# ZZWaang/polyphonic-chord-texture-disentanglement

Measured on AMD Instinct MI355X. Metric: 2-bar piano-roll samples/sec (train step), higher is better.
Workload: dtype bf16; 1 GPU; configs[1]: 1xMI355X batch=512/GPU, bf16 MFMA GRU/Linear, z_dim=256+256, teacher-forced decoder (tfr=1), fwd+bwd+clip+Adam; per_gpu_batch=512, global_batch=512, parallelism=dp1

## Files before the change

### include/ptvae_hip.h

```cpp
#ifndef PTVAE_HIP_H
#define PTVAE_HIP_H

#ifdef __cplusplus
extern "C" {
#endif

#define PTV_PREC_F32 0
#define PTV_PREC_BF16 1

#define PTV_A_BF16 1
#define PTV_B_BF16 2
#define PTV_C_BF16 4
#define PTV_GRU_GATES_BF16 1
#define PTV_GRU_GI_BF16 2
#define PTV_GRU_GI2_BF16 4
#define PTV_GRU_DG_BF16 8
#define PTV_GRU_W_BF16 16
#define PTV_GRU_EXT_BF16 64
#define PTV_GRU_SKIP_CAST0 32

const char* ptv_arch(void);
int ptv_abi_version(void);
const char* ptv_header_hash(void);

int ptv_gemm(int prec, int transA, int transB, int M, int N, int K,
             const void* A, long lda, const void* B, long ldb,
             void* C, long ldc, const float* bias, float alpha,
             int accumulate, int act, int splitk, int dtypes, void* stream);
int ptv_gemm_mtop(int prec, int transA, int transB, int M, int N, int K, const void* A, long lda, const void* B, long ldb,
                  void* C, long ldc, const float* bias, float alpha, int accumulate, int act, int splitk, int dtypes,
                  const int* m_top, long m_unit, void* stream);
int ptv_gemm_mtop_seg(int prec, int transA, int transB, int M, int N, int K, const void* A, long lda, const void* B, long ldb,
                      void* C, long ldc, const float* bias, float alpha, int accumulate, int act, int splitk, int dtypes,
                      const int* m_top, long m_unit, const int* seg_n, long seg_unit, int seg_period, void* stream);
int ptv_gemm_priority(int p);

int ptv_gru_seq_fwd(int prec, int M, int H, int T,
                    const void* gi, long gi_step_stride, long gi_ld,
                    const void* gi2, long gi2_step_stride, long gi2_ld,
                    const void* w_hh, const float* b_hh,
                    float* hall, void* hall16, void* gates,
                    const int* lengths, int reverse, const int* gi_idx, int flags, void* stream);

int ptv_gru_step_fwd(int prec, int M, int H,
                     const float* hprev, long ld_hprev, const void* hprev16, void* hout16,
                     const void* gi, long gi_ld, const void* gi2, long gi2_ld,
                     const void* w_hh, const float* b_hh,
                     float* hout, long ld_hout,
                     void* gates, long gates_plane,
                     const int* lengths, int t, const int* gi_idx, int flags, void* stream);

int ptv_gru_seq_bwd(int prec, int M, int H, int T,
                    const float* hall, const void* gates, const void* w_hh,
                    const void* dh_ext, long ext_step_stride, long ext_ld,
                    const float* dh_last, long last_ld,
                    const float* lr_a, long lr_step_stride, long lr_lda, int lr_k, const float* lr_b,
                    void* dgi, void* dgh, float* dhz, float* dh0,
                    int reverse, int flags, void* stream);

int ptv_gru_persist_supported(int NC, int M, int H);
int ptv_gru_persist_cu_reserve(int cus);
int ptv_gru_persist_load_policy(int lp);
int ptv_gru_persist_fwd(int NC, int M, int H, int T,
                        const void* const* gi, const long* gi_step, const long* gi_ld,
                        const void* const* gi2, const long* gi2_step, const long* gi2_ld,
                        const void* const* w_hh16, const float* const* b_hh,
                        float* const* hall, void* const* hall16, void* const* gates,
                        const int* const* lengths, const int* reverse, void* const* xch, unsigned* sync, void* stream);
int ptv_gru_persist_bwd(int NC, int M, int H, int T,
                        const float* const* hall, const void* const* gates, const void* const* w_t16,
                        const void* const* dh_ext, const long* ext_step, const long* ext_ld, const int* ext_bf16,
                        const float* const* dh_last, const long* last_ld,
                        void* const* dgi, void* const* dgh, float* const* dh0,
                        const int* reverse, void* const* xch, unsigned* sync, void* stream);
int ptv_gru_persist_splitk_supported(int NC, int M, int H, int S);
long ptv_gru_persist_part_elems(int NC, int M, int H, int S);
int ptv_gru_persist_bwd_splitk(int S, int NC, int M, int H, int T,
                               const float* const* hall, const void* const* gates, const void* const* w_t16,
                               const void* const* dh_ext, const long* ext_step, const long* ext_ld, const int* ext_bf16,
                               const float* const* dh_last, const long* last_ld,
                               void* const* dgi, void* const* dgh, float* const* dh0,
                               const int* reverse, void* const* xch, float* const* part, unsigned* sync, void* stream);

int ptv_copy2d(float* dst, long ldd, const float* src, long lds, long rows, int cols, float alpha,
               int accumulate, void* stream);
int ptv_transpose01(float* dst, const float* src, int D0, int D1, int W, void* stream);
int ptv_sum_steps(float* out, const void* in, long n, int T, long stride, int accumulate, int in_bf16, void* stream);
int ptv_zero_skip(int enable);
int ptv_last_nonzero_unit(const float* x, long rows, int cols, long ld, long unit, int* top, void* stream);
int ptv_sum_steps_top(float* out, const void* in, long n, int T, long stride, int accumulate, int in_bf16, const int* t_top,
                      void* stream);
int ptv_sum_steps_seg(float* out, const void* in, long n, int T, long stride, int accumulate, int in_bf16, const int* t_top,
                      const int* seg_n, long row_elems, void* stream);
int ptv_colsum(float* out, const void* A, long lda, long rows, int N, const int* sel, int G, int a_bf16, void* stream);

int ptv_embed_fwd(const long* x, const float* W, const float* bias, float* emb, int* lengths, int B, int E, void* stream);
int ptv_multihot(const long* x, float* out, long ld, int B, void* stream);
int ptv_grid_lengths(const long* x, int* lengths, int B, void* stream);
int ptv_multihot_bf16(const long* x, void* out, long ld, int B, void* stream);
int ptv_embed_fwd_geom(const long* x, const float* W, const float* bias, float* emb, int* lengths, int B, int E,
                       int S, int N, int P, int D, int pad, void* stream);
int ptv_grid_lengths_geom(const long* x, int* lengths, int B, int S, int N, int D, int pad, void* stream);
int ptv_multihot_geom(const long* x, void* out, long ld, int B, int S, int N, int P, int D, int bf16, void* stream);

int ptv_txt_conv_relu_pool_fwd(const float* pr_mat, const float* w, const float* bias, float* pooled, int B, int C, void* stream);
int ptv_txt_conv_relu_pool_bwd(const float* pr_mat, const float* w, const float* bias, const float* dpooled,
                               float* dw, float* dbias, int B, int C, void* stream);
int ptv_txt_conv_relu_pool_fwd_rows(const float* pr_mat, const float* w, const float* bias, float* feat, long ld, int B, int C,
                                    signed char* arg, void* stream);
int ptv_txt_conv_relu_pool_bwd_rows(const float* pr_mat, const float* w, const float* bias, const float* dfeat, long ld,
                                    float* dw, float* dbias, int B, int C, const signed char* arg, void* stream);

int ptv_philox_normal(float* out, long rows, int Z, unsigned long long seed, unsigned long long stream_id, long row_offset,
                      void* stream);
int ptv_reparam_kl_fwd(const float* mu, const float* sd, const float* eps, float* z, long ldz, float* kl_sum, int B, int Z, void* stream);
int ptv_reparam_kl_bwd(const float* mu, const float* sd, const float* eps, const float* dz, long lddz,
                       const float* dmu_ext, const float* dsd_ext, float klw, int mul_sd, float* dmu, float* dlv, int B, int Z, void* stream);

int ptv_pianotree_targets(const long* x, int B, int step_major, int* pitch_t, int* dur_t, int* counts, void* stream);
int ptv_pianotree_targets_rows(const long* x, int B, int step_major, int* pitch_t, int* dur_t, int* counts, int* row_live, void* stream);
int ptv_gather_rows(void* dst, const void* src, const int* idx, long rows, int row_words, long src_plane_words, long dst_plane_words, int planes,
                    void* stream);
int ptv_scatter_rows(void* dst, const void* src, const int* idx, long rows, int row_words, long src_plane_words, long dst_plane_words, int planes,
                     void* stream);
int ptv_gather_rows_seg(void* dst, const void* src, const int* idx, long rows, int row_words, long src_plane_words, long dst_plane_words,
                        int planes, const int* seg_n, void* stream);
int ptv_scatter_rows_seg(void* dst, const void* src, const int* idx, long rows, int row_words, long src_plane_words, long dst_plane_words,
                         int planes, const int* seg_n, void* stream);
int ptv_chord_targets(const float* c, int B, int step_major, int* root_t, int* chroma_t, int* bass_t, void* stream);
int ptv_ce_fwd(const float* logits, long ld, const int* targets, long rows, int C, int ignore_index, float* nll_sum, void* stream);
int ptv_ce_bwd(const float* logits, long ld, const int* targets, long rows, int C, int ignore_index, const float* gscale,
               float* dlogits, long ldd, void* stream);
int ptv_ce_group_fwd(const float* logits, long ld, const int* targets, long rows, int C, int ignore_index, int G,
                     float* nll_sum, int* count, void* stream);
int ptv_ce_group_bwd(const float* logits, long ld, const int* targets, long rows, int C, int ignore_index, int G,
// ... 413 lines not shown
```

### polyphonic_chord_texture_disentanglement_amd/csrc/composite.hip

```cpp
#include "common.hpp"
#include "../../include/ptvae_hip.h"

namespace {

inline const void* T_(const void* const* t, int i) { return t[i]; }
template <typename X> inline X* M_(const void* const* t, int i) { return reinterpret_cast<X*>(const_cast<void*>(t[i])); }

constexpr int A16 = 1, B16 = 2, C16 = 4, CBLK16 = 16;

struct WgradGroup {
  ptv_wgrad_job jobs[8]; int n = 0; int P; void* stream;
  WgradGroup(int prec, void* st) : P(prec), stream(st) {}
  int add(int M, int N, long K, const void* A, long lda, int a_bf16, const void* B, long ldb, int b_bf16, float* C, long ldc, float* csum,
          const int* k_top = nullptr, long k_unit = 0, int k_rev = 0, int accumulate = 1, const int* seg_n = nullptr, long seg_unit = 0,
          int seg_period = 0) {
    if (P == PTV_PREC_BF16 && K >= 512) {
      if (n == 8) PTV_TRY(flush());
      jobs[n++] = ptv_wgrad_job{M, N, (int)K, A, lda, B, ldb, C, ldc, 1.f, accumulate, (a_bf16 ? 1 : 0) | (b_bf16 ? 2 : 0), 0, csum, k_top, k_unit, k_rev,
                                seg_n, seg_n ? seg_unit : 0, seg_n ? seg_period : 0};
      return PTV_OK;
    }
    if (k_top) return PTV_ERR_ARG;
    PTV_TRY(ptv_gemm(P, 1, 1, M, N, (int)K, A, lda, B, ldb, C, ldc, nullptr, 1.f, accumulate, 0, 0, (a_bf16 ? A16 : 0) | (b_bf16 ? B16 : 0), stream));
    if (csum) PTV_TRY(ptv_colsum(csum, A, lda, K, M, nullptr, 1, a_bf16, stream));
// ... 123 lines not shown
  PTV_TRY(ptv_gemm(P, 0, 0, (int)TB, nr, H, hs, H, T_(t, PTV_CDF_W_ROOT), H, M_<void>(t, PTV_CDF_ROOT), nr, (const float*)T_(t, PTV_CDF_B_ROOT), 1.f, 0,
                   0, 0, 0, stream));
  PTV_TRY(ptv_gemm(P, 0, 0, (int)TB, nc, H, hs, H, T_(t, PTV_CDF_W_CHROMA), H, M_<void>(t, PTV_CDF_CHROMA), nc, (const float*)T_(t, PTV_CDF_B_CHROMA),
                   1.f, 0, 0, 0, 0, stream));
  PTV_TRY(ptv_gemm(P, 0, 0, (int)TB, nb, H, hs, H, T_(t, PTV_CDF_W_BASS), H, M_<void>(t, PTV_CDF_BASS), nb, (const float*)T_(t, PTV_CDF_B_BASS), 1.f, 0,
                   0, 0, 0, stream));
  return PTV_OK;
}

extern "C" int ptv_chord_decoder_bwd(const void* const* t, const long* d, void* stream) {
  if (!t || !d) return PTV_ERR_ARG;
  const int B = (int)d[PTV_CDB_D_B], T = (int)d[PTV_CDB_D_T], H = (int)d[PTV_CDB_D_H], I = (int)d[PTV_CDB_D_I], Z = (int)d[PTV_CDB_D_Z],
            Zi = (int)d[PTV_CDB_D_ZI], P = (int)d[PTV_CDB_D_PREC], abf = d[PTV_CDB_D_ACT_BF16] ? 1 : 0, persist = (int)d[PTV_CDB_D_PERSIST],
            S = (int)d[PTV_CDB_D_SPLITK];
  if (B <= 0 || T <= 0 || H <= 0 || I <= 0 || Z <= 0 || Zi <= 0 || (P != PTV_PREC_F32 && P != PTV_PREC_BF16)) return PTV_ERR_ARG;
  for (int i = 0; i < PTV_CDB_COUNT; i++) {
    const bool optional = i == PTV_CDB_WT16_HH || i == PTV_CDB_DROOT || i == PTV_CDB_DCHROMA || i == PTV_CDB_DBASS || i == PTV_CDB_DHZ ||
                          i == PTV_CDB_XCH || i == PTV_CDB_PART || i == PTV_CDB_SYNC || i == PTV_CDB_WAIT_EVENT || i == PTV_CDB_RECORD_EVENT;
    if (!t[i] && !optional) return PTV_ERR_ARG;
  }
  if (persist && (!t[PTV_CDB_WT16_HH] || !t[PTV_CDB_XCH] || !t[PTV_CDB_SYNC] || !abf || (S && !t[PTV_CDB_PART]))) return PTV_ERR_ARG;
  if (!persist && !t[PTV_CDB_DHZ]) return PTV_ERR_ARG;
  hipStream_t s = (hipStream_t)stream;
  const long TB = (long)T * B, ld_ih = (long)I + Zi;
  const float* hall = (const float*)T_(t, PTV_CDB_HALL);
  const float* hs = hall + (long)B * H;
  float* dhs = M_<float>(t, PTV_CDB_DHS);
  const int heads[3][4] = {{PTV_CDB_DROOT, PTV_CDB_W_ROOT, PTV_CDB_G_W_ROOT, PTV_CDB_G_B_ROOT},
                           {PTV_CDB_DCHROMA, PTV_CDB_W_CHROMA, PTV_CDB_G_W_CHROMA, PTV_CDB_G_B_CHROMA},
                           {PTV_CDB_DBASS, PTV_CDB_W_BASS, PTV_CDB_G_W_BASS, PTV_CDB_G_B_BASS}};
  const int ncls[3] = {(int)d[PTV_CDB_D_NROOT], (int)d[PTV_CDB_D_NCHROMA], (int)d[PTV_CDB_D_NBASS]};
  bool have = false;
  WgradGroup wg(P, stream);
  for (int k = 0; k < 3; k++) {
    const void* dl = T_(t, heads[k][0]);
    if (!dl) continue;
    const int n = ncls[k];
    PTV_TRY(ptv_gemm(P, 0, 1, (int)TB, H, n, dl, n, T_(t, heads[k][1]), H, dhs, H, nullptr, 1.f, have ? 1 : 0, 0, 0, 0, stream));
    have = true;
    PTV_TRY(wg.add(n, H, TB, dl, n, 0, hs, H, 0, M_<float>(t, heads[k][2]), H, M_<float>(t, heads[k][3])));
  }
  PTV_TRY(wg.flush());
  if (!have && hipMemsetAsync(dhs, 0, sizeof(float) * TB * H, s) != hipSuccess) return PTV_ERR_LAUNCH;
  void* dgi = M_<void>(t, PTV_CDB_DGI); void* dgh = M_<void>(t, PTV_CDB_DGH);
  float* dh0 = M_<float>(t, PTV_CDB_DH0);
  if (persist) {
    const float* hall_[1] = {hall}; const void* gates_[1] = {T_(t, PTV_CDB_GATES)}; const void* wt_[1] = {T_(t, PTV_CDB_WT16_HH)};
    const void* ext_[1] = {dhs}; const long ext_step[1] = {(long)B * H}, ext_ld[1] = {(long)H}; const int ext_bf[1] = {0};
    const float* last_[1] = {nullptr}; const long last_ld[1] = {0};
    void* dgi_[1] = {dgi}; void* dgh_[1] = {dgh}; float* dh0_[1] = {dh0}; const int rev[1] = {0};
    void* xch_[1] = {M_<void>(t, PTV_CDB_XCH)}; float* part_[1] = {M_<float>(t, PTV_CDB_PART)};
    if (t[PTV_CDB_WAIT_EVENT] && hipStreamWaitEvent(s, (hipEvent_t)const_cast<void*>(t[PTV_CDB_WAIT_EVENT]), 0) != hipSuccess) return PTV_ERR_LAUNCH;
    if (S) PTV_TRY(ptv_gru_persist_bwd_splitk(S, 1, B, H, T, hall_, gates_, wt_, ext_, ext_step, ext_ld, ext_bf, last_, last_ld, dgi_, dgh_, dh0_, rev,
                                              xch_, part_, M_<unsigned>(t, PTV_CDB_SYNC), stream));
    else PTV_TRY(ptv_gru_persist_bwd(1, B, H, T, hall_, gates_, wt_, ext_, ext_step, ext_ld, ext_bf, last_, last_ld, dgi_, dgh_, dh0_, rev, xch_,
                                     M_<unsigned>(t, PTV_CDB_SYNC), stream));
    if (t[PTV_CDB_RECORD_EVENT] && hipEventRecord((hipEvent_t)const_cast<void*>(t[PTV_CDB_RECORD_EVENT]), s) != hipSuccess) return PTV_ERR_LAUNCH;
  } else {
    const void* w = t[PTV_CDB_WT16_HH] ? T_(t, PTV_CDB_WT16_HH) : T_(t, PTV_CDB_W_HH);
    const int flags = abf | (abf << 3) | ((t[PTV_CDB_WT16_HH] ? 1 : 0) << 4);
    PTV_TRY(ptv_gru_seq_bwd(P, B, H, T, hall, T_(t, PTV_CDB_GATES), w, dhs, (long)B * H, H, nullptr, 0, nullptr, 0, 0, 0, nullptr, dgi, dgh,
                            M_<float>(t, PTV_CDB_DHZ), dh0, 0, flags, stream));
  }
  const int A = abf ? A16 : 0;
  float* dzg = M_<float>(t, PTV_CDB_DZG);
  PTV_TRY(ptv_sum_steps_top(dzg, dgi, (long)B * 3 * H, T, (long)B * 3 * H, 0, abf, nullptr, stream));
  float* g_ih = M_<float>(t, PTV_CDB_G_W_IH);
  const float* w_ih = (const float*)T_(t, PTV_CDB_W_IH);
  float* dz_in = M_<float>(t, PTV_CDB_DZ_IN); float* dtok0 = M_<float>(t, PTV_CDB_DTOK0);
  PTV_TRY(ptv_gemm(P, 0, 1, B, Zi, 3 * H, dzg, 3L * H, w_ih + I, ld_ih, dz_in, Zi, nullptr, 1.f, 0, 0, 0, 0, stream));
  PTV_TRY(ptv_gemm(P, 0, 1, B, I, 3 * H, dgi, 3L * H, w_ih, ld_ih, dtok0, I, nullptr, 1.f, 0, 0, 0, A, stream));
  float* dz = M_<float>(t, PTV_CDB_DZ);
  PTV_TRY(ptv_gemm(P, 0, 1, B, Z, H, dh0, H, T_(t, PTV_CDB_W_ZHID), Z, dz, Z, nullptr, 1.f, 0, 0, 0, 0, stream));
  PTV_TRY(ptv_gemm(P, 0, 1, B, Z, Zi, dz_in, Zi, T_(t, PTV_CDB_W_ZIN), Z, dz, Z, nullptr, 1.f, 1, 0, 0, 0, stream));
  PTV_TRY(wg.add(3 * H, H, TB, dgh, 3L * H, abf, hall, H, 0, M_<float>(t, PTV_CDB_G_W_HH), H, M_<float>(t, PTV_CDB_G_B_HH)));
  PTV_TRY(wg.add(3 * H, Zi, B, dzg, 3L * H, 0, T_(t, PTV_CDB_Z_IN), Zi, 0, g_ih + I, ld_ih, M_<float>(t, PTV_CDB_G_B_IH)));
  PTV_TRY(wg.add(3 * H, I, TB, dgi, 3L * H, abf, T_(t, PTV_CDB_TOKS), I, 0, g_ih, ld_ih, nullptr));
  PTV_TRY(wg.add(H, Z, B, dh0, H, 0, T_(t, PTV_CDB_Z), Z, 0, M_<float>(t, PTV_CDB_G_W_ZHID), Z, M_<float>(t, PTV_CDB_G_B_ZHID)));
  PTV_TRY(wg.add(Zi, Z, B, dz_in, Zi, 0, T_(t, PTV_CDB_Z), Z, 0, M_<float>(t, PTV_CDB_G_W_ZIN), Z, M_<float>(t, PTV_CDB_G_B_ZIN)));
  PTV_TRY(wg.flush());
  PTV_TRY(ptv_colsum(M_<float>(t, PTV_CDB_G_INIT_INPUT), dtok0, I, B, I, nullptr, 1, 0, stream));
  return PTV_OK;
}

extern "C" int ptv_decoder_tf_bwd(const void* const* t, const long* d, void* stream) {
  if (!t || !d) return PTV_ERR_ARG;
  for (int i = 0; i < PTV_DTB_COUNT; i++)
    if (!t[i] && i != PTV_DTB_TOP_H && i != PTV_DTB_PART_T && i != PTV_DTB_WAIT_EVENT && i != PTV_DTB_RECORD_EVENT && i != PTV_DTB_PERM &&
        i != PTV_DTB_ROW_LEN && i != PTV_DTB_NS16S && i != PTV_DTB_DNS_S && i != PTV_DTB_DTOK_S && i != PTV_DTB_SEG_N)
      return PTV_ERR_ARG;
  const bool sorted = t[PTV_DTB_PERM] != nullptr;
  if (sorted != (t[PTV_DTB_ROW_LEN] != nullptr) || sorted != (t[PTV_DTB_NS16S] != nullptr) || sorted != (t[PTV_DTB_DNS_S] != nullptr) ||
      sorted != (t[PTV_DTB_DTOK_S] != nullptr) || (sorted && !t[PTV_DTB_TOP_H]))
    return PTV_ERR_ARG;
  const int* perm = (const int*)T_(t, PTV_DTB_PERM);
  const int* row_len = (const int*)T_(t, PTV_DTB_ROW_LEN);

  const int B = (int)d[PTV_DTB_D_B], E = (int)d[PTV_DTB_D_E], He = (int)d[PTV_DTB_D_HE], Ht = (int)d[PTV_DTB_D_HT], Hn = (int)d[PTV_DTB_D_HN],
            Hd = (int)d[PTV_DTB_D_HD], NP = (int)d[PTV_DTB_D_NP], Zs = (int)d[PTV_DTB_D_ZS], Zi = (int)d[PTV_DTB_D_ZI], nblk = (int)d[PTV_DTB_D_NBLK],
            S = (int)d[PTV_DTB_D_SPLITK];
  const long ldp = d[PTV_DTB_D_LDP];
  if (B <= 0 || E != 128 || Hn != 512 || Hd != 64 || NP != 130 || ldp < NP || nblk <= 0 || (S && !t[PTV_DTB_PART_T])) return PTV_ERR_UNSUPPORTED;
  const int R = 32 * B;
  const int* seg_n = t[PTV_DTB_PERM] ? (const int*)T_(t, PTV_DTB_SEG_N) : nullptr;
  if (seg_n && !ptv_wgrad_seg_supported(15L * R, R)) return PTV_ERR_ARG;
  const long M = 15L * R;
  const int P = PTV_PREC_BF16;
  hipStream_t s = (hipStream_t)stream, side = (hipStream_t)const_cast<void*>(t[PTV_DTB_SIDE_STREAM]);
  void* sside = (void*)side;
  const int psz = ptv_dur_gru_bwd_part_size();
  const int* top_h = (const int*)T_(t, PTV_DTB_TOP_H);
  const long top_unit = top_h ? R : 0;
  auto fork = [&](int k) -> int {
    hipEvent_t e = (hipEvent_t)const_cast<void*>(t[PTV_DTB_FORK_EVENT0 + k]);
    if (hipEventRecord(e, s) != hipSuccess || hipStreamWaitEvent(side, e, 0) != hipSuccess) return PTV_ERR_LAUNCH;
    return PTV_OK;
  };
  float* G_ = nullptr; (void)G_;
#define GB(i) M_<float>(t, i)

  float* ddur = GB(PTV_DTB_DDUR); float* dHD0 = GB(PTV_DTB_DHD0); float* part = GB(PTV_DTB_PART);
  const void* HD16 = T_(t, PTV_DTB_HD16);
  ptv_gemm_priority(1);
  PTV_TRY(ptv_dur_gru_bwd(Hd, M, nullptr, M * Hd, 4 * M * Hd, HD16, M * Hd, 1, ddur, 10, (const float*)T_(t, PTV_DTB_W_HH_D),
                          (const float*)T_(t, PTV_DTB_W_OUT_D), (const int*)T_(t, PTV_DTB_IDX), M, dHD0, part, nblk,
                          (const float*)T_(t, PTV_DTB_B_HH_D), (const float*)T_(t, PTV_DTB_TAB0), (const float*)T_(t, PTV_DTB_TAB), stream));
  PTV_TRY(fork(0));
  ptv_gemm_priority(0);
  PTV_TRY(ptv_dur_out_wgrad(ddur, 10, HD16, M * Hd, GB(PTV_DTB_G_W_OUT_D), M, Hd, sside));
  PTV_TRY(ptv_colsum(GB(PTV_DTB_TMP64), ddur, 64, M * 10 / 64, 64, nullptr, 1, 0, sside));
  PTV_TRY(ptv_colsum(GB(PTV_DTB_G_B_OUT_D), GB(PTV_DTB_TMP64), 2, 32, 2, nullptr, 1, 0, sside));
  PTV_TRY(ptv_colsum(GB(PTV_DTB_S), part, psz, nblk, psz, nullptr, 1, 0, sside));
  PTV_TRY(ptv_dur_bwd_finalize(GB(PTV_DTB_S), GB(PTV_DTB_G_W_HH_D), GB(PTV_DTB_G_B_HH_D), GB(PTV_DTB_G_B_IH_D), GB(PTV_DTB_G_W_IH_D), GB(PTV_DTB_G_SOS),
                               (const float*)T_(t, PTV_DTB_W_IH_D), (const float*)T_(t, PTV_DTB_SOS), 5, sside));

  float* dP = GB(PTV_DTB_DP);
  void* dNSUM = M_<void>(t, PTV_DTB_DNSUM); void* dY16 = M_<void>(t, PTV_DTB_DY16);
  ptv_gemm_priority(1);
  PTV_TRY(ptv_heads_bwd_rows(dP, ldp, dHD0, T_(t, PTV_DTB_PK_WDPT), T_(t, PTV_DTB_PK_WCAT), dNSUM, top_h ? 3 : 1, dY16, top_h, top_unit, row_len, M,
                             stream));
  PTV_TRY(fork(1));
  ptv_gemm_priority(0);
  {
    const __bf16* HN16 = (const __bf16*)T_(t, PTV_DTB_HN16);
    const __bf16* nsum = HN16 + (long)R * Hn;
    float* tmp = GB(PTV_DTB_TMP200); float* cs = GB(PTV_DTB_CS200);
    WgradGroup wg(P, sside);
    PTV_TRY(wg.add(200, Hn, M, dY16, 200, 1, nsum, Hn, 1, tmp, Hn, cs, top_h, top_unit, 0, 0, seg_n, R, 15));
    PTV_TRY(wg.add(Hd, NP, M, dHD0, Hd, 0, T_(t, PTV_DTB_PITCH), ldp, 0, GB(PTV_DTB_G_W_DH) + Hn, (long)Hn + NP, nullptr, top_h, top_unit, 0, 1, seg_n, R, 15));
    PTV_TRY(wg.flush());
    PTV_TRY(ptv_copy2d(GB(PTV_DTB_G_W_P), Hn, tmp, Hn, NP, Hn, 1.f, 1, sside));
    PTV_TRY(ptv_copy2d(GB(PTV_DTB_G_B_P), NP, cs, NP, 1, NP, 1.f, 1, sside));
    PTV_TRY(ptv_copy2d(GB(PTV_DTB_G_W_DH), (long)Hn + NP, tmp + 136L * Hn, Hn, Hd, Hn, 1.f, 1, sside));
    PTV_TRY(ptv_copy2d(GB(PTV_DTB_G_B_DH), Hd, cs + 136, Hd, 1, Hd, 1.f, 1, sside));
  }

  void* dgi_n = M_<void>(t, PTV_DTB_DGI_N); void* dgh_n = M_<void>(t, PTV_DTB_DGH_N);
  float* dHN0 = GB(PTV_DTB_DHN0); int* top_step = M_<int>(t, PTV_DTB_TOP_STEP);
  float* dGC = GB(PTV_DTB_DGC);
  float* dNS_out = GB(PTV_DTB_DNS); float* dtok_out = GB(PTV_DTB_DTOK);
  float* dNS = sorted ? GB(PTV_DTB_DNS_S) : dNS_out;
  float* dtok = sorted ? GB(PTV_DTB_DTOK_S) : dtok_out;
  const __bf16* wt_ih_n = (const __bf16*)T_(t, PTV_DTB_WT_IH_N);
  ptv_gemm_priority(1);
  PTV_TRY(ptv_notes_gru_persist_bwd_rows(T_(t, PTV_DTB_PK_NOTES_WT), T_(t, PTV_DTB_HN16), T_(t, PTV_DTB_GATES_N), dNSUM, dgi_n, dgh_n, dHN0,
                                         M_<void>(t, PTV_DTB_SCRATCH_N), R, 15 | (seg_n ? 0x10000 : 0), top_h, row_len, top_step, stream));
  PTV_TRY(ptv_sum_steps_seg(dGC, dgi_n, (long)R * 3 * Hn, 15, (long)R * 3 * Hn, 0, 1, top_step, seg_n, 3L * Hn, stream));
  if (hipMemsetAsync(dtok_out + 15L * R * E, 0, sizeof(float) * R * E, s) != hipSuccess) return PTV_ERR_LAUNCH;
  PTV_TRY(ptv_gemm_mtop_seg(P, 0, 0, (int)M, E, 3 * Hn, dgi_n, 3L * Hn, wt_ih_n + (long)Ht * 3 * Hn, 3L * Hn, dtok, E, nullptr, 1.f, 0, 0, 0, A16 | B16,
                            top_step, R, seg_n, R, 15, stream));
  PTV_TRY(ptv_gemm(P, 0, 0, R, Ht, 3 * Hn, dGC, 3L * Hn, wt_ih_n, 3L * Hn, dNS, Ht, nullptr, 1.f, 0, 0, 0, B16, stream));
  PTV_TRY(ptv_gemm(P, 0, 0, R, Ht, Hn, dHN0, Hn, T_(t, PTV_DTB_WT_T2N), Hn, dNS, Ht, nullptr, 1.f, 1, 0, 0, B16, stream));
  if (sorted) {
    PTV_TRY(ptv_scatter_rows(dNS_out, dNS, perm, R, Ht, 0, 0, 1, stream));
    PTV_TRY(ptv_scatter_rows_seg(dtok_out, dtok, perm, R, E, (long)R * E, (long)R * E, 15, seg_n, stream));
  }
  PTV_TRY(fork(2));
  ptv_gemm_priority(0);
  {
    const __bf16* HN16 = (const __bf16*)T_(t, PTV_DTB_HN16);
    const __bf16* NSf = sorted ? (const __bf16*)T_(t, PTV_DTB_NS16S) : (const __bf16*)T_(t, PTV_DTB_NS16) + (long)B * Ht;
    float* gw = GB(PTV_DTB_G_W_HH_N); float* gb = GB(PTV_DTB_G_B_HH_N); float* gih = GB(PTV_DTB_G_W_IH_N);
    WgradGroup wg(P, sside);
    PTV_TRY(wg.add(2 * Hn, Hn, M, dgi_n, 3L * Hn, 1, HN16, Hn, 1, gw, Hn, gb, top_step, R, 0, 1, seg_n, R, 15));
    PTV_TRY(wg.add(Hn, Hn, M, dgh_n, Hn, 1, HN16, Hn, 1, gw + 2L * Hn * Hn, Hn, gb + 2 * Hn, top_step, R, 0, 1, seg_n, R, 15));
    PTV_TRY(wg.add(3 * Hn, Ht, R, dGC, 3L * Hn, 0, NSf, Ht, 1, gih, (long)Ht + E, GB(PTV_DTB_G_B_IH_N)));
    PTV_TRY(wg.add(3 * Hn, E, M, dgi_n, 3L * Hn, 1, T_(t, PTV_DTB_TOK_OP), E, 0, gih + Ht, (long)Ht + E, nullptr, top_step, R, 0, 1, seg_n, R, 15));
    PTV_TRY(wg.add(Hn, Ht, R, dHN0, Hn, 0, NSf, Ht, 1, GB(PTV_DTB_G_W_T2N), Ht, GB(PTV_DTB_G_B_T2N)));
    PTV_TRY(wg.flush());
  }

  void* dgi_t = M_<void>(t, PTV_DTB_DGI_T); void* dgh_t = M_<void>(t, PTV_DTB_DGH_T);
  float* dzhid = GB(PTV_DTB_DZHID); float* dZG = GB(PTV_DTB_DZG); float* dz_in = GB(PTV_DTB_DZ_IN); float* dTOKS = GB(PTV_DTB_DTOKS);
  float* dz = GB(PTV_DTB_DZ);
  const __bf16* wt_ih_t = (const __bf16*)T_(t, PTV_DTB_WT_IH_T);
  ptv_gemm_priority(1);
  {
    const float* hall_[1] = {(const float*)T_(t, PTV_DTB_NS)}; const void* gates_[1] = {T_(t, PTV_DTB_GATES_T)};
    const void* wt_[1] = {T_(t, PTV_DTB_WT_HH_T)};
    const void* ext_[1] = {dNS_out}; const long ext_step[1] = {(long)B * Ht}, ext_ld[1] = {(long)Ht}; const int ext_bf[1] = {0};
    const float* last_[1] = {nullptr}; const long last_ld[1] = {0};
    void* dgi_[1] = {dgi_t}; void* dgh_[1] = {dgh_t}; float* dh0_[1] = {dzhid}; const int rev[1] = {0};
    void* xch_[1] = {M_<void>(t, PTV_DTB_XCH)}; float* part_[1] = {M_<float>(t, PTV_DTB_PART_T)};
    if (t[PTV_DTB_WAIT_EVENT] && hipStreamWaitEvent(s, (hipEvent_t)const_cast<void*>(t[PTV_DTB_WAIT_EVENT]), 0) != hipSuccess) return PTV_ERR_LAUNCH;
    if (S) PTV_TRY(ptv_gru_persist_bwd_splitk(S, 1, B, Ht, 32, hall_, gates_, wt_, ext_, ext_step, ext_ld, ext_bf, last_, last_ld, dgi_, dgh_, dh0_,
                                              rev, xch_, part_, M_<unsigned>(t, PTV_DTB_SYNC), stream));
    else PTV_TRY(ptv_gru_persist_bwd(1, B, Ht, 32, hall_, gates_, wt_, ext_, ext_step, ext_ld, ext_bf, last_, last_ld, dgi_, dgh_, dh0_, rev, xch_,
                                     M_<unsigned>(t, PTV_DTB_SYNC), stream));
    if (t[PTV_DTB_RECORD_EVENT] && hipEventRecord((hipEvent_t)const_cast<void*>(t[PTV_DTB_RECORD_EVENT]), s) != hipSuccess) return PTV_ERR_LAUNCH;
  }
  PTV_TRY(ptv_sum_steps_top(dZG, dgi_t, (long)B * 3 * Ht, 32, (long)B * 3 * Ht, 0, 1, nullptr, stream));
  PTV_TRY(ptv_gemm(P, 0, 0, B, Zi, 3 * Ht, dZG, 3L * Ht, wt_ih_t + 2L * He * 3 * Ht, 3L * Ht, dz_in, Zi, nullptr, 1.f, 0, 0, 0, B16, stream));
  if (hipMemsetAsync(dTOKS + 32L * B * 2 * He, 0, sizeof(float) * B * 2 * He, s) != hipSuccess) return PTV_ERR_LAUNCH;
  PTV_TRY(ptv_gemm(P, 0, 0, R, 2 * He, 3 * Ht, dgi_t, 3L * Ht, wt_ih_t, 3L * Ht, dTOKS, 2L * He, nullptr, 1.f, 0, 0, 0, A16 | B16, stream));
  PTV_TRY(ptv_gemm(P, 0, 0, B, Zs, Ht, dzhid, Ht, T_(t, PTV_DTB_WT_ZHID), Ht, dz, Zs, nullptr, 1.f, 0, 0, 0, B16, stream));
  PTV_TRY(ptv_gemm(P, 0, 0, B, Zs, Zi, dz_in, Zi, T_(t, PTV_DTB_WT_ZIN), Zi, dz, Zs, nullptr, 1.f, 1, 0, 0, B16, stream));
  PTV_TRY(fork(3));
  ptv_gemm_priority(0);
  {
    const __bf16* NS16 = (const __bf16*)T_(t, PTV_DTB_NS16);
    float* g_ih = GB(PTV_DTB_G_W_IH_T); float* gb_ih = GB(PTV_DTB_G_B_IH_T); float* gb_hh = GB(PTV_DTB_G_B_HH_T);
    const long ld_t = 2L * He + Zi;
    WgradGroup wg(P, sside);
    PTV_TRY(wg.add(3 * Ht, Ht, R, dgh_t, 3L * Ht, 1, NS16, Ht, 1, GB(PTV_DTB_G_W_HH_T), Ht, gb_hh));
    PTV_TRY(wg.add(3 * Ht, Zi, B, dZG, 3L * Ht, 0, T_(t, PTV_DTB_Z_IN), Zi, 0, g_ih + 2 * He, ld_t, gb_ih));
    PTV_TRY(wg.add(3 * Ht, 2 * He, R, dgi_t, 3L * Ht, 1, T_(t, PTV_DTB_TOKS), 2L * He, 0, g_ih, ld_t, nullptr));
    PTV_TRY(wg.add(Ht, Zs, B, dzhid, Ht, 0, T_(t, PTV_DTB_Z), Zs, 0, GB(PTV_DTB_G_W_ZHID), Zs, GB(PTV_DTB_G_B_ZHID)));
    PTV_TRY(wg.add(Zi, Zs, B, dz_in, Zi, 0, T_(t, PTV_DTB_Z), Zs, 0, GB(PTV_DTB_G_W_ZIN), Zs, GB(PTV_DTB_G_B_ZIN)));
    PTV_TRY(wg.flush());
    PTV_TRY(ptv_colsum(GB(PTV_DTB_G_INIT_INPUT), dTOKS, 2L * He, B, 2 * He, nullptr, 1, 0, sside));
  }
  ptv_gemm_priority(1);
#undef GB
  return PTV_OK;
}

extern "C" int ptv_bigru_final_bwd(const void* const* t, const long* d, void* stream) {
  if (!t || !d) return PTV_ERR_ARG;
  const int M = (int)d[PTV_BGB_D_M], T = (int)d[PTV_BGB_D_T], H = (int)d[PTV_BGB_D_H], I = (int)d[PTV_BGB_D_I], xbf = d[PTV_BGB_D_X_BF16] ? 1 : 0,
            dx_acc = d[PTV_BGB_D_DX_ACC] ? 1 : 0, S = (int)d[PTV_BGB_D_SPLITK];
  if (M <= 0 || T < 2 || H <= 0 || I <= 0) return PTV_ERR_ARG;
  const bool want_dx = t[PTV_BGB_DX] != nullptr;
  for (int i = 0; i < PTV_BGB_COUNT; i++) {
    const bool optional = i == PTV_BGB_WT_IH0 || i == PTV_BGB_WT_IH1 || i == PTV_BGB_DX || i == PTV_BGB_PART0 || i == PTV_BGB_PART1 ||
                          i == PTV_BGB_WAIT_EVENT || i == PTV_BGB_RECORD_EVENT;
    if (!t[i] && !optional) return PTV_ERR_ARG;
  }
  if ((want_dx && (!t[PTV_BGB_WT_IH0] || !t[PTV_BGB_WT_IH1])) || (S && (!t[PTV_BGB_PART0] || !t[PTV_BGB_PART1]))) return PTV_ERR_ARG;
  const int P = PTV_PREC_BF16;
  hipStream_t s = (hipStream_t)stream, side = (hipStream_t)const_cast<void*>(t[PTV_BGB_SIDE_STREAM]);
  void* sside = (void*)side;
  const long TM = (long)T * M;
  const float* dout = (const float*)T_(t, PTV_BGB_DOUT);
  void* dgi[2] = {M_<void>(t, PTV_BGB_DGI0), M_<void>(t, PTV_BGB_DGI1)};
  void* dgh[2] = {M_<void>(t, PTV_BGB_DGH0), M_<void>(t, PTV_BGB_DGH1)};
  ptv_gemm_priority(1);
  {
    const float* hall_[2] = {(const float*)T_(t, PTV_BGB_HALL0), (const float*)T_(t, PTV_BGB_HALL1)};
    const void* gates_[2] = {T_(t, PTV_BGB_GATES0), T_(t, PTV_BGB_GATES1)};
    const void* wt_[2] = {T_(t, PTV_BGB_WT_HH0), T_(t, PTV_BGB_WT_HH1)};
    const void* ext_[2] = {nullptr, nullptr}; const long ext_step[2] = {0, 0}, ext_ld[2] = {0, 0}; const int ext_bf[2] = {0, 0};
    const float* last_[2] = {dout, dout + H}; const long last_ld[2] = {2L * H, 2L * H};
    float* dh0_[2] = {nullptr, nullptr}; const int rev[2] = {0, 1};
    void* xch_[2] = {M_<void>(t, PTV_BGB_XCH0), M_<void>(t, PTV_BGB_XCH1)};
    float* part_[2] = {M_<float>(t, PTV_BGB_PART0), M_<float>(t, PTV_BGB_PART1)};
    if (t[PTV_BGB_WAIT_EVENT] && hipStreamWaitEvent(s, (hipEvent_t)const_cast<void*>(t[PTV_BGB_WAIT_EVENT]), 0) != hipSuccess) return PTV_ERR_LAUNCH;
    if (S) PTV_TRY(ptv_gru_persist_bwd_splitk(S, 2, M, H, T, hall_, gates_, wt_, ext_, ext_step, ext_ld, ext_bf, last_, last_ld, dgi, dgh, dh0_, rev,
                                              xch_, part_, M_<unsigned>(t, PTV_BGB_SYNC), stream));
    else PTV_TRY(ptv_gru_persist_bwd(2, M, H, T, hall_, gates_, wt_, ext_, ext_step, ext_ld, ext_bf, last_, last_ld, dgi, dgh, dh0_, rev, xch_,
                                     M_<unsigned>(t, PTV_BGB_SYNC), stream));
    if (t[PTV_BGB_RECORD_EVENT] && hipEventRecord((hipEvent_t)const_cast<void*>(t[PTV_BGB_RECORD_EVENT]), s) != hipSuccess) return PTV_ERR_LAUNCH;
  }
  const void* x = T_(t, PTV_BGB_X);
  auto products = [&](int dir, void* st) -> int {
    const int o = dir ? 4 : 0;
    WgradGroup wg(P, st);
    PTV_TRY(wg.add(3 * H, I, TM, dgi[dir], 3L * H, 1, x, I, xbf, M_<float>(t, PTV_BGB_G_W_IH0 + o), I, M_<float>(t, PTV_BGB_G_B_IH0 + o)));
    PTV_TRY(wg.add(3 * H, H, TM, dgh[dir], 3L * H, 1, T_(t, dir ? PTV_BGB_H16_1 : PTV_BGB_H16_0), H, 1, M_<float>(t, PTV_BGB_G_W_HH0 + o), H,
                   M_<float>(t, PTV_BGB_G_B_HH0 + o), nullptr, 0, dir ? T : 0));
    return wg.flush();
  };
  hipEvent_t ef = (hipEvent_t)const_cast<void*>(t[PTV_BGB_FORK_EVENT]), ej = (hipEvent_t)const_cast<void*>(t[PTV_BGB_JOIN_EVENT]);
  if (hipEventRecord(ef, s) != hipSuccess || hipStreamWaitEvent(side, ef, 0) != hipSuccess) return PTV_ERR_LAUNCH;
  ptv_gemm_priority(0);
  PTV_TRY(products(1, sside));
  ptv_gemm_priority(1);
  PTV_TRY(products(0, stream));
  float* dx = M_<float>(t, PTV_BGB_DX);
  if (want_dx) PTV_TRY(ptv_gemm(P, 0, 0, (int)TM, I, 3 * H, dgi[0], 3L * H, T_(t, PTV_BGB_WT_IH0), 3L * H, dx, I, nullptr, 1.f, dx_acc, 0, 0, A16 | B16, stream));
  if (hipEventRecord(ej, side) != hipSuccess || hipStreamWaitEvent(s, ej, 0) != hipSuccess) return PTV_ERR_LAUNCH;
  if (want_dx) PTV_TRY(ptv_gemm(P, 0, 0, (int)TM, I, 3 * H, dgi[1], 3L * H, T_(t, PTV_BGB_WT_IH1), 3L * H, dx, I, nullptr, 1.f, 1, 0, 0, A16 | B16, stream));
  return PTV_OK;
}

extern "C" int ptv_bigru_final_fwd(const void* const* t, const long* d, void* stream) {
  if (!t || !d) return PTV_ERR_ARG;
  const int M = (int)d[PTV_BGF_D_M], T = (int)d[PTV_BGF_D_T], H = (int)d[PTV_BGF_D_H], I = (int)d[PTV_BGF_D_I], xbf = d[PTV_BGF_D_X_BF16] ? 1 : 0;
  if (M <= 0 || T < 2 || H <= 0 || I <= 0) return PTV_ERR_ARG;
  for (int i = 0; i < PTV_BGF_COUNT; i++)
    if (!t[i] && i != PTV_BGF_LENGTHS && i != PTV_BGF_WAIT_EVENT && i != PTV_BGF_RECORD_EVENT) return PTV_ERR_ARG;
  const int P = PTV_PREC_BF16;
  hipStream_t s = (hipStream_t)stream;
  const long TM = (long)T * M;
  const int gi_slot[2] = {PTV_BGF_GI0, PTV_BGF_GI1}, hall_slot[2] = {PTV_BGF_HALL0, PTV_BGF_HALL1};
  const int wih_slot[2] = {PTV_BGF_W16_IH0, PTV_BGF_W16_IH1}, bih_slot[2] = {PTV_BGF_B_IH0, PTV_BGF_B_IH1};
  for (int dir = 0; dir < 2; dir++) {
    PTV_TRY(ptv_gemm(P, 0, 0, (int)TM, 3 * H, I, T_(t, PTV_BGF_X), I, T_(t, wih_slot[dir]), I, M_<void>(t, gi_slot[dir]), 3L * H,
                     (const float*)T_(t, bih_slot[dir]), 1.f, 0, 0, -1, (xbf ? A16 : 0) | (d[PTV_BGF_D_WIH_F32] ? 0 : B16) | C16, stream));
    if (hipMemsetAsync(M_<void>(t, hall_slot[dir]), 0, sizeof(float) * M * H, s) != hipSuccess) return PTV_ERR_LAUNCH;
  }
  {
    const void* gi[2] = {T_(t, PTV_BGF_GI0), T_(t, PTV_BGF_GI1)}; const long gi_step[2] = {(long)M * 3 * H, (long)M * 3 * H}, gi_ld[2] = {3L * H, 3L * H};
    const void* gi2[2] = {nullptr, nullptr}; const long z2[2] = {0, 0};
    const void* w16[2] = {T_(t, PTV_BGF_W16_HH0), T_(t, PTV_BGF_W16_HH1)};
    const float* bhh[2] = {(const float*)T_(t, PTV_BGF_B_HH0), (const float*)T_(t, PTV_BGF_B_HH1)};
    float* hall[2] = {M_<float>(t, PTV_BGF_HALL0), M_<float>(t, PTV_BGF_HALL1)};
    void* h16[2] = {M_<void>(t, PTV_BGF_H16_0), M_<void>(t, PTV_BGF_H16_1)};
    void* gates[2] = {M_<void>(t, PTV_BGF_GATES0), M_<void>(t, PTV_BGF_GATES1)};
    const int* len[2] = {(const int*)T_(t, PTV_BGF_LENGTHS), (const int*)T_(t, PTV_BGF_LENGTHS)}; const int rev[2] = {0, 1};
    void* xch[2] = {M_<void>(t, PTV_BGF_XCH0), M_<void>(t, PTV_BGF_XCH1)};
    if (t[PTV_BGF_WAIT_EVENT] && hipStreamWaitEvent(s, (hipEvent_t)const_cast<void*>(t[PTV_BGF_WAIT_EVENT]), 0) != hipSuccess) return PTV_ERR_LAUNCH;
    PTV_TRY(ptv_gru_persist_fwd(2, M, H, T, gi, gi_step, gi_ld, gi2, z2, z2, w16, bhh, hall, h16, gates, len, rev, xch, M_<unsigned>(t, PTV_BGF_SYNC),
                                stream));
// ... 283 lines not shown
```

### polyphonic_chord_texture_disentanglement_amd/csrc/gemm.hip

```cpp
#include <stdlib.h>
#include <mutex>
#include <type_traits>
#include "common.hpp"
#include "gemm_core.hpp"
#include "../../include/ptvae_hip.h"

namespace ptv {

struct EpiPlain {
  struct Params {
    void* C; long ldc;
    const float* bias;
    float alpha;
    int accumulate;
    int act;
    int atomic;
    int c_bf16;
    int c_blocked;
    int c_rows;
    long split_stride;
  };
  static __device__ __forceinline__ long coff(const Params& p, int m, int n) {
    return p.c_blocked ? (((long)(n >> p.c_blocked) * p.c_rows + m) << p.c_blocked) + (n & ((1 << p.c_blocked) - 1)) : (long)m * p.ldc + n;
  }
  static __device__ __forceinline__ bool dead_is_noop(const Params& p) { return (p.accumulate || p.atomic) && p.act == 0 && p.bias == nullptr; }
  template <int FM, int FN, int NG> struct Pre {};
  template <int FM, int FN, int NG>
  static __device__ __forceinline__ void prefetch(const Params&, Pre<FM, FN, NG>&, int, int, int, int) {}
  template <int FN> static constexpr bool staged() { return FN == 2 || FN == 4; }
  template <int FM, int FN, int NG> static constexpr int lds_bytes() { return staged<FN>() ? 4 * RowStage<1, (staged<FN>() ? FN * 16 : 64)>::WAVE_BYTES : 0; }
  template <int FM, int FN, int NG>
  static __device__ __forceinline__ void apply(const Params& p_in, f32x4 (&acc)[FM][NG * FN], const Pre<FM, FN, NG>&,
                                               int m0, int n0, int M, int N, int split, char* lds) {
    Params q = p_in;
    if (q.split_stride) q.C = reinterpret_cast<float*>(q.C) + (long)split * q.split_stride;
    const Params& p = q;
    const bool bf = p.c_bf16 != 0;
    const bool vec = (p.c_blocked || (p.ldc & 3) == 0) && ((reinterpret_cast<uintptr_t>(p.C) & (bf ? 7 : 15)) == 0);
    const bool use_bias = p.bias != nullptr && split == 0;
    if constexpr (staged<FN>()) {
      using RS = RowStage<1, FN * 16>;
      float* st = RS::base(lds);
      const int u = RS::unit();
      const bool bias_ok = !use_bias || (reinterpret_cast<uintptr_t>(p.bias) & 15) == 0;
      if (vec && bias_ok && p.act == 0 && m0 + 16 * FM <= M && n0 + 16 * FN <= N && !(bf && p.atomic)) {
        const int mode = p.atomic ? 3 : (p.accumulate ? (bf ? 4 : 2) : (bf ? 1 : 0));
        float4 b4 = make_float4(0.f, 0.f, 0.f, 0.f);
        if (use_bias) b4 = *reinterpret_cast<const float4*>(p.bias + n0 + u);
        if (mode == 0) fast_rows<FM, FN, 0>(p, acc, st, m0, n0 + u, b4);
        else if (mode == 1) fast_rows<FM, FN, 1>(p, acc, st, m0, n0 + u, b4);
        else if (mode == 2) fast_rows<FM, FN, 2>(p, acc, st, m0, n0 + u, b4);
        else if (mode == 4) fast_rows<FM, FN, 4>(p, acc, st, m0, n0 + u, b4);
        else fast_rows<FM, FN, 3>(p, acc, st, m0, n0 + u, b4);
        return;
      }
#pragma unroll
      for (int i = 0; i < FM; i++) {
        RS::put(st, acc[i]);
#pragma unroll
        for (int c = 0; c < RS::PASSES; c++) {
          const int row = RS::row(c), m = m0 + i * 16 + row, n = n0 + u;
          if (m < M && n < N) cell(p, m, n, N, RS::get(st, row, u), bf, vec, use_bias);
        }
        __builtin_amdgcn_wave_barrier();
      }
    } else {
      const int lane = threadIdx.x & 63;
#pragma unroll
      for (int i = 0; i < FM; i++)
#pragma unroll
        for (int j = 0; j < FN; j++) {
          const int m = m0 + i * 16 + (lane & 15), n = n0 + j * 16 + (lane >> 4) * 4;
          if (m < M && n < N) cell(p, m, n, N, acc[i][j], bf, vec, use_bias);
        }
    }
  }
  template <int FM, int FN, int MODE>
  static __device__ __forceinline__ void fast_rows(const Params& p, f32x4 (&acc)[FM][FN], float* st, int m0, int n, const float4& b4) {
    using RS = RowStage<1, FN * 16>;
    const int u = RS::unit();
#pragma unroll
    for (int i = 0; i < FM; i++) {
      RS::put(st, acc[i]);
#pragma unroll
      for (int c = 0; c < RS::PASSES; c++) {
        const int row = RS::row(c);
        const f32x4 a = RS::get(st, row, u);
        const long off = coff(p, m0 + i * 16 + row, n);
        float v0 = p.alpha * a[0] + b4.x, v1 = p.alpha * a[1] + b4.y, v2 = p.alpha * a[2] + b4.z, v3 = p.alpha * a[3] + b4.w;
        if constexpr (MODE == 1 || MODE == 4) {
          if constexpr (MODE == 4) {
            const bf16x4 q = *reinterpret_cast<const bf16x4*>(reinterpret_cast<const __bf16*>(p.C) + off);
            v0 += (float)q[0]; v1 += (float)q[1]; v2 += (float)q[2]; v3 += (float)q[3];
          }
          bf16x4 o; o[0] = (__bf16)v0; o[1] = (__bf16)v1; o[2] = (__bf16)v2; o[3] = (__bf16)v3;
          *reinterpret_cast<bf16x4*>(reinterpret_cast<__bf16*>(p.C) + off) = o;
        } else if constexpr (MODE == 3) {
          float* cp = reinterpret_cast<float*>(p.C) + off;
          atomicAdd(cp, v0); atomicAdd(cp + 1, v1); atomicAdd(cp + 2, v2); atomicAdd(cp + 3, v3);
        } else {
          float4* cp = reinterpret_cast<float4*>(reinterpret_cast<float*>(p.C) + off);
          if constexpr (MODE == 2) { const float4 q = *cp; v0 += q.x; v1 += q.y; v2 += q.z; v3 += q.w; }
          *cp = make_float4(v0, v1, v2, v3);
        }
      }
      __builtin_amdgcn_wave_barrier();
    }
  }
  static __device__ __forceinline__ void cell(const Params& p, int m, int n, int N, const f32x4& a, bool bf, bool vec, bool use_bias) {
    float v[4];
#pragma unroll
    for (int e = 0; e < 4; e++) {
      v[e] = p.alpha * a[e];
      if (use_bias && n + e < N) v[e] += p.bias[n + e];
      if (p.act == 1) v[e] = expf(v[e]);
    }
    const long off = coff(p, m, n);
    if (p.atomic) {
      float* c = reinterpret_cast<float*>(p.C) + off;
#pragma unroll
      for (int e = 0; e < 4; e++) if (n + e < N) atomicAdd(c + e, v[e]);
    } else if (vec && n + 3 < N) {
      if (p.accumulate) { const float4 q = ld4f(p.C, off, bf); v[0] += q.x; v[1] += q.y; v[2] += q.z; v[3] += q.w; }
      st4f(p.C, off, bf, v[0], v[1], v[2], v[3]);
    } else {
#pragma unroll
      for (int e = 0; e < 4; e++) if (n + e < N) st1f(p.C, off + e, bf, p.accumulate ? ld1f(p.C, off + e, bf) + v[e] : v[e]);
    }
  }
};

#ifndef PTV_PF_TN
#define PTV_PF_TN 3
#endif
#ifndef PTV_PF_NT
#define PTV_PF_NT 2
#endif
#define PLAIN_PF_BIG(KA, KB, SA, SB) ((SA) && (SB) ? ((KA) ? PTV_PF_TN : PTV_PF_NT) : 1)

template <class CT, int BM, int BN, int WGM, int WGN, bool KA, bool KB, bool SA, bool SB>
__global__ __launch_bounds__(NTHREADS, 2) void gemm_plain_kernel(GemmArgs g, EpiPlain::Params ep) {
  if (g.prio) __builtin_amdgcn_s_setprio(3);
  gemm_body<CT, BM, BN, WGM, WGN, 1, KA, KB, EpiPlain, SA, SB, (BM * BN <= 64 * 64 ? 2 : PLAIN_PF_BIG(KA, KB, SA, SB))>(g, ep);
}

__global__ void splitk_reduce_kernel(float* __restrict__ C, long ldc, const float* __restrict__ ws, int M, int N, int splits, int accumulate) {
  const long total = (long)M * N;
  for (long i = (long)blockIdx.x * blockDim.x + threadIdx.x; i < total; i += (long)gridDim.x * blockDim.x) {
    float sum = 0.f;
    for (int z = 0; z < splits; z++) sum += ws[(long)z * total + i];
    float* cp = C + (i / N) * ldc + (i % N);
    *cp = (accumulate ? *cp : 0.f) + sum;
  }
}

__global__ void fill_rows_kernel(float* C, long ldc, int M, int N, float v) {
  long i = (long)blockIdx.x * blockDim.x + threadIdx.x;
  long total = (long)M * N;
  for (; i < total; i += (long)gridDim.x * blockDim.x) C[(i / N) * ldc + (i % N)] = v;
}

template <class CT, int BM, int BN, bool KA, bool KB, bool SA, bool SB>
static void launch_plain(const GemmArgs& g, const EpiPlain::Params& ep, int splits, hipStream_t s) {
  dim3 grid(cdiv(g.N, BN), cdiv(g.M, BM), splits);
  hipLaunchKernelGGL((gemm_plain_kernel<CT, BM, BN, 2, 2, KA, KB, SA, SB>), grid, dim3(NTHREADS), 0, s, g, ep);
}

int g_splitk_ordered = [] { const char* e = getenv("PTV_WGRAD_ORDERED"); return (e && e[0] == '0') ? 0 : 1; }();

static float* splitk_workspace(hipStream_t s, size_t bytes) {
  struct Buf { float* p; size_t bytes; };
  static Buf pool[64]; static hipStream_t keys[64]; static int n = 0; static std::mutex mu;
  std::lock_guard<std::mutex> lock(mu);
  int i = 0;
  for (; i < n; i++) if (keys[i] == s) break;
  if (i == n) { if (n == 64) return nullptr; keys[n++] = s; pool[i] = Buf{nullptr, 0}; }
  Buf& b = pool[i];
  if (b.bytes < bytes) {
    hipStreamCaptureStatus st = hipStreamCaptureStatusNone;
    if (hipStreamIsCapturing(s, &st) == hipSuccess && st != hipStreamCaptureStatusNone) return nullptr;
    const size_t want = bytes + bytes / 4;
    if (hipMalloc(reinterpret_cast<void**>(&b.p), want) != hipSuccess) { b = Buf{nullptr, 0}; return nullptr; }
    b.bytes = want;
  }
  return b.p;
}

template <class CT, bool SA, bool SB>
static int gemm_dispatch(int transA, int transB, GemmArgs g, EpiPlain::Params ep, int splitk, hipStream_t s) {
  const long blocks_big = (long)cdiv(g.M, 128) * cdiv(g.N, 128);
  const bool deepk = transA && g.K >= 4096;
  const bool big = blocks_big >= 192 || (deepk && g.M >= 256 && g.N >= 256);
  const int bm = big ? 128 : 64;
  long blocks = (long)cdiv(g.M, bm) * cdiv(g.N, bm);
  int splits = 1;
  if (splitk > 0) splits = splitk;
  else if (splitk == 0 && blocks < 256 && g.K >= 8 * CT::BK && ep.act == 0 && !ep.c_bf16) {
    const long target = deepk ? (big ? 640 : 1536) : 512;
    splits = (int)((target + blocks - 1) / blocks);
    int maxs = g.K / (4 * CT::BK);
    if (splits > maxs) splits = maxs;
    if (splits > 192) splits = 192;
    if (splits < 1) splits = 1;
  }
  int kper = g.K;
  if (splits > 1) {
    if (splits >= 8) splits = (splits + 7) / 8 * 8;
    kper = cdiv(cdiv(g.K, splits), CT::BK) * CT::BK;
    const int s2 = cdiv(g.K, kper);
    if (s2 != splits && (s2 & 7) != 0 && s2 >= 8) {
      splits = s2 / 8 * 8;
      kper = cdiv(cdiv(g.K, splits), CT::BK) * CT::BK;
      splits = cdiv(g.K, kper);
    } else splits = s2;
  }
  g.k_per_split = kper;
  float* ws = nullptr;
  const EpiPlain::Params ep_user = ep;
  if (splits > 1 && g_splitk_ordered) {
    ws = splitk_workspace(s, (size_t)splits * g.M * g.N * sizeof(float));
    if (!ws) g_ord_fallbacks++;
  }
  if (ws) {
    ep.C = ws; ep.ldc = g.N; ep.accumulate = 0; ep.atomic = 0; ep.split_stride = (long)g.M * g.N;
  } else if (splits > 1) {
    ep.atomic = 1;
    if (!ep.accumulate) {
      long total = (long)g.M * g.N;
      int nb = (int)((total + 255) / 256); if (nb > 2048) nb = 2048;
      hipLaunchKernelGGL(fill_rows_kernel, dim3(nb), dim3(256), 0, s, reinterpret_cast<float*>(ep.C), ep.ldc, g.M, g.N, 0.f);
    }
  }
#define PTV_LAUNCH(KA, KB)                                              \
  do {                                                                  \
    if (big) launch_plain<CT, 128, 128, KA, KB, SA, SB>(g, ep, splits, s);      \
    else launch_plain<CT, 64, 64, KA, KB, SA, SB>(g, ep, splits, s);            \
  } while (0)
  if (!transA && !transB) PTV_LAUNCH(false, false);
  else if (!transA && transB) PTV_LAUNCH(false, true);
  else if (transA && transB) PTV_LAUNCH(true, true);
  else PTV_LAUNCH(true, false);
#undef PTV_LAUNCH
  if (ws) {
    const long total = (long)g.M * g.N;
    int nb = (int)((total + 255) / 256); if (nb > 2048) nb = 2048;
    hipLaunchKernelGGL(splitk_reduce_kernel, dim3(nb), dim3(256), 0, s, reinterpret_cast<float*>(ep_user.C), ep_user.ldc, ws, g.M, g.N, splits, ep_user.accumulate);
  }
  return PTV_OK;
}

}

namespace ptv { int g_gemm_prio = 0; }
extern "C" int ptv_gemm_priority(int p) { ptv::g_gemm_prio = p ? 1 : 0; return PTV_OK; }

extern "C" int ptv_gemm_mtop(int prec, int transA, int transB, int M, int N, int K,
                             const void* A, long lda, const void* B, long ldb,
                             void* C, long ldc, const float* bias, float alpha,
                             int accumulate, int act, int splitk, int dtypes, const int* m_top, long m_unit, void* stream) {
  return ptv_gemm_mtop_seg(prec, transA, transB, M, N, K, A, lda, B, ldb, C, ldc, bias, alpha, accumulate, act, splitk, dtypes, m_top, m_unit, nullptr, 0, 0,
                           stream);
}

extern "C" int ptv_gemm_mtop_seg(int prec, int transA, int transB, int M, int N, int K,
                                 const void* A, long lda, const void* B, long ldb,
                                 void* C, long ldc, const float* bias, float alpha,
                                 int accumulate, int act, int splitk, int dtypes, const int* m_top, long m_unit,
                                 const int* seg_n, long seg_unit, int seg_period, void* stream) {
  if (M < 0 || N < 0 || K < 0 || !A || !B || !C) return PTV_ERR_ARG;
  if (M == 0 || N == 0) return PTV_OK;
  const bool sa = dtypes & 1, sb = dtypes & 2, sc = dtypes & 4;
  if ((sa || sb) && prec != PTV_PREC_BF16) return PTV_ERR_ARG;
  if (sc && splitk > 1) return PTV_ERR_ARG;
  if ((dtypes & 8) && (dtypes & 16)) return PTV_ERR_ARG;
  if ((dtypes & 8) && ((N & 31) || splitk > 1)) return PTV_ERR_ARG;
  if ((dtypes & 16) && ((N & 15) || splitk > 1)) return PTV_ERR_ARG;
  if ((dtypes & 24) && splitk == 0) splitk = 1;
  if (prec == PTV_PREC_BF16 && transA && transB && !sc && !(dtypes & 24) && !bias && act == 0 && K >= 512 && splitk <= 0)
    return ptv_wgrad(M, N, K, A, lda, B, ldb, reinterpret_cast<float*>(C), ldc, alpha, accumulate, dtypes & 3, 0, nullptr, nullptr, 0, 0, stream);
  if (m_top && (transA || m_unit <= 0)) return PTV_ERR_ARG;
  if (seg_n && (transA || seg_unit <= 0 || (seg_unit & 127) || seg_period <= 0)) return PTV_ERR_ARG;
  ptv::GemmArgs g{A, lda, B, ldb, M, N, K, K, 0, m_top, m_unit, ptv::g_gemm_prio, seg_n, (int)seg_unit, seg_period};
  ptv::EpiPlain::Params ep{C, ldc, bias, alpha, accumulate, act, 0, sc ? 1 : 0, (dtypes & 8) ? 5 : ((dtypes & 16) ? 4 : 0), M, 0};
  hipStream_t s = (hipStream_t)stream;
  int rc;
  if (prec != PTV_PREC_BF16) rc = ptv::gemm_dispatch<ptv::F32, false, false>(transA, transB, g, ep, splitk, s);
  else if (sa && sb) rc = ptv::gemm_dispatch<ptv::BF16, true, true>(transA, transB, g, ep, splitk, s);
  else if (sa) rc = ptv::gemm_dispatch<ptv::BF16, true, false>(transA, transB, g, ep, splitk, s);
  else if (sb) rc = ptv::gemm_dispatch<ptv::BF16, false, true>(transA, transB, g, ep, splitk, s);
  else rc = ptv::gemm_dispatch<ptv::BF16, false, false>(transA, transB, g, ep, splitk, s);
  if (rc != PTV_OK) return rc;
  PTV_CHECK_LAUNCH();
  return PTV_OK;
}

extern "C" int ptv_gemm(int prec, int transA, int transB, int M, int N, int K,
                        const void* A, long lda, const void* B, long ldb,
                        void* C, long ldc, const float* bias, float alpha,
                        int accumulate, int act, int splitk, int dtypes, void* stream) {
  return ptv_gemm_mtop(prec, transA, transB, M, N, K, A, lda, B, ldb, C, ldc, bias, alpha, accumulate, act, splitk, dtypes, nullptr, 0, stream);
}
```

### polyphonic_chord_texture_disentanglement_amd/csrc/gemm_core.hpp

```cpp
#pragma once
#include <hip/hip_runtime.h>
#include <stdint.h>
#include <type_traits>

namespace ptv {

typedef __attribute__((ext_vector_type(8))) __bf16 bf16x8;
typedef __attribute__((ext_vector_type(4))) __bf16 bf16x4;
typedef __attribute__((ext_vector_type(4))) float f32x4;

constexpr int NTHREADS = 256;

__device__ __forceinline__ float4 ld4f(const void* p, long i, bool bf) {
  if (bf) {
    const bf16x4 v = *reinterpret_cast<const bf16x4*>(reinterpret_cast<const __bf16*>(p) + i);
    return make_float4((float)v[0], (float)v[1], (float)v[2], (float)v[3]);
  }
  return *reinterpret_cast<const float4*>(reinterpret_cast<const float*>(p) + i);
}
__device__ __forceinline__ void st4f(void* p, long i, bool bf, float a, float b, float c, float d) {
  if (bf) {
    bf16x4 v; v[0] = (__bf16)a; v[1] = (__bf16)b; v[2] = (__bf16)c; v[3] = (__bf16)d;
    *reinterpret_cast<bf16x4*>(reinterpret_cast<__bf16*>(p) + i) = v;
  } else {
    *reinterpret_cast<float4*>(reinterpret_cast<float*>(p) + i) = make_float4(a, b, c, d);
  }
}
__device__ __forceinline__ float ld1f(const void* p, long i, bool bf) {
  return bf ? (float)reinterpret_cast<const __bf16*>(p)[i] : reinterpret_cast<const float*>(p)[i];
}
__device__ __forceinline__ void st1f(void* p, long i, bool bf, float v) {
  if (bf) reinterpret_cast<__bf16*>(p)[i] = (__bf16)v; else reinterpret_cast<float*>(p)[i] = v;
}

struct BF16 {
  using T = __bf16;
  static constexpr int BK = 64;
  static constexpr int LDS_LD = 64;
  static constexpr int CH = 8;
};
struct F32 {
  using T = float;
  static constexpr int BK = 32;
  static constexpr int LDS_LD = 32;
  static constexpr int CH = 4;
};

struct GemmArgs {
  const void* A; long lda;
  const void* B; long ldb;
  int M, N, K;
  int k_per_split;
  long gate_stride;
  const int* m_top; long m_unit;
  int prio;
  const int* seg_n = nullptr; int seg_unit = 0, seg_period = 0;
};

template <class CT> __device__ __forceinline__ int swz(int row, int k) {
  return row * CT::LDS_LD + ((((k / CT::CH) ^ ((row >> 2) ^ row)) & 7) * CT::CH) + (k % CT::CH);
}

template <bool SB> struct SrcT { using T = float; };
template <> struct SrcT<true> { using T = __bf16; };

template <class CT, bool SB> struct Chunk;
template <> struct Chunk<BF16, false> {
  float4 lo, hi;
  __device__ __forceinline__ void zero() { lo = hi = make_float4(0.f, 0.f, 0.f, 0.f); }
  __device__ __forceinline__ void set(int e, float x) { if (e < 4) (&lo.x)[e] = x; else (&hi.x)[e - 4] = x; }
  __device__ __forceinline__ void load16(const float* q) { lo = *reinterpret_cast<const float4*>(q); hi = *reinterpret_cast<const float4*>(q + 4); }
  __device__ __forceinline__ void store(__bf16* d) const {
    bf16x8 v;
    v[0] = (__bf16)lo.x; v[1] = (__bf16)lo.y; v[2] = (__bf16)lo.z; v[3] = (__bf16)lo.w;
    v[4] = (__bf16)hi.x; v[5] = (__bf16)hi.y; v[6] = (__bf16)hi.z; v[7] = (__bf16)hi.w;
    *reinterpret_cast<bf16x8*>(d) = v;
  }
};
template <> struct Chunk<BF16, true> {
  bf16x8 v;
  __device__ __forceinline__ void zero() { for (int e = 0; e < 8; e++) v[e] = (__bf16)0.f; }
  __device__ __forceinline__ void set(int e, __bf16 x) { v[e] = x; }
  __device__ __forceinline__ void load16(const __bf16* q) { v = *reinterpret_cast<const bf16x8*>(q); }
  __device__ __forceinline__ void store(__bf16* d) const { *reinterpret_cast<bf16x8*>(d) = v; }
};
template <> struct Chunk<F32, false> {
  float4 lo;
  __device__ __forceinline__ void zero() { lo = make_float4(0.f, 0.f, 0.f, 0.f); }
  __device__ __forceinline__ void set(int e, float x) { (&lo.x)[e] = x; }
  __device__ __forceinline__ void load16(const float* q) { lo = *reinterpret_cast<const float4*>(q); }
  __device__ __forceinline__ void store(float* d) const { *reinterpret_cast<float4*>(d) = lo; }
};

template <class CT, int ROWS, bool SB>
struct StageKC {
  using S = typename SrcT<SB>::T;
  static constexpr int CPR = 8;
  static constexpr int RPP = NTHREADS / CPR;
  static constexpr int NP = ROWS / RPP;
  static_assert(ROWS % RPP == 0, "tile rows must be a multiple of 32");
  Chunk<CT, SB> v[NP];

  template <class RowMap>
  __device__ __forceinline__ void load(const S* __restrict__ p, long ld, int k0, int kend, bool vec_ok, RowMap rowmap) {
    const int tid = threadIdx.x;
    const int c = tid % CPR, r0 = tid / CPR;
    const int k = k0 + c * CT::CH;
#pragma unroll
    for (int i = 0; i < NP; i++) {
// ... 164 lines not shown
  template <class BRow>
  static __device__ __forceinline__ void run(const float* As, int a_row0, const float* Bs, BRow b_row, f32x4 (&acc)[FM][FNT]) {
    const int lane = threadIdx.x & 63;
    const int r = lane & 15, kq = (lane >> 4) * 4;
#pragma unroll
    for (int ks = 0; ks < F32::BK; ks += 16) {
      float4 a[FM], b[FNT];
#pragma unroll
      for (int i = 0; i < FM; i++) a[i] = *reinterpret_cast<const float4*>(As + swz<F32>(a_row0 + i * 16 + r, ks + kq));
#pragma unroll
      for (int j = 0; j < FNT; j++) b[j] = *reinterpret_cast<const float4*>(Bs + swz<F32>(b_row(j) + r, ks + kq));
#pragma unroll
      for (int i = 0; i < FM; i++)
#pragma unroll
        for (int j = 0; j < FNT; j++) {
          acc[i][j] = __builtin_amdgcn_mfma_f32_16x16x4f32(b[j].x, a[i].x, acc[i][j], 0, 0, 0);
          acc[i][j] = __builtin_amdgcn_mfma_f32_16x16x4f32(b[j].y, a[i].y, acc[i][j], 0, 0, 0);
          acc[i][j] = __builtin_amdgcn_mfma_f32_16x16x4f32(b[j].z, a[i].z, acc[i][j], 0, 0, 0);
          acc[i][j] = __builtin_amdgcn_mfma_f32_16x16x4f32(b[j].w, a[i].w, acc[i][j], 0, 0, 0);
        }
    }
  }
};

template <int NG, int W>
struct RowStage {
  static_assert(W == 32 || W == 64, "wave tiles of 32 or 64 units");
  static constexpr int NF = NG * W / 16;
  static constexpr int S = NG * W + 4;
  static constexpr int WAVE_BYTES = 16 * S * 4;
  static constexpr int PASSES = W == 64 ? 4 : 2;
  static __device__ __forceinline__ float* base(char* lds) { return reinterpret_cast<float*>(lds) + (threadIdx.x >> 6) * (16 * S); }
  static __device__ __forceinline__ void put(float* st, const f32x4 (&a)[NF]) {
    const int lane = threadIdx.x & 63;
    float* w = st + (lane & 15) * S + (lane >> 4) * 4;
#pragma unroll
    for (int f = 0; f < NF; f++) *reinterpret_cast<f32x4*>(w + f * 16) = a[f];
    __builtin_amdgcn_wave_barrier();
  }
  static __device__ __forceinline__ int row(int ps) {
    const int lane = threadIdx.x & 63, q = (lane >> 2) & 7;
    const int grp = (lane >> 5) * 2 + ((0x96 >> q) & 1);
    return W == 64 ? ps * 4 + grp : ps * 4 + grp + 8 * (q >> 2);
  }
  static __device__ __forceinline__ int unit() {
    const int lane = threadIdx.x & 63, q = (lane >> 2) & 7;
    return W == 64 ? ((q >> 1) * 4 + (lane & 3)) * 4 : (((q >> 1) & 1) * 4 + (lane & 3)) * 4;
  }
  static __device__ __forceinline__ f32x4 get(const float* st, int r, int col) {
    return *reinterpret_cast<const f32x4*>(st + r * S + col);
  }
};

template <class CT, int BM, int BN, int WGM, int WGN, int NG, bool KMAJOR_A, bool KMAJOR_B, class Epi, bool SA = false, bool SB = false, int PF = 1>
__device__ __forceinline__ void gemm_body(const GemmArgs& g, const typename Epi::Params& ep) {
  static_assert(WGM * WGN == 4, "4 waves");
  static_assert(!(NG == 3 && KMAJOR_B), "gate gather needs K-contiguous weights");
  using T = typename CT::T;
  constexpr int WTM = BM / WGM, WTN = BN / WGN;
  constexpr int FM = WTM / 16, FN = WTN / 16;
  constexpr int BROWS = NG * BN;
  constexpr int MAIN_BYTES = (BM + BROWS) * CT::LDS_LD * (int)sizeof(T);
  constexpr int EPI_BYTES = Epi::template lds_bytes<FM, FN, NG>();
  __shared__ __attribute__((aligned(16))) char smem[MAIN_BYTES > EPI_BYTES ? MAIN_BYTES : EPI_BYTES];
  T* As = reinterpret_cast<T*>(smem);
  T* Bs = As + BM * CT::LDS_LD;

  const int ntn = gridDim.x, ntm = gridDim.y, nsp = gridDim.z;
  const int bid = blockIdx.x + ntn * (blockIdx.y + ntm * blockIdx.z);
  const int per = ntm * ntn;
  int mt, nt, split;
  if (nsp > 1 && (nsp & 7) == 0) {
    const int slot = bid >> 3;
    split = (bid & 7) + 8 * (slot / per);
    const int tile = slot % per;
    mt = tile / ntn; nt = tile % ntn;
  } else if (nsp == 1 && g.M >= g.N && (ntm & 7) == 0) {
    const int slot = bid >> 3;
    split = 0;
    mt = (slot / ntn) * 8 + (bid & 7); nt = slot % ntn;
  } else if (nsp == 1 && g.M < g.N && (ntn & 7) == 0) {
    const int slot = bid >> 3;
    split = 0;
    nt = (slot / ntm) * 8 + (bid & 7); mt = slot % ntm;
  } else {
    split = bid / per;
    const int tile = bid % per;
    mt = tile / ntn; nt = tile % ntn;
  }
  const int m_blk = mt * BM, n_blk = nt * BN;
  const int kbeg = split * g.k_per_split;
  const bool dead = (g.m_top != nullptr && m_blk >= ((long)*g.m_top + 1) * g.m_unit) ||
                    (g.seg_n != nullptr && (m_blk % g.seg_unit) >= g.seg_n[(m_blk / g.seg_unit) % g.seg_period]);
  if (dead && Epi::dead_is_noop(ep)) return;
  const int kend = dead ? kbeg : min(g.K, kbeg + g.k_per_split);
  const int wave = threadIdx.x >> 6;
  const int wm = wave / WGN, wn = wave % WGN;

  static_assert(!(SA || SB) || std::is_same<CT, BF16>::value, "bf16 sources feed the bf16 MFMA path only");
  using TA = typename SrcT<SA>::T;
  using TB = typename SrcT<SB>::T;
  const TA* Ap = reinterpret_cast<const TA*>(g.A);
  const TB* Bp = reinterpret_cast<const TB*>(g.B);
  const bool vecA = ((g.lda & (SA ? 7 : 3)) == 0) && ((reinterpret_cast<uintptr_t>(g.A) & 15) == 0);
  const bool vecB = ((g.ldb & (SB ? 7 : 3)) == 0) && ((reinterpret_cast<uintptr_t>(g.B) & 15) == 0);

  auto rowmapA = [&](int r) -> long { long m = m_blk + r; return m < g.M ? m : -1; };
  auto rowmapB = [&](int r) -> long {
    const int gate = r / BN, jj = r % BN;
    long n = n_blk + jj;
    return n < g.N ? (long)gate * g.gate_stride + n : -1;
  };

  typename std::conditional<KMAJOR_A, StageKM<CT, BM, SA>, StageKC<CT, BM, SA>>::type sa[PF];
  typename std::conditional<KMAJOR_B, StageKM<CT, BROWS, SB>, StageKC<CT, BROWS, SB>>::type sb[PF];

  typename Epi::template Pre<FM, FN, NG> pre;
  Epi::template prefetch<FM, FN, NG>(ep, pre, m_blk + wm * WTM, n_blk + wn * WTN, g.M, g.N);

  f32x4 acc[FM][NG * FN];
#pragma unroll
  for (int i = 0; i < FM; i++)
#pragma unroll
    for (int j = 0; j < NG * FN; j++) acc[i][j] = f32x4{0.f, 0.f, 0.f, 0.f};

  const bool fullA = vecA && (m_blk + BM <= g.M);
  const bool fullB = vecB && (n_blk + BN <= g.N);
  auto rowfastA = [&](int r) -> long { return m_blk + r; };
  auto rowfastB = [&](int r) -> long { return (long)(r / BN) * g.gate_stride + n_blk + (r % BN); };
  static_assert(BN % 32 == 0 && BM % 32 == 0, "row passes must not straddle a gate block");
  auto load_tiles = [&](auto& sa_, auto& sb_, int k0) {
    const bool kfull = k0 + CT::BK <= kend;
    if (fullA && kfull) {
      if constexpr (KMAJOR_A) sa_.load_fast(Ap, g.lda, k0, m_blk);
      else sa_.load_fast(Ap, g.lda, k0, rowfastA);
    } else {
      if constexpr (KMAJOR_A) sa_.load(Ap, g.lda, k0, kend, vecA, m_blk, g.M);
      else sa_.load(Ap, g.lda, k0, kend, vecA, rowmapA);
    }
    if (fullB && kfull) {
      if constexpr (KMAJOR_B) sb_.load_fast(Bp, g.ldb, k0, n_blk);
      else sb_.load_fast(Bp, g.ldb, k0, rowfastB);
    } else {
      if constexpr (KMAJOR_B) sb_.load(Bp, g.ldb, k0, kend, vecB, n_blk, g.N);
      else sb_.load(Bp, g.ldb, k0, kend, vecB, rowmapB);
    }
  };
  auto fast_tiles = [&](auto& sa_, auto& sb_, int k0) {
    if constexpr (KMAJOR_A) sa_.load_fast(Ap, g.lda, k0, m_blk);
    else sa_.load_fast(Ap, g.lda, k0, rowfastA);
    if constexpr (KMAJOR_B) sb_.load_fast(Bp, g.ldb, k0, n_blk);
    else sb_.load_fast(Bp, g.ldb, k0, rowfastB);
  };
  auto consume = [&](auto& sa_, auto& sb_) {
    __syncthreads();
    sa_.store(As);
    sb_.store(Bs);
    __syncthreads();
  };
  auto mma = [&]() {
    TileMma<CT, FM, NG * FN>::run(As, wm * WTM, Bs,
                                  [&](int j) { return (j / FN) * BN + wn * WTN + (j % FN) * 16; }, acc);
  };

  int k0 = kbeg;
  {
    if (fullA && fullB && kbeg + 2 * PF * CT::BK <= kend) {
#pragma unroll
      for (int p = 0; p < PF; p++) fast_tiles(sa[p], sb[p], k0 + p * CT::BK);
      for (; k0 + 2 * PF * CT::BK <= kend; k0 += PF * CT::BK) {
#pragma unroll
        for (int p = 0; p < PF; p++) {
          consume(sa[p], sb[p]);
          fast_tiles(sa[p], sb[p], k0 + (PF + p) * CT::BK);
          mma();
        }
      }
#pragma unroll
      for (int p = 0; p < PF; p++) {
        consume(sa[p], sb[p]);
        mma();
      }
      k0 += PF * CT::BK;
    }
  }
  if (k0 < kend) load_tiles(sa[0], sb[0], k0);
  for (; k0 < kend; k0 += CT::BK) {
    consume(sa[0], sb[0]);
    if (k0 + CT::BK < kend) load_tiles(sa[0], sb[0], k0 + CT::BK);
    mma();
  }
  if constexpr (EPI_BYTES > 0) __syncthreads();
  Epi::template apply<FM, FN, NG>(ep, acc, pre, m_blk + wm * WTM, n_blk + wn * WTN, g.M, g.N, split, smem);
}

}
```

### polyphonic_chord_texture_disentanglement_amd/csrc/gru_persist.hip

```cpp
#include "common.hpp"
#include "prof.hpp"
#include "gemm_core.hpp"
#include "../../include/ptvae_hip.h"

namespace ptv {

typedef __attribute__((ext_vector_type(4))) unsigned u32x4;
typedef __attribute__((address_space(1))) unsigned gu32;
typedef __attribute__((address_space(1))) unsigned long long gu64;

constexpr int PU = 16;
constexpr int PMAXC = 4;
constexpr int PLDS = 96 * 1024;
constexpr unsigned SPIN_LIMIT = 4000000u;

struct PChainF {
  const __bf16* w_hh; const float* b_hh;
  const __bf16* gi; long gi_step, gi_ld;
  const __bf16* gi2; long gi2_step, gi2_ld;
  float* hall; __bf16* hall16; __bf16* gates;
  __bf16* xch;
  const int* lengths; int reverse;
};
struct PGruFwdArgs {
  PChainF c[PMAXC];
  int NC, M, H, T, RG, UG, rows_wg, dbg;
  unsigned* sync;
};

struct PChainB {
  const __bf16* w_t;
  const float* hall; const __bf16* gates;
  const void* dh_ext; long ext_step, ext_ld; int ext_bf16;
  const float* dh_last; long last_ld;
  __bf16* dgi; __bf16* dgh; float* dh0;
  __bf16* xch;
  int reverse;
  float* part;
};
struct PGruBwdArgs {
  PChainB c[PMAXC];
  int NC, M, H, T, RG, UG, rows_wg, dbg;
  unsigned* sync;
};

__device__ __forceinline__ __amdgpu_buffer_rsrc_t make_rsrc(const void* p, long bytes) {
  return __builtin_amdgcn_make_buffer_rsrc(const_cast<void*>(p), 0, (int)(bytes > 0x7fffffffL ? 0x7fffffffL : bytes), 0x00020000);
}
__device__ __forceinline__ bf16x8 as_bf16x8(const u32x4& v) {
  union { u32x4 u; bf16x8 b; } x; x.u = v; return x.b;
}
__device__ __forceinline__ void store_bf16x4_sc1(__bf16* p, float a, float b, float c, float d) {
  union { bf16x4 v; unsigned long long u; } x;
  x.v[0] = (__bf16)a; x.v[1] = (__bf16)b; x.v[2] = (__bf16)c; x.v[3] = (__bf16)d;
  __hip_atomic_store((gu64*)(reinterpret_cast<unsigned long long*>(p)), x.u, __ATOMIC_RELAXED, __HIP_MEMORY_SCOPE_AGENT);
}
__device__ __forceinline__ float4 ld_bf16x4(const __bf16* p) {
  const bf16x4 v = *reinterpret_cast<const bf16x4*>(p);
  return make_float4((float)v[0], (float)v[1], (float)v[2], (float)v[3]);
}
__device__ __forceinline__ void st_bf16x4(__bf16* p, float a, float b, float c, float d) {
  bf16x4 v; v[0] = (__bf16)a; v[1] = (__bf16)b; v[2] = (__bf16)c; v[3] = (__bf16)d;
  *reinterpret_cast<bf16x4*>(p) = v;
}

__device__ __forceinline__ void block_map(int G, int UG, int& grp, int& idx) {
  const int bid = blockIdx.x, nW = G * UG;
  if (G <= 8 && (8 % G) == 0 && (nW & 7) == 0) {
    const int per = 8 / G, x = bid & 7;
    grp = x / per; idx = (x % per) * (nW >> 3) + (bid >> 3);
  } else { grp = bid / UG; idx = bid % UG; }
}

template <int NBR, class RowOff>
__device__ __forceinline__ void load_w_slice(__bf16* Ws, const __bf16* src, int K, RowOff rowoff) {
  const int cpr = K >> 3;
  for (int c = threadIdx.x; c < NBR * cpr; c += NTHREADS) {
    const int r = c / cpr, kc = c - r * cpr;
    const bf16x8 v = *reinterpret_cast<const bf16x8*>(src + rowoff(r) + kc * 8);
    *reinterpret_cast<bf16x8*>(Ws + (kc >> 3) * (NBR * 64) + swz<BF16>(r, (kc & 7) * 8)) = v;
  }
}

template <bool ACQ>
__device__ __forceinline__ void wait_arrivals(gu32* cnt, unsigned target, gu32* err, bool& dead) {
  if (threadIdx.x == 0) {
    if (!dead) {
      unsigned spins = 0;
      while (__hip_atomic_load(cnt, __ATOMIC_RELAXED, __HIP_MEMORY_SCOPE_AGENT) < target) {
        __builtin_amdgcn_s_sleep(1);
        if (++spins > SPIN_LIMIT) { __hip_atomic_store(err, 1u, __ATOMIC_RELAXED, __HIP_MEMORY_SCOPE_AGENT); dead = true; break; }
      }
    }
    if (ACQ) __builtin_amdgcn_fence(__ATOMIC_ACQUIRE, "agent");
  }
  __syncthreads();
}
__device__ __forceinline__ void publish(gu32* cnt) {
  asm volatile("s_waitcnt vmcnt(0)" ::: "memory");
  __syncthreads();
  if (threadIdx.x == 0) __hip_atomic_fetch_add(cnt, 1u, __ATOMIC_RELAXED, __HIP_MEMORY_SCOPE_AGENT);
}

template <int LP> struct LoadAux { static constexpr int v = LP == 0 ? 16 : (LP == 1 ? 2 : 0); };
template <int FM, int KU, int NB, int LP>
struct PMma {
  u32x4 buf[2][KU][FM];
  unsigned kstride;
  __device__ __forceinline__ void load(int b, __amdgpu_buffer_rsrc_t rs, const unsigned (&rowoff)[FM], int kb0) {
#pragma unroll
    for (int j = 0; j < KU; j++)
#pragma unroll
      for (int i = 0; i < FM; i++) buf[b][j][i] = __builtin_amdgcn_raw_buffer_load_b128(rs, rowoff[i] + (unsigned)(kb0 + j) * kstride, 0, LoadAux<LP>::v);
// ... 97 lines not shown
        z[e] = sigmoid_fast(iz[e] + acc[i][1][e] + bZ[e]);
        hn[e] = acc[i][2][e] + bN[e];
        n[e] = tanh_fast(in_[e] + r[e] * hn[e]);
        if (!live) { r[e] = 0.f; z[e] = 1.f; n[e] = 0.f; }
        h[e] = (1.0f - z[e]) * n[e] + z[e] * hP[e];
      }
      hp[i] = make_float4(h[0], h[1], h[2], h[3]);
      gR[i] = make_float4(r[0], r[1], r[2], r[3]); gZ[i] = make_float4(z[0], z[1], z[2], z[3]);
      gN[i] = make_float4(n[0], n[1], n[2], n[3]); gHN[i] = make_float4(hn[0], hn[1], hn[2], hn[3]);
      if (ok[i] && !(a.dbg & 8)) store_bf16x4_sc1(c.xch + (long)(s + 1) * MH + ((long)xc * M + row[i]) * 8 + xe, h[0], h[1], h[2], h[3]);
    }
    if (s + 1 < T && !(a.dbg & 2)) publish(cnt);
#pragma unroll
    for (int i = 0; i < FM; i++) {
      if (ok[i] && !(a.dbg & 8)) {
        const long o = (long)row[i] * H + u;
        *reinterpret_cast<float4*>(c.hall + (long)(s + 1) * MH + o) = hp[i];
        st_bf16x4(c.hall16 + (long)(s + 1) * MH + o, hp[i].x, hp[i].y, hp[i].z, hp[i].w);
        if (c.gates) {
          __bf16* gp = c.gates + (long)s * 4 * MH + o;
          st_bf16x4(gp, gR[i].x, gR[i].y, gR[i].z, gR[i].w);
          st_bf16x4(gp + MH, gZ[i].x, gZ[i].y, gZ[i].z, gZ[i].w);
          st_bf16x4(gp + 2 * MH, gN[i].x, gN[i].y, gN[i].z, gN[i].w);
          st_bf16x4(gp + 3 * MH, gHN[i].x, gHN[i].y, gHN[i].z, gHN[i].w);
        }
      }
    }
  }
}

template <int FM, int KU, int LP>
__global__ __launch_bounds__(NTHREADS, 2) void pgru_bwd_kernel(PGruBwdArgs a) {
  __builtin_amdgcn_s_setprio(3);
  __shared__ __attribute__((aligned(16))) char smem[PLDS];
  __bf16* Ws = reinterpret_cast<__bf16*>(smem);
  int grp, ug;
  block_map(a.NC * a.RG, a.UG, grp, ug);
  const int ch = grp / a.RG, rg = grp - ch * a.RG;
  const PChainB& c = a.c[ch];
  const int H = a.H, M = a.M, T = a.T;
  const long MH = (long)M * H, M3H = 3 * MH;
  const int u0 = ug * PU;
  gu32* cnt = (gu32*)(a.sync + 16 * (1 + grp));
  gu32* err = (gu32*)(a.sync);

  load_w_slice<16>(Ws, c.w_t, 3 * H, [&](int r) { return (long)(u0 + r) * 3 * H; });
  __syncthreads();

  const int lane = threadIdx.x & 63, wave = threadIdx.x >> 6;
  const int rl = lane & 15, kq = lane >> 4;
  const int u = u0 + kq * 4;
  const int row0 = rg * a.rows_wg + wave * (FM * 16);
  int row[FM]; bool ok[FM]; unsigned rowoff[FM]; float4 dhz[FM];
#pragma unroll
  for (int i = 0; i < FM; i++) {
    const int r = row0 + i * 16 + rl;
    ok[i] = r < M; row[i] = r < M ? r : M - 1;
    rowoff[i] = (unsigned)(((long)kq * M + row[i]) * 16);
    dhz[i] = make_float4(0.f, 0.f, 0.f, 0.f);
  }
  bool dead = false;
  PMma<FM, KU, 1, LP> mm;
  mm.kstride = (unsigned)M * 64u;
  const int xe = (kq & 1) * 4;
  const int nkb = (3 * H) >> 5;

  for (int step = T - 1; step >= (c.dh0 ? -1 : 0); step--) {
    const int t = step < 0 ? 0 : (c.reverse ? T - 1 - step : step);
    const bool last = step == T - 1;
    float4 gr[FM], gz[FM], gn[FM], gh[FM], hpv[FM], ex[FM];
    if (step >= 0) {
#pragma unroll
      for (int i = 0; i < FM; i++) {
        const long o = (long)row[i] * H + u;
        const __bf16* gp = c.gates + (long)step * 4 * MH + o;
        gr[i] = ld_bf16x4(gp); gz[i] = ld_bf16x4(gp + MH); gn[i] = ld_bf16x4(gp + 2 * MH); gh[i] = ld_bf16x4(gp + 3 * MH);
        hpv[i] = *reinterpret_cast<const float4*>(c.hall + (long)step * MH + o);
        float4 e = make_float4(0.f, 0.f, 0.f, 0.f);
        if (c.dh_ext) {
          const long eo = (long)step * c.ext_step + (long)row[i] * c.ext_ld + u;
          e = c.ext_bf16 ? ld_bf16x4(reinterpret_cast<const __bf16*>(c.dh_ext) + eo) : *reinterpret_cast<const float4*>(reinterpret_cast<const float*>(c.dh_ext) + eo);
        }
        if (last && c.dh_last) {
          const float4 q = *reinterpret_cast<const float4*>(c.dh_last + (long)row[i] * c.last_ld + u);
          e.x += q.x; e.y += q.y; e.z += q.z; e.w += q.w;
        }
        ex[i] = e;
      }
    }
    f32x4 acc[FM][1];
#pragma unroll
    for (int i = 0; i < FM; i++) acc[i][0] = f32x4{0.f, 0.f, 0.f, 0.f};
    if (!last) {
      wait_arrivals<LP == 2>(cnt, (unsigned)(a.UG * (T - 1 - step)), err, dead);
      mm.run(make_rsrc(c.xch + (long)(step + 1) * M3H, M3H * 2), rowoff, Ws, nkb, acc);
    }
    if (step < 0) {
#pragma unroll
      for (int i = 0; i < FM; i++)
        if (ok[i]) *reinterpret_cast<float4*>(c.dh0 + (long)row[i] * H + u) =
            make_float4(acc[i][0][0] + dhz[i].x, acc[i][0][1] + dhz[i].y, acc[i][0][2] + dhz[i].z, acc[i][0][3] + dhz[i].w);
      break;
    }
    float4 dR[FM], dZ[FM], dN[FM], dNR[FM];
#pragma unroll
    for (int i = 0; i < FM; i++) {
      const float dzn[4] = {dhz[i].x, dhz[i].y, dhz[i].z, dhz[i].w}, e1[4] = {ex[i].x, ex[i].y, ex[i].z, ex[i].w};
      const float R[4] = {gr[i].x, gr[i].y, gr[i].z, gr[i].w}, Z[4] = {gz[i].x, gz[i].y, gz[i].z, gz[i].w};
      const float N[4] = {gn[i].x, gn[i].y, gn[i].z, gn[i].w}, HN[4] = {gh[i].x, gh[i].y, gh[i].z, gh[i].w};
      const float hP[4] = {hpv[i].x, hpv[i].y, hpv[i].z, hpv[i].w};
      float dr[4], dz[4], dn[4], dnr[4], dq[4];
#pragma unroll
      for (int e = 0; e < 4; e++) {
        const float dh = acc[i][0][e] + dzn[e] + e1[e];
        dn[e] = dh * (1.0f - Z[e]) * (1.0f - N[e] * N[e]);
        dz[e] = dh * (hP[e] - N[e]) * Z[e] * (1.0f - Z[e]);
        dr[e] = dn[e] * HN[e] * R[e] * (1.0f - R[e]);
        dnr[e] = dn[e] * R[e];
        dq[e] = dh * Z[e];
      }
      dhz[i] = make_float4(dq[0], dq[1], dq[2], dq[3]);
      dR[i] = make_float4(dr[0], dr[1], dr[2], dr[3]); dZ[i] = make_float4(dz[0], dz[1], dz[2], dz[3]);
      dN[i] = make_float4(dn[0], dn[1], dn[2], dn[3]);
      dNR[i] = make_float4(dnr[0], dnr[1], dnr[2], dnr[3]);
      if (ok[i]) {
        __bf16* px = c.xch + (long)step * M3H + (long)row[i] * 8 + xe;
        store_bf16x4_sc1(px + (long)((u) >> 3) * M * 8, dr[0], dr[1], dr[2], dr[3]);
        store_bf16x4_sc1(px + (long)((H + u) >> 3) * M * 8, dz[0], dz[1], dz[2], dz[3]);
        store_bf16x4_sc1(px + (long)((2 * H + u) >> 3) * M * 8, dnr[0], dnr[1], dnr[2], dnr[3]);
      }
    }
    if (step > 0 || c.dh0) publish(cnt);
#pragma unroll
    for (int i = 0; i < FM; i++) {
      if (ok[i]) {
        __bf16* ph = c.dgh + (long)step * M3H + (long)row[i] * 3 * H + u;
        st_bf16x4(ph, dR[i].x, dR[i].y, dR[i].z, dR[i].w);
        st_bf16x4(ph + H, dZ[i].x, dZ[i].y, dZ[i].z, dZ[i].w);
        st_bf16x4(ph + 2 * H, dNR[i].x, dNR[i].y, dNR[i].z, dNR[i].w);
        __bf16* pi = c.dgi + (long)t * M3H + (long)row[i] * 3 * H + u;
        st_bf16x4(pi, dR[i].x, dR[i].y, dR[i].z, dR[i].w);
        st_bf16x4(pi + H, dZ[i].x, dZ[i].y, dZ[i].z, dZ[i].w);
        st_bf16x4(pi + 2 * H, dN[i].x, dN[i].y, dN[i].z, dN[i].w);
      }
    }
  }
}

__device__ __forceinline__ u32x4 as_u32x4(const f32x4& v) { union { f32x4 f; u32x4 u; } x; x.f = v; return x.u; }
__device__ __forceinline__ f32x4 as_f32x4(const u32x4& v) { union { u32x4 u; f32x4 f; } x; x.u = v; return x.f; }

template <int FM, int KU, int S>
__global__ __launch_bounds__(NTHREADS, 2) void pgru_bwd_sk_kernel(PGruBwdArgs a) {
  __builtin_amdgcn_s_setprio(3);
  __shared__ __attribute__((aligned(16))) char smem[PLDS];
  __bf16* Ws = reinterpret_cast<__bf16*>(smem);
  int grp, idx;
  block_map(a.NC * a.RG, a.UG, grp, idx);
  const int ch = grp / a.RG, rg = grp - ch * a.RG;
  const int team = idx / S, ks = idx - team * S;
  const PChainB& c = a.c[ch];
  const int H = a.H, M = a.M, T = a.T;
  const long MH = (long)M * H, M3H = 3 * MH;
  const int KS = 3 * H / S;
  const int uq0 = team * (PU * S), u0 = uq0 + ks * PU;
  const int TPG = a.UG / S;
  gu32* cnt = (gu32*)(a.sync + 16 * (1 + grp));
  gu32* tcnt = (gu32*)(a.sync + 16 * (33 + grp * TPG + team));
  gu32* err = (gu32*)(a.sync);

  load_w_slice<PU * S>(Ws, c.w_t + (long)ks * KS, KS, [&](int r) { return (long)(uq0 + r) * 3 * H; });
  __syncthreads();

  const int lane = threadIdx.x & 63, wave = threadIdx.x >> 6;
  const int rl = lane & 15, kq = lane >> 4;
  const int u = u0 + kq * 4;
  const int rw0 = wave * (FM * 16);
  const int row0 = rg * a.rows_wg + rw0;
  int row[FM]; bool ok[FM]; unsigned rowoff[FM]; float4 dhz[FM];
#pragma unroll
  for (int i = 0; i < FM; i++) {
    const int r = row0 + i * 16 + rl;
    ok[i] = r < M; row[i] = r < M ? r : M - 1;
    rowoff[i] = (unsigned)(((long)kq * M + row[i]) * 16);
    dhz[i] = make_float4(0.f, 0.f, 0.f, 0.f);
  }
  bool dead = false;
  PMma<FM, KU, S, 0> mm;
  mm.kstride = (unsigned)M * 64u;
  const int xe = (kq & 1) * 4;
  const int nkb = KS >> 5;
  const long xks = (long)ks * KS * M;
  const long ptile = (long)a.rows_wg * 16;
  const long pteam = (long)S * S * ptile, pslot = (long)a.RG * TPG * pteam;
  float* pbase = c.part + ((long)rg * TPG + team) * pteam;
  const unsigned plane = (unsigned)(((rw0 + rl) * 16 + kq * 4) * 4);

  for (int step = T - 1; step >= (c.dh0 ? -1 : 0); step--) {
    const int t = step < 0 ? 0 : (c.reverse ? T - 1 - step : step);
    const bool last = step == T - 1;
    f32x4 own[FM];
#pragma unroll
    for (int i = 0; i < FM; i++) own[i] = f32x4{0.f, 0.f, 0.f, 0.f};
    __amdgpu_buffer_rsrc_t prs = make_rsrc(pbase + ((step + 1) & 1) * pslot, pteam * 4);
    if (!last) {
      wait_arrivals<false>(cnt, (unsigned)(a.UG * (T - 1 - step)), err, dead);
      f32x4 acc[FM][S];
#pragma unroll
      for (int i = 0; i < FM; i++)
#pragma unroll
        for (int j = 0; j < S; j++) acc[i][j] = f32x4{0.f, 0.f, 0.f, 0.f};
      mm.run(make_rsrc(c.xch + (long)(step + 1) * M3H + xks, (long)KS * M * 2), rowoff, Ws, nkb, acc);
#pragma unroll
      for (int j = 0; j < S; j++) {
        if (j == ks) {
#pragma unroll
          for (int i = 0; i < FM; i++) own[i] = acc[i][j];
        } else {
#pragma unroll
          for (int i = 0; i < FM; i++)
            __builtin_amdgcn_raw_buffer_store_b128(as_u32x4(acc[i][j]), prs, plane + (unsigned)i * 1024u, (unsigned)((j * S + ks) * ptile * 4), 16);
        }
      }
      publish(tcnt);
    }
    float4 gr[FM], gz[FM], gn[FM], gh[FM], hpv[FM], ex[FM];
    if (step >= 0) {
#pragma unroll
      for (int i = 0; i < FM; i++) {
        const long o = (long)row[i] * H + u;
        const __bf16* gp = c.gates + (long)step * 4 * MH + o;
        gr[i] = ld_bf16x4(gp); gz[i] = ld_bf16x4(gp + MH); gn[i] = ld_bf16x4(gp + 2 * MH); gh[i] = ld_bf16x4(gp + 3 * MH);
// ... 14 lines not shown
    if (!last) {
      wait_arrivals<false>(tcnt, (unsigned)(S * (T - 1 - step)), err, dead);
      f32x4 p[S][FM];
#pragma unroll
      for (int q = 0; q < S; q++) {
        if (q == ks) {
#pragma unroll
          for (int i = 0; i < FM; i++) p[q][i] = own[i];
        } else {
#pragma unroll
          for (int i = 0; i < FM; i++)
            p[q][i] = as_f32x4(__builtin_amdgcn_raw_buffer_load_b128(prs, plane + (unsigned)i * 1024u, (unsigned)((ks * S + q) * ptile * 4), 16));
        }
      }
#pragma unroll
      for (int i = 0; i < FM; i++) {
        f32x4 s_ = p[0][i];
#pragma unroll
        for (int q = 1; q < S; q++) s_ += p[q][i];
        sum[i] = s_;
      }
    } else {
#pragma unroll
      for (int i = 0; i < FM; i++) sum[i] = own[i];
    }
    if (step < 0) {
#pragma unroll
      for (int i = 0; i < FM; i++)
        if (ok[i]) *reinterpret_cast<float4*>(c.dh0 + (long)row[i] * H + u) =
            make_float4(sum[i][0] + dhz[i].x, sum[i][1] + dhz[i].y, sum[i][2] + dhz[i].z, sum[i][3] + dhz[i].w);
      break;
    }
    float4 dR[FM], dZ[FM], dN[FM], dNR[FM];
#pragma unroll
    for (int i = 0; i < FM; i++) {
      const float dzn[4] = {dhz[i].x, dhz[i].y, dhz[i].z, dhz[i].w}, e1[4] = {ex[i].x, ex[i].y, ex[i].z, ex[i].w};
      const float R[4] = {gr[i].x, gr[i].y, gr[i].z, gr[i].w}, Z[4] = {gz[i].x, gz[i].y, gz[i].z, gz[i].w};
      const float N[4] = {gn[i].x, gn[i].y, gn[i].z, gn[i].w}, HN[4] = {gh[i].x, gh[i].y, gh[i].z, gh[i].w};
      const float hP[4] = {hpv[i].x, hpv[i].y, hpv[i].z, hpv[i].w};
      float dr[4], dz[4], dn[4], dnr[4], dq[4];
#pragma unroll
      for (int e = 0; e < 4; e++) {
        const float dh = sum[i][e] + dzn[e] + e1[e];
        dn[e] = dh * (1.0f - Z[e]) * (1.0f - N[e] * N[e]);
        dz[e] = dh * (hP[e] - N[e]) * Z[e] * (1.0f - Z[e]);
        dr[e] = dn[e] * HN[e] * R[e] * (1.0f - R[e]);
        dnr[e] = dn[e] * R[e];
        dq[e] = dh * Z[e];
      }
      dhz[i] = make_float4(dq[0], dq[1], dq[2], dq[3]);
      dR[i] = make_float4(dr[0], dr[1], dr[2], dr[3]); dZ[i] = make_float4(dz[0], dz[1], dz[2], dz[3]);
      dN[i] = make_float4(dn[0], dn[1], dn[2], dn[3]);
      dNR[i] = make_float4(dnr[0], dnr[1], dnr[2], dnr[3]);
      if (ok[i]) {
        __bf16* px = c.xch + (long)step * M3H + (long)row[i] * 8 + xe;
        store_bf16x4_sc1(px + (long)((u) >> 3) * M * 8, dr[0], dr[1], dr[2], dr[3]);
        store_bf16x4_sc1(px + (long)((H + u) >> 3) * M * 8, dz[0], dz[1], dz[2], dz[3]);
        store_bf16x4_sc1(px + (long)((2 * H + u) >> 3) * M * 8, dnr[0], dnr[1], dnr[2], dnr[3]);
      }
    }
    if (step > 0 || c.dh0) publish(cnt);
#pragma unroll
    for (int i = 0; i < FM; i++) {
      if (ok[i]) {
        __bf16* ph = c.dgh + (long)step * M3H + (long)row[i] * 3 * H + u;
        st_bf16x4(ph, dR[i].x, dR[i].y, dR[i].z, dR[i].w);
        st_bf16x4(ph + H, dZ[i].x, dZ[i].y, dZ[i].z, dZ[i].w);
        st_bf16x4(ph + 2 * H, dNR[i].x, dNR[i].y, dNR[i].z, dNR[i].w);
        __bf16* pi = c.dgi + (long)t * M3H + (long)row[i] * 3 * H + u;
        st_bf16x4(pi, dR[i].x, dR[i].y, dR[i].z, dR[i].w);
        st_bf16x4(pi + H, dZ[i].x, dZ[i].y, dZ[i].z, dZ[i].w);
        st_bf16x4(pi + 2 * H, dN[i].x, dN[i].y, dN[i].z, dN[i].w);
      }
    }
  }
}

__global__ void pack_blocked_kernel(const float* __restrict__ h, __bf16* __restrict__ x, int M, int H) {
  const long n = (long)M * (H >> 3);
  for (long i = (long)blockIdx.x * blockDim.x + threadIdx.x; i < n; i += (long)gridDim.x * blockDim.x) {
    const int row = (int)(i % M), kc = (int)(i / M);
    const float4 a = *reinterpret_cast<const float4*>(h + (long)row * H + kc * 8);
    const float4 b = *reinterpret_cast<const float4*>(h + (long)row * H + kc * 8 + 4);
    bf16x8 v;
    v[0] = (__bf16)a.x; v[1] = (__bf16)a.y; v[2] = (__bf16)a.z; v[3] = (__bf16)a.w;
    v[4] = (__bf16)b.x; v[5] = (__bf16)b.y; v[6] = (__bf16)b.z; v[7] = (__bf16)b.w;
    *reinterpret_cast<bf16x8*>(x + i * 8) = v;
  }
}

static int g_load_policy = 0, g_dbg = 0;
static int g_num_cu = 0, g_cu_reserve = 0;
static int num_cu() {
  if (g_num_cu == 0) {
    int dev = 0, n = 0;
    if (hipGetDevice(&dev) != hipSuccess || hipDeviceGetAttribute(&n, hipDeviceAttributeMultiprocessorCount, dev) != hipSuccess) n = -1;
    g_num_cu = n;
  }
  return g_num_cu;
}

static int plan(int NC, int M, int H, int& RG, int& rows_wg, int& FM, int fm_max = 4) {
  if (NC < 1 || NC > PMAXC || M <= 0 || H < 256 || H > 1024 || (H & 255)) return PTV_ERR_UNSUPPORTED;
  const int ncu = num_cu() - g_cu_reserve;
  const int UG = H / PU;
  int rg = ncu / (NC * UG);
  if (rg < 1) return PTV_ERR_UNSUPPORTED;
  int p2 = 1; while (p2 * 2 <= rg) p2 *= 2;
  rg = p2;
  while (rg > 1 && (M + rg - 1) / rg < 64 && (M + rg / 2 - 1) / (rg / 2) <= 256) rg /= 2;
  int fm = ((M + rg - 1) / rg + 63) / 64;
  if (fm == 3) fm = 4;
  if (fm > 4 && fm <= 8) fm = 8;
  if (fm > fm_max) return PTV_ERR_UNSUPPORTED;
  RG = rg; rows_wg = fm * 64; FM = fm;
  return PTV_OK;
}
static bool splitk_ok(int H, int S) { return (S == 2 || S == 4) && (H / PU) % S == 0 && (3 * H / S) % 192 == 0; }

}

using namespace ptv;

extern "C" int ptv_gru_persist_load_policy(int lp) {
  if (lp >= 100) { ptv::g_dbg = lp - 100; return PTV_OK; }
  if (lp < 0 || lp > 2) return PTV_ERR_ARG;
  ptv::g_load_policy = lp;
  return PTV_OK;
}

extern "C" int ptv_gru_persist_cu_reserve(int cus) {
  if (cus < 0 || cus > 255) return PTV_ERR_ARG;
  ptv::g_cu_reserve = cus;
  return PTV_OK;
}

extern "C" int ptv_gru_persist_supported(int NC, int M, int H) {
  int RG, rows, FM;
  return plan(NC, M, H, RG, rows, FM) == PTV_OK ? 1 : 0;
}

extern "C" int ptv_gru_persist_fwd(int NC, int M, int H, int T,
                                   const void* const* gi, const long* gi_step, const long* gi_ld,
                                   const void* const* gi2, const long* gi2_step, const long* gi2_ld,
                                   const void* const* w_hh16, const float* const* b_hh,
                                   float* const* hall, void* const* hall16, void* const* gates,
                                   const int* const* lengths, const int* reverse, void* const* xch, unsigned* sync, void* stream) {
  if (T <= 0 || !gi || !gi_step || !gi_ld || !w_hh16 || !b_hh || !hall || !hall16 || !reverse || !xch || !sync) return PTV_ERR_ARG;
  int RG, rows, FM;
  PTV_TRY(plan(NC, M, H, RG, rows, FM));
  PGruFwdArgs a{};
  for (int i = 0; i < NC; i++) {
    if (!gi[i] || !w_hh16[i] || !b_hh[i] || !hall[i] || !hall16[i] || !xch[i]) return PTV_ERR_ARG;
    if ((gi_ld[i] & 3) || (gi_step[i] & 3)) return PTV_ERR_ARG;
    const bool has2 = gi2 && gi2[i];
    if (has2 && ((gi2_ld[i] & 3) || (gi2_step[i] & 3))) return PTV_ERR_ARG;
    a.c[i] = PChainF{(const __bf16*)w_hh16[i], b_hh[i], (const __bf16*)gi[i], gi_step[i], gi_ld[i],
                     has2 ? (const __bf16*)gi2[i] : nullptr, has2 ? gi2_step[i] : 0, has2 ? gi2_ld[i] : 0,
                     hall[i], (__bf16*)hall16[i], gates ? (__bf16*)gates[i] : nullptr, (__bf16*)xch[i],
                     lengths ? lengths[i] : nullptr, reverse[i]};
  }
  a.NC = NC; a.M = M; a.H = H; a.T = T; a.RG = RG; a.UG = H / PU; a.rows_wg = rows; a.sync = sync; a.dbg = g_dbg;
  for (int i = 0; i < NC; i++) {
    PTV_TRY(ptv_cast_bf16(hall[i], hall16[i], (long)M * H, stream));
    long nb = ((long)M * (H >> 3) + 255) / 256; if (nb > 1024) nb = 1024;
    hipLaunchKernelGGL(pack_blocked_kernel, dim3((int)nb), dim3(256), 0, (hipStream_t)stream, hall[i], (__bf16*)xch[i], M, H);
  }
  const dim3 grid(NC * RG * a.UG), block(NTHREADS);
  hipStream_t s = (hipStream_t)stream;
#define PTV_PG_LAUNCH(K, LP_, KK)                                                     \
  do {                                                                                \
    const bool k8 = ((KK) % 512) == 0;                                                \
    if (FM == 1) { if (k8) hipLaunchKernelGGL((K<1, 8, LP_>), grid, block, 0, s, a); else hipLaunchKernelGGL((K<1, 4, LP_>), grid, block, 0, s, a); } \
    else if (FM == 2) hipLaunchKernelGGL((K<2, 4, LP_>), grid, block, 0, s, a);       \
    else hipLaunchKernelGGL((K<4, 2, LP_>), grid, block, 0, s, a);                    \
  } while (0)
  if (g_load_policy == 0) PTV_PG_LAUNCH(pgru_fwd_kernel, 0, H);
  else if (g_load_policy == 1) PTV_PG_LAUNCH(pgru_fwd_kernel, 1, H);
  else PTV_PG_LAUNCH(pgru_fwd_kernel, 2, H);
  PTV_CHECK_LAUNCH();
  return PTV_OK;
}

extern "C" int ptv_gru_persist_bwd(int NC, int M, int H, int T,
                                   const float* const* hall, const void* const* gates, const void* const* w_t16,
                                   const void* const* dh_ext, const long* ext_step, const long* ext_ld, const int* ext_bf16,
                                   const float* const* dh_last, const long* last_ld,
                                   void* const* dgi, void* const* dgh, float* const* dh0,
                                   const int* reverse, void* const* xch, unsigned* sync, void* stream) {
  if (T <= 0 || !hall || !gates || !w_t16 || !dgi || !dgh || !reverse || !xch || !sync) return PTV_ERR_ARG;
  int RG, rows, FM;
  PTV_TRY(plan(NC, M, H, RG, rows, FM));
  PGruBwdArgs a{};
  for (int i = 0; i < NC; i++) {
    if (!hall[i] || !gates[i] || !w_t16[i] || !dgi[i] || !dgh[i] || !xch[i]) return PTV_ERR_ARG;
    const bool hext = dh_ext && dh_ext[i];
    if (hext && ((ext_ld[i] & 3) || (ext_step[i] & 3))) return PTV_ERR_ARG;
    const bool hl = dh_last && dh_last[i];
    if (hl && (last_ld[i] & 3)) return PTV_ERR_ARG;
    a.c[i] = PChainB{(const __bf16*)w_t16[i], hall[i], (const __bf16*)gates[i],
                     hext ? dh_ext[i] : nullptr, hext ? ext_step[i] : 0, hext ? ext_ld[i] : 0, hext && ext_bf16 ? ext_bf16[i] : 0,
                     hl ? dh_last[i] : nullptr, hl ? last_ld[i] : 0,
                     (__bf16*)dgi[i], (__bf16*)dgh[i], dh0 ? dh0[i] : nullptr, (__bf16*)xch[i], reverse[i]};
  }
  a.NC = NC; a.M = M; a.H = H; a.T = T; a.RG = RG; a.UG = H / PU; a.rows_wg = rows; a.sync = sync;
  const dim3 grid(NC * RG * a.UG), block(NTHREADS);
  hipStream_t s = (hipStream_t)stream;
  const int pi = prof::want(6, M, H) ? prof::begin(s) : -1;
  if (g_load_policy == 0) PTV_PG_LAUNCH(pgru_bwd_kernel, 0, 3 * H);
  else if (g_load_policy == 1) PTV_PG_LAUNCH(pgru_bwd_kernel, 1, 3 * H);
  else PTV_PG_LAUNCH(pgru_bwd_kernel, 2, 3 * H);
  if (pi >= 0) prof::end(pi, s, 2.0 * NC * M * 3.0 * H * H * T);
  PTV_CHECK_LAUNCH();
  return PTV_OK;
}

extern "C" int ptv_gru_persist_splitk_supported(int NC, int M, int H, int S) {
  int RG, rows, FM;
  return splitk_ok(H, S) && plan(NC, M, H, RG, rows, FM, 8) == PTV_OK ? 1 : 0;
}

extern "C" long ptv_gru_persist_part_elems(int NC, int M, int H, int S) {
  int RG, rows, FM;
  if (!splitk_ok(H, S) || plan(NC, M, H, RG, rows, FM, 8) != PTV_OK) return 0;
  return 2L * RG * rows * H * S;
}

extern "C" int ptv_gru_persist_bwd_splitk(int S, int NC, int M, int H, int T,
                                          const float* const* hall, const void* const* gates, const void* const* w_t16,
                                          const void* const* dh_ext, const long* ext_step, const long* ext_ld, const int* ext_bf16,
                                          const float* const* dh_last, const long* last_ld,
                                          void* const* dgi, void* const* dgh, float* const* dh0,
                                          const int* reverse, void* const* xch, float* const* part, unsigned* sync, void* stream) {
  if (T <= 0 || !hall || !gates || !w_t16 || !dgi || !dgh || !reverse || !xch || !part || !sync) return PTV_ERR_ARG;
  if (!splitk_ok(H, S)) return PTV_ERR_UNSUPPORTED;
  int RG, rows, FM;
  PTV_TRY(plan(NC, M, H, RG, rows, FM, 8));
  PGruBwdArgs a{};
  for (int i = 0; i < NC; i++) {
    if (!hall[i] || !gates[i] || !w_t16[i] || !dgi[i] || !dgh[i] || !xch[i] || !part[i]) return PTV_ERR_ARG;
    const bool hext = dh_ext && dh_ext[i];
    if (hext && ((ext_ld[i] & 3) || (ext_step[i] & 3))) return PTV_ERR_ARG;
    const bool hl = dh_last && dh_last[i];
    if (hl && (last_ld[i] & 3)) return PTV_ERR_ARG;
    a.c[i] = PChainB{(const __bf16*)w_t16[i], hall[i], (const __bf16*)gates[i],
                     hext ? dh_ext[i] : nullptr, hext ? ext_step[i] : 0, hext ? ext_ld[i] : 0, hext && ext_bf16 ? ext_bf16[i] : 0,
                     hl ? dh_last[i] : nullptr, hl ? last_ld[i] : 0,
                     (__bf16*)dgi[i], (__bf16*)dgh[i], dh0 ? dh0[i] : nullptr, (__bf16*)xch[i], reverse[i], part[i]};
  }
  a.NC = NC; a.M = M; a.H = H; a.T = T; a.RG = RG; a.UG = H / PU; a.rows_wg = rows; a.sync = sync;
  if (NC * RG > 32 || NC * RG * (a.UG / S) > 128) return PTV_ERR_UNSUPPORTED;
  const dim3 grid(NC * RG * a.UG), block(NTHREADS);
  hipStream_t s = (hipStream_t)stream;
#define PTV_SK_LAUNCH(S_)                                                                                  \
  do {                                                                                                     \
    if (FM == 1) hipLaunchKernelGGL((pgru_bwd_sk_kernel<1, 3, S_>), grid, block, 0, s, a);                 \
    else if (FM == 2) hipLaunchKernelGGL((pgru_bwd_sk_kernel<2, 3, S_>), grid, block, 0, s, a);            \
    else if (FM == 4) hipLaunchKernelGGL((pgru_bwd_sk_kernel<4, 3, S_>), grid, block, 0, s, a);            \
    else hipLaunchKernelGGL((pgru_bwd_sk_kernel<8, 1, S_>), grid, block, 0, s, a);                         \
  } while (0)
  const int pi = prof::want(6, M, H) ? prof::begin(s) : -1;
  if (S == 4) PTV_SK_LAUNCH(4); else PTV_SK_LAUNCH(2);
  if (pi >= 0) prof::end(pi, s, 2.0 * NC * M * 3.0 * H * H * T);
  PTV_CHECK_LAUNCH();
  return PTV_OK;
}
```

### polyphonic_chord_texture_disentanglement_amd/functional.py

```python
import contextlib
import ctypes
import os
import time
import weakref

import torch

from . import _lib as _libmod
from ._lib import SlotTable, call, check, lib, prec_code, ptr, stream_ptr


_get_cur = getattr(torch._C, '_cuda_getCurrentStream', None)
_get_dev = getattr(torch._C, '_cuda_getDevice', None)
_set_stream = getattr(torch._C, '_cuda_setStream', None)


def cur_stream():
    if _get_cur is None or _get_dev is None:
        return torch.cuda.current_stream()
    sid, di, dt = _get_cur(_get_dev())
    return torch.cuda.Stream(stream_id=sid, device_index=di, device_type=dt)

F32 = torch.float32
BF16 = torch.bfloat16
# ... 153 lines not shown
    if _row_dense(t):
        return t.as_strided((t.numel() // t.shape[-1], t.shape[-1]), (t.stride(-2), 1), t.storage_offset())
    return t.contiguous().view(-1, t.shape[-1])


def _ld(t):
    assert t.dim() == 2 and t.stride(1) == 1, (t.shape, t.stride())
    return t.stride(0)


CHAIN_PRIO = True
_SIDE_DEPTH = [0, 0]


def _forget_prio():
    _SIDE_DEPTH[1] = -1


if _forget_prio not in _libmod.ERROR_HOOKS:
    _libmod.ERROR_HOOKS.append(_forget_prio)


def _chain_prio():
    if CHAIN_PRIO:
        want = 1 if _SIDE_DEPTH[0] == 0 else 0
        if want != _SIDE_DEPTH[1]:
            lib().ptv_gemm_priority(want)
            _SIDE_DEPTH[1] = want


def gemm(a, b, out=None, *, ta=False, tb=False, bias=None, alpha=1.0, acc=False, act=0, prec=0, splitk=0, out_dtype=F32, m_top=None,
         m_unit=0, out_blocked=False):
    M, K = (a.shape[1], a.shape[0]) if ta else (a.shape[0], a.shape[1])
    N, Kb = (b.shape[1], b.shape[0]) if tb else (b.shape[0], b.shape[1])
    assert K == Kb, (a.shape, b.shape, ta, tb)
    if out is None:
        assert not acc
        out = _empty(M, N, dev=a.device, dtype=out_dtype)
    assert tuple(out.shape) == (M, N), (out.shape, M, N)
    dt = _bf(a) | (_bf(b) << 1) | (_bf(out) << 2)
    if out_blocked:
        assert out_blocked in (True, 16, 32) and N % 32 == 0 and out.is_contiguous()
        dt |= 16 if out_blocked == 16 else 8
    _chain_prio()
    if m_top is not None:
        call('ptv_gemm_mtop', prec, int(ta), int(tb), M, N, K, ptr(a), _ld(a), ptr(b), _ld(b), ptr(out), _ld(out),
             ptr(bias), float(alpha), int(acc), int(act), int(-1 if _bf(out) else splitk), dt, ptr(m_top), int(m_unit), stream_ptr())
        return out
    call('ptv_gemm', prec, int(ta), int(tb), M, N, K, ptr(a), _ld(a), ptr(b), _ld(b), ptr(out), _ld(out),
         ptr(bias), float(alpha), int(acc), int(act), int(-1 if _bf(out) else splitk), dt, stream_ptr())
    return out


def copy2d(dst, src, *, alpha=1.0, acc=False, rows=None, cols=None, lds=None):
    rows = dst.shape[0] if rows is None else rows
    cols = dst.shape[1] if cols is None else cols
    call('ptv_copy2d', ptr(dst), _ld(dst), ptr(src), (_ld(src) if lds is None else lds), rows, cols,
         float(alpha), int(acc), stream_ptr())
    return dst


def colsum(out, a, sel=None, groups=1):
    call('ptv_colsum', ptr(out), ptr(a), _ld(a), a.shape[0], a.shape[1], ptr(sel), groups, _bf(a), stream_ptr())
    return out


def sum_steps(x3, out=None, acc=False, t_top=None):
    T = x3.shape[0]
    n = x3[0].numel()
    assert x3.is_contiguous()
    if out is None:
        out = _empty(*x3.shape[1:], dev=x3.device)
    call('ptv_sum_steps_top', ptr(out), ptr(x3), n, T, n, int(acc), _bf(x3), ptr(t_top), stream_ptr())
    return out


def transpose01(x):
    D0, D1 = x.shape[0], x.shape[1]
    W = x[0, 0].numel()
    x = x.contiguous()
    out = torch.empty((D1, D0) + tuple(x.shape[2:]), device=x.device, dtype=F32)
    call('ptv_transpose01', ptr(out), ptr(x), D0, D1, W, stream_ptr())
    return out


def _WT(p, prec):
    if prec == 1 and BF16_STORAGE and p.dim() == 2:
        from .optim import weight_shadow_t
        return weight_shadow_t(p)
    return None


def gemm_dx(dy, w, cols=None, out=None, *, acc=False, prec=0, m_top=None, m_unit=0, out_blocked=False):
    wt = _WT(w, prec)
    if wt is not None:
        return gemm(dy, wt if cols is None else wt[cols, :], out, acc=acc, prec=prec, m_top=m_top, m_unit=m_unit, out_blocked=out_blocked)
    return gemm(dy, w if cols is None else w[:, cols], out, tb=True, acc=acc, prec=prec, m_top=m_top, m_unit=m_unit, out_blocked=out_blocked)


def _gru_flags(gates=None, gi=None, gi2=None, dg=None, w=None, ext=None):
    return _bf(gates) | (_bf(gi) << 1) | (_bf(gi2) << 2) | (_bf(dg) << 3) | (_bf(w) << 4) | (_bf(ext) << 6)


_PERSIST_LAST = {}
_DEFER = None

# ... 96 lines not shown
    bad = [i for i, sw in enumerate(_PERSIST_SYNC) if int(sw[0].item()) != 0]
    del _PERSIST_SYNC[:]
    badc = [i for i, sw in enumerate(_CLUSTER_SYNC) if int(sw[-1].item()) != 0]
    del _CLUSTER_SYNC[:]
    if bad:
        raise RuntimeError('persistent GRU launch gave up waiting for its row group (recent launches %s)' % bad)
    if badc:
        raise RuntimeError('cluster-mode note loop: a member gave up waiting for its panel (recent forward passes %s)' % badc)


def gru_persist_fwd(M, H, T, chains):
    NC = len(chains)
    g = lambda k: [c.get(k) for c in chains]
    dev = chains[0]['hall'].device
    sync = _persist_sync(NC, dev)
    xch = [torch.empty((T + 1) * M * H, device=dev, dtype=BF16) for _ in chains]
    with _PersistTurn():
        rc = lib().ptv_gru_persist_fwd(NC, M, H, T, _parr(g('gi')), _larr(g('gi_step')), _larr(g('gi_ld')),
                                       _parr(g('gi2')), _larr([c.get('gi2_step', 0) for c in chains]),
                                       _larr([c.get('gi2_ld', 0) for c in chains]), _parr(g('w16')), _parr(g('b_hh')),
                                       _parr(g('hall')), _parr(g('hall16')), _parr(g('gates')), _parr(g('lengths')),
                                       _iarr([int(bool(c.get('reverse'))) for c in chains]), _parr(xch), ptr(sync), stream_ptr())
    check(rc, 'ptv_gru_persist_fwd')


PERSIST_SPLITK = os.environ.get('PTV_PERSIST_SPLITK', 'auto')
PERSIST_SPLITK = PERSIST_SPLITK if PERSIST_SPLITK == 'auto' else int(PERSIST_SPLITK)
_SPLITK_OK = {}


def persist_splitk(NC, M, H):
    S = PERSIST_SPLITK
    if S == 'auto':
        S = 2 if (H >= 1024 and M >= 512) else 0
        if not S and not persist_supported(NC, M, H):
            S = 2
    if S not in (2, 4):
        return 0
    key = (NC, M, H, S, torch.cuda.current_device())
    if key not in _SPLITK_OK:
        _SPLITK_OK[key] = bool(lib().ptv_gru_persist_splitk_supported(NC, M, H, S))
    return S if _SPLITK_OK[key] else 0


def gru_persist_bwd(M, H, T, chains):
    NC = len(chains)
    g = lambda k: [c.get(k) for c in chains]
    ext = g('dh_ext')
    last = g('dh_last')
    dev = chains[0]['hall'].device
    sync = _persist_sync(NC, dev)
    xch = [torch.empty(T * M * 3 * H, device=dev, dtype=BF16) for _ in chains]
    S = persist_splitk(NC, M, H)
    args = (NC, M, H, T, _parr(g('hall')), _parr(g('gates')), _parr(g('wt16')),
            _parr(ext), _larr([e.stride(0) if e is not None else 0 for e in ext]),
            _larr([e.stride(1) if e is not None else 0 for e in ext]),
            _iarr([_bf(e) for e in ext]),
            _parr(last), _larr([l.stride(0) if l is not None else 0 for l in last]),
            _parr(g('dgi')), _parr(g('dgh')), _parr(g('dh0')),
            _iarr([int(bool(c.get('reverse'))) for c in chains]), _parr(xch))
    with _PersistTurn():
        if S:
            n = lib().ptv_gru_persist_part_elems(NC, M, H, S)
            part = [torch.empty(n, device=dev) for _ in chains]
            rc = lib().ptv_gru_persist_bwd_splitk(S, *args, _parr(part), ptr(sync), stream_ptr())
        else:
            rc = lib().ptv_gru_persist_bwd(*args, ptr(sync), stream_ptr())
    check(rc, 'ptv_gru_persist_bwd')


def _persist_fwd_ok(prec, M, H, T, gi, gi2, gates, gi_idx, hall16, w16, NC=1):
    return (prec == 1 and T >= 2 and hall16 is not None and gi.dtype == BF16 and (gi2 is None or gi2.dtype == BF16)
            and (gates is None or gates.dtype == BF16) and gi_idx is None and w16 is not None and w16.dtype == BF16
            and persist_supported(NC, M, H, T))


def gru_fwd(prec, gi, gi_step, gi_ld, w_hh, b_hh, hall, gates, *, gi2=None, gi2_step=0, gi2_ld=0, lengths=None,
            reverse=False, gi_idx=None, T=None, hall16=None, skip_cast0=False):
    T1, M, H = hall.shape
    T = T1 - 1 if T is None else T
    if hall16 is not None:
        w_hh = _W(w_hh, prec)
    if not skip_cast0 and _persist_fwd_ok(prec, M, H, T, gi, gi2, gates, gi_idx, hall16, w_hh):
        return gru_persist_fwd(M, H, T, [dict(gi=gi, gi_step=gi_step, gi_ld=gi_ld, gi2=gi2, gi2_step=gi2_step, gi2_ld=gi2_ld,
                                              w16=w_hh, b_hh=b_hh, hall=hall, hall16=hall16, gates=gates, lengths=lengths,
                                              reverse=reverse)])
    call('ptv_gru_seq_fwd', prec, M, H, T, ptr(gi), gi_step, gi_ld, ptr(gi2), gi2_step, gi2_ld, ptr(w_hh),
         ptr(b_hh), ptr(hall), ptr(hall16), ptr(gates), ptr(lengths), int(reverse), ptr(gi_idx),
         _gru_flags(gates, gi, gi2, w=w_hh) | (32 if skip_cast0 else 0), stream_ptr())


def _hall16(prec, T1, M, H, dev):
    return _empty(T1, M, H, dev=dev, dtype=BF16) if _act_dtype(prec, H) == BF16 else None


def gru_bwd(prec, hall, gates, w_hh, *, dh_ext=None, dh_last=None, lr=None, reverse=False, need_dh0=True, allow_persist=True):
    T1, M, H = hall.shape
    T = T1 - 1
    dev = hall.device
    dt = _act_dtype(prec, H)
    dgi = _empty(T, M, 3 * H, dev=dev, dtype=dt)
    dgh = _empty(T, M, 3 * H, dev=dev, dtype=dt)
    dhz = _empty(2, M, H, dev=dev)
    dh0 = _empty(M, H, dev=dev) if need_dh0 else None
    ext = (ptr(dh_ext), dh_ext.stride(0), dh_ext.stride(1)) if dh_ext is not None else (None, 0, 0)
    last = (ptr(dh_last), dh_last.stride(0)) if dh_last is not None else (None, 0)
    lra = (ptr(lr[0]), lr[1], lr[2], lr[3], ptr(lr[4])) if lr is not None else (None, 0, 0, 0, None)
    if dt == BF16:
        wt = _WT(w_hh, prec)
        if (allow_persist and wt is not None and lr is None and T >= 2 and gates.dtype == BF16 and persist_supported(1, M, H, T)
                and (dh_ext is None or dh_ext.stride(2) == 1)):
            gru_persist_bwd(M, H, T, [dict(hall=hall, gates=gates, wt16=wt, dh_ext=dh_ext, dh_last=dh_last, dgi=dgi, dgh=dgh,
                                           dh0=dh0, reverse=reverse)])
            return dgi, dgh, dh0
        w_hh = wt if wt is not None else w_hh
    call('ptv_gru_seq_bwd', prec, M, H, T, ptr(hall), ptr(gates), ptr(w_hh), *ext, *last, *lra, ptr(dgi),
         ptr(dgh), ptr(dhz), ptr(dh0), int(reverse), _gru_flags(gates, dg=dgi, w=w_hh, ext=dh_ext), stream_ptr())
    return dgi, dgh, dh0


_CHILD_STREAMS = {}
OVERLAP = True


def _record_stream(obj, stream):
    if isinstance(obj, torch.Tensor):
        if obj.is_cuda:
            obj.record_stream(stream)
    elif isinstance(obj, (list, tuple)):
        for o in obj:
            _record_stream(o, stream)
    elif isinstance(obj, dict):
        for o in obj.values():
            _record_stream(o, stream)
    elif hasattr(obj, '__dict__') and not callable(obj):
        for o in vars(obj).values():
            if isinstance(o, (torch.Tensor, list, tuple, dict)):
                _record_stream(o, stream)




POOL_MAP = (0, 1, 2, 3)


class Side:

    def __init__(self, slot=0, chain=False):
        self.main = cur_stream()
        self.chain = chain
        key = ('pool', self.main.device.index, POOL_MAP[slot % 4])
        if key not in _CHILD_STREAMS:
            for k in (1, 2, 0, 3):
                _CHILD_STREAMS.setdefault(('pool', self.main.device.index, k), torch.cuda.Stream(device=self.main.device))
        self.s = _CHILD_STREAMS[key]
        self.keep = []
        self.used = False

    def __call__(self, fn, *keep, after=None):
        if not OVERLAP:
            return fn()
        if after is not None:
            wait_event(self.s, after)
        else:
            wait_stream(self.s, self.main)
        self.used = True
        self.keep.extend(keep)
        depth = 0 if self.chain else 1
        _SIDE_DEPTH[0] += depth
        _chain_prio()
# ... 1155 lines not shown
                'dec_notes_gru.weight_ih_l0', 'dec_time_to_notes_hid.weight', 'dec_time_gru.weight_ih_l0', 'dec_time_gru.weight_hh_l0',
                'z2dec_hid_linear.weight', 'z2dec_in_linear.weight'))))


def _decoder_bwd_composite(P, st, z, tok_op, dP, ddur, top_h, side, G):
    B, R, E, He, Ht, Hn, Hd, NP, prec = (st[k] for k in ('B', 'R', 'E', 'He', 'Ht', 'Hn', 'Hd', 'NP', 'prec'))
    dev = z.device
    M = 15 * R
    HN16, HD16, NS16, gates_n, gates_t = st.get('HN16'), st.get('HD16'), st.get('NS16'), st['gates_n'], st['gates_t']
    if (prec != 1 or not ZERO_SKIP or not OVERLAP or SUMMARY_FAMILY_SLOT >= 0 or torch.cuda.is_current_stream_capturing()
            or not st.get('dur16_only') or st['gates_d'] is not None or st.get('dur_tabs') is None or HD16 is None or HN16 is None
            or NS16 is None or not st.get('gates_n_rowk') or gates_n.dtype != BF16 or gates_t.dtype != BF16 or not HEADS_WGRAD_FUSED
            or not heads_ok(prec, Hn, NP, Hd, HN16, HD16) or not notes_persist_ok(prec, Hn, E, BF16)
            or dP.stride(0) != _pad8(NP) or dP.data_ptr() % 16 or not ddur.is_contiguous() or ddur.dtype != F32
            or tok_op.dtype != F32 or not tok_op.is_contiguous() or z.dtype != F32 or not z.is_contiguous()
            or not persist_supported(1, B, Ht, 32) or side.s == side.main or M * 5 < 4096):
        _defer_flush()
        return None
    wts = [_WT(P[n], prec) for n in ('dec_notes_gru.weight_ih_l0', 'dec_time_to_notes_hid.weight', 'dec_time_gru.weight_ih_l0',
                                      'dec_time_gru.weight_hh_l0', 'z2dec_hid_linear.weight', 'z2dec_in_linear.weight')]
    if any(w is None for w in wts) or st['pitch'].stride(0) != _pad8(NP) or st['idx'].dtype != torch.int32:
        _defer_flush()
        return None
    Zs, Zi = z.shape[1], st['z_in'].shape[1]
    S = persist_splitk(1, B, Ht)
    nblk = min(256, (M + 63) // 64)
    psz = lib().ptv_dur_gru_bwd_part_size()
    dims = {'B': B, 'E': E, 'HE': He, 'HT': Ht, 'HN': Hn, 'HD': Hd, 'NP': NP, 'ZS': Zs, 'ZI': Zi, 'LDP': _pad8(NP), 'NBLK': nblk, 'SPLITK': S}
    hp = heads_packs(P['pitch_out_linear.weight'], P['dur_hid_linear.weight'])
    pk = notes_packs(P['dec_notes_gru.weight_ih_l0'], P['dec_notes_gru.weight_hh_l0'], Ht)
    for _, n in _DTB_G:
        G[n] = _gbuf(P[n])
    dz, dtok, dTOKS = _empty(B, Zs, dev=dev), _empty(16, R, E, dev=dev), _empty(33, B, 2 * He, dev=dev)
    tab0, tab = st['dur_tabs']
    tens = {'Z': z, 'TOK_OP': tok_op, 'DP': dP, 'DDUR': ddur, 'TOP_H': top_h,
            'W_HH_D': P['dec_dur_gru.weight_hh_l0'], 'B_HH_D': P['dec_dur_gru.bias_hh_l0'], 'W_IH_D': P['dec_dur_gru.weight_ih_l0'],
            'W_OUT_D': P['dur_out_linear.weight'], 'SOS': P['dur_sos_token'], 'PK_WDPT': hp['wdpT'], 'PK_WCAT': hp['wcat'],
            'PK_NOTES_WT': pk['wt'], 'WT_IH_N': wts[0], 'WT_T2N': wts[1], 'WT_IH_T': wts[2], 'WT_HH_T': wts[3], 'WT_ZHID': wts[4],
            'WT_ZIN': wts[5], 'NS': st['NS'], 'NS16': NS16, 'Z_IN': st['z_in'], 'TOKS': st['TOKS'], 'GATES_T': gates_t, 'HN16': HN16,
            'GATES_N': gates_n, 'PITCH': st['pitch'], 'HD16': HD16, 'TAB0': tab0, 'TAB': tab, 'IDX': st['idx'],
            'DZ': dz, 'DTOK': dtok, 'DTOKS': dTOKS,
            'DHD0': _empty(M, Hd, dev=dev), 'PART': _empty(nblk, psz, dev=dev), 'S': _zeros(1, psz, dev=dev), 'TMP64': _zeros(1, 64, dev=dev),
            'DNSUM': _empty(M, Hn, dev=dev, dtype=BF16), 'DY16': _empty(M, 200, dev=dev, dtype=BF16), 'TMP200': _empty(200, Hn, dev=dev),
            'CS200': _zeros(200, dev=dev), 'DGI_N': _empty(15, R, 3 * Hn, dev=dev, dtype=BF16), 'DGH_N': _empty(15, R, Hn, dev=dev, dtype=BF16),
            'DHN0': _empty(R, Hn, dev=dev), 'SCRATCH_N': _empty(lib().ptv_notes_gru_persist_scratch_elems(R), dev=dev, dtype=BF16),
            'TOP_STEP': _ineg1(dev), 'DGC': _empty(R, 3 * Hn, dev=dev), 'DNS': _empty(R, Ht, dev=dev),
            'DGI_T': _empty(32, B, 3 * Ht, dev=dev, dtype=BF16), 'DGH_T': _empty(32, B, 3 * Ht, dev=dev, dtype=BF16),
            'DZHID': _empty(B, Ht, dev=dev), 'DZG': _empty(B, 3 * Ht, dev=dev), 'DZ_IN': _empty(B, Zi, dev=dev),
            'XCH': torch.empty(32 * B * 3 * Ht, device=dev, dtype=BF16),
            'PART_T': torch.empty(lib().ptv_gru_persist_part_elems(1, B, Ht, S), device=dev) if S else None,
            'SYNC': _persist_sync(1, dev)}
    srt = st.get('sorted')
    if srt is not None:
        tens.update(PERM=srt['perm'], ROW_LEN=srt['len'], NS16S=srt['NS16S'], TOK_OP=srt['TOK_S'].view(M, E), DNS_S=_empty(R, Ht, dev=dev),
                    DTOK_S=_empty(15, R, E, dev=dev), SEG_N=srt.get('seg_n'))
    if POISON_DEAD_STEPS and top_h is not None and st.get('live_top') is not None:
        _poison(tens['DNSUM'], tens['DGI_N'], tens['DGH_N'], tens['DY16'])
    evs = _fork_events('DTB', 4)
    turn = _CompositeTurn(cur_stream())
    arr_ = _DTB.pointers(tens, {k: G[n] for k, n in _DTB_G},
                         handles={'FORK_EVENT0': evs[0].cuda_event, 'FORK_EVENT1': evs[1].cuda_event, 'FORK_EVENT2': evs[2].cuda_event,
                                  'FORK_EVENT3': evs[3].cuda_event, 'SIDE_STREAM': side.s.cuda_stream, **turn.handles})
    mark('dec_bwd:composite')
    darr_, sp_ = _DTB.dims(dims), stream_ptr()
    rc = _defer_or_run('tf_bwd', (arr_, darr_, tens, turn.prev, turn.done, evs), lambda: lib().ptv_decoder_tf_bwd(arr_, darr_, sp_))
    _SIDE_DEPTH[1] = 1
    if rc == -3:
        raise RuntimeError('ptv_decoder_tf_bwd refused a configuration its Python-side checks accepted')
    check(rc, 'ptv_decoder_tf_bwd')
    turn.taken()
    _DTB.count()
    st['ev_dtoks'] = None
    side.used = True
    side.keep.extend([v for k, v in tens.items() if v is not None] + [st, z, tok_op])
    return dz, dtok, dTOKS, G, side


def decoder_bwd_core(P, st, z, tok_op, dpitch, ddur):
    B, R, E, He, Ht, Hn, Hd, NP, prec = (st[k] for k in ('B', 'R', 'E', 'He', 'Ht', 'Hn', 'Hd', 'NP', 'prec'))
    W = P
    dev = z.device
    M = 15 * R
    G = {n: None for n in DEC_PARAM_NAMES}
    NS, HN, HD, TOKS = st['NS'], st['HN'], st['HD'], st['TOKS']
    NSo = st['NS16'] if st.get('NS16') is not None else NS
    HNo = st['HN16'] if st.get('HN16') is not None else HN
    HDo = st['HD16'] if st.get('HD16') is not None else HD
    NSf_op, NSUM_op = NSo[1:].view(R, Ht), HNo[1:].view(M, Hn)
    side = Side(DEC_WGRAD_SLOT)

    def wgrad(name, dy, x, sub=None):
        if G[name] is None:
            G[name] = _gbuf(P[name])
        out = G[name] if sub is None else G[name][:, sub]
        gemm(dy, x, out, ta=True, tb=True, acc=True, prec=prec)

    def bgrad(name, a):
        G[name] = _bgrad(P[name], a)

    def wgrad_b(name, bname, dy, x, sub=None, k_top=None):
        if G[name] is None:
            G[name] = _gbuf(P[name])
        if bname is not None and G[bname] is None:
            G[bname] = _gbuf(P[bname])
        wgrad_bias(dy, x, G[name] if sub is None else G[name][:, sub], G[bname] if bname is not None else None, prec, k_top, R)

    hint = _loss_top_hint(dpitch, ddur)
# ... 72 lines not shown
        call('ptv_heads_bwd', ptr(dP), dP.stride(0), ptr(dHD0), ptr(hp['wdpT']), ptr(hp['wcat']), ptr(dNSUM),
             int(rowk_bwd) | (2 if bound_n is not None else 0), ptr(dY16), ptr(top_h), R if top_h is not None else 0, M, stream_ptr())
    else:
        gemm_dx(dHD0, w_dh, slice(Hn, None), out=dP, acc=True, prec=prec, m_top=top_h, m_unit=R)

    def head_wgrads():
        if fused_heads and dY16 is not None:
            tmp, cs = _empty(200, Hn, dev=dev), _zeros(200, dev=dev)
            _chain_prio()
            call('ptv_wgrad', 200, Hn, M, ptr(dY16), 200, ptr(NSUM_op), _ld(NSUM_op), ptr(tmp), Hn, 1.0, 0, 3, 0, ptr(cs), ptr(top_h),
                 R if top_h is not None else 0, 0, stream_ptr())
            for name, bname, lo, hi, sub in (('pitch_out_linear.weight', 'pitch_out_linear.bias', 0, NP, None),
                                             ('dur_hid_linear.weight', 'dur_hid_linear.bias', 136, 136 + Hd, slice(0, Hn))):
                if G[name] is None:
                    G[name] = _gbuf(P[name])
                if G[bname] is None:
                    G[bname] = _gbuf(P[bname])
                copy2d(G[name] if sub is None else G[name][:, sub], tmp[lo:hi], acc=True)
                copy2d(G[bname].view(1, -1), cs[lo:hi].view(1, -1), acc=True)
            wgrad_b('dur_hid_linear.weight', None, dHD0, st['pitch'], slice(Hn, None), top_h)
            return
        wgrad_b('dur_hid_linear.weight', 'dur_hid_linear.bias', dHD0, NSUM_op, slice(0, Hn), top_h)
        wgrad_b('dur_hid_linear.weight', None, dHD0, st['pitch'], slice(Hn, None), top_h)
        wgrad_b('pitch_out_linear.weight', 'pitch_out_linear.bias', dP, NSUM_op, None, top_h)
    if not fused_heads:
        gemm_dx(dHD0, w_dh, slice(0, Hn), out=dNSUM, prec=prec, m_top=top_h, m_unit=R, out_blocked=rowk_bwd)
        gemm_dx(dP, w_p, out=dNSUM, acc=True, prec=prec, m_top=top_h, m_unit=R, out_blocked=rowk_bwd)
    side(head_wgrads, dHD0, dP, dY16)

    mark('dec_bwd:head_dx')
    w_hh_n, w_ih_n = W['dec_notes_gru.weight_hh_l0'], W['dec_notes_gru.weight_ih_l0']
    if rowk_bwd:
        pk = notes_packs(w_ih_n, w_hh_n, Ht)
        dgi_n = _empty(15, R, 3 * Hn, dev=dev, dtype=BF16)
        dgh_n = _empty(15, R, Hn, dev=dev, dtype=BF16)
        if POISON_DEAD_STEPS and top_h is not None and st.get('live_top') is not None:
            _poison(dgi_n, dgh_n)
        dHN0 = _empty(R, Hn, dev=dev)
        scratch = _empty(lib().ptv_notes_gru_persist_scratch_elems(R), dev=dev, dtype=BF16)
        top_step = _ineg1(dev) if ZERO_SKIP else None
        call('ptv_notes_gru_persist_bwd_top', ptr(pk['wt']), ptr(st['HN16']), ptr(st['gates_n']), ptr(dNSUM), ptr(dgi_n), ptr(dgh_n), ptr(dHN0),
             ptr(scratch), R, 15, ptr(bound_n if fused_heads else None), ptr(top_step), stream_ptr())
    else:
        top_step = None
        dgi_n, dgh_n, dHN0 = gru_bwd(prec, HN, st['gates_n'], w_hh_n, dh_ext=dNSUM.view(15, R, Hn))
    mark('dec_bwd:notes_bptt')
    dGC = sum_steps(dgi_n, t_top=top_step)

    dtok = _empty(16, R, E, dev=dev)
    dtok[15].zero_()

    def notes_dx():
        gemm_dx(dgi_n.view(M, 3 * Hn), w_ih_n, slice(Ht, None), out=dtok[:15].view(M, E), prec=prec, m_top=top_step, m_unit=R)
        dNS = gemm_dx(dGC, w_ih_n, slice(0, Ht), prec=prec)
        w_tn = W['dec_time_to_notes_hid.weight']
        gemm_dx(dHN0, w_tn, out=dNS, acc=True, prec=prec)
        return dtok, dNS

    def notes_wgrads():
        if dgh_n.shape[-1] == Hn:
            for name in ('dec_notes_gru.weight_hh_l0', 'dec_notes_gru.bias_hh_l0'):
                if G[name] is None:
                    G[name] = _gbuf(P[name])
            gw, gb, h_op = G['dec_notes_gru.weight_hh_l0'], G['dec_notes_gru.bias_hh_l0'], HNo[:15].view(M, Hn)
            wgrad_bias(dgi_n.view(M, 3 * Hn)[:, :2 * Hn], h_op, gw[:2 * Hn], gb[:2 * Hn], prec, top_step, R)
            wgrad_bias(dgh_n.view(M, Hn), h_op, gw[2 * Hn:], gb[2 * Hn:], prec, top_step, R)
        else:
            wgrad_b('dec_notes_gru.weight_hh_l0', 'dec_notes_gru.bias_hh_l0', dgh_n.view(M, 3 * Hn), HNo[:15].view(M, Hn))
        wgrad_b('dec_notes_gru.weight_ih_l0', 'dec_notes_gru.bias_ih_l0', dGC, NSf_op, slice(0, Ht))
        if top_step is not None:
            if G['dec_notes_gru.weight_ih_l0'] is None:
                G['dec_notes_gru.weight_ih_l0'] = _gbuf(P['dec_notes_gru.weight_ih_l0'])
            wgrad_bias(dgi_n.view(M, 3 * Hn), tok_op, G['dec_notes_gru.weight_ih_l0'][:, Ht:], None, prec, top_step, R)
        else:
            wgrad('dec_notes_gru.weight_ih_l0', dgi_n.view(M, 3 * Hn), tok_op, slice(Ht, None))
        wgrad_b('dec_time_to_notes_hid.weight', 'dec_time_to_notes_hid.bias', dHN0, NSf_op)
    dtok, dNS = notes_dx()
    side(notes_wgrads, dgi_n, dgh_n, dGC, dHN0, dNSUM)

    mark('dec_bwd:notes_dx')
    w_hh_t, w_ih_t = W['dec_time_gru.weight_hh_l0'], W['dec_time_gru.weight_ih_l0']
    dgi_t, dgh_t, dzhid = gru_bwd(prec, NS, st['gates_t'], w_hh_t, dh_ext=dNS.view(32, B, Ht))
    mark('dec_bwd:time_bptt')
    dZG = sum_steps(dgi_t)
    dz_in = gemm_dx(dZG, w_ih_t, slice(2 * He, None), prec=prec)
    dTOKS = _empty(33, B, 2 * He, dev=dev)
    dTOKS[32].zero_()
    gemm_dx(dgi_t.view(R, 3 * Ht), w_ih_t, slice(0, 2 * He), out=dTOKS[:32].view(R, 2 * He), prec=prec)
    st['ev_dtoks'] = record_event() if SUMMARY_FAMILY_SLOT >= 0 and OVERLAP else None
    w_zh, w_zi = W['z2dec_hid_linear.weight'], W['z2dec_in_linear.weight']
    dz = gemm_dx(dzhid, w_zh, prec=prec)
    gemm_dx(dz_in, w_zi, out=dz, acc=True, prec=prec)

    def time_wgrads():
        wgrad_b('dec_time_gru.weight_hh_l0', 'dec_time_gru.bias_hh_l0', dgh_t.view(R, 3 * Ht), NSo[:32].view(R, Ht))
        wgrad_b('dec_time_gru.weight_ih_l0', 'dec_time_gru.bias_ih_l0', dZG, st['z_in'], slice(2 * He, None))
        wgrad('dec_time_gru.weight_ih_l0', dgi_t.view(R, 3 * Ht), TOKS[:32].view(R, 2 * He), slice(0, 2 * He))
        wgrad_b('z2dec_hid_linear.weight', 'z2dec_hid_linear.bias', dzhid, z)
        wgrad_b('z2dec_in_linear.weight', 'z2dec_in_linear.bias', dz_in, z)
        bgrad('dec_init_input', dTOKS[0])
    side(time_wgrads, dgi_t, dgh_t, dZG, dTOKS, dzhid, dz_in, dNS)
    side.keep.extend((st, z, tok_op))
    return dz, dtok, dTOKS, G, side


CHD_PARAM_NAMES = ['init_input', 'z2dec_hid.weight', 'z2dec_hid.bias', 'z2dec_in.weight', 'z2dec_in.bias',
                   'gru.weight_ih_l0', 'gru.weight_hh_l0', 'gru.bias_ih_l0', 'gru.bias_hh_l0',
                   'root_out.weight', 'root_out.bias', 'chroma_out.weight', 'chroma_out.bias',
                   'bass_out.weight', 'bass_out.bias']


CHD_BWD_COMPOSITE = os.environ.get('PTV_BWD_COMPOSITES', '1') != '0'
_CDB = SlotTable('CDB')


def _chord_decoder_bwd_composite(P, st, z, droot, dchroma, dbass):
    prec, T, B, H, I = st['prec'], st['T'], st['B'], st['H'], st['I']
    dev = z.device
    hall, gates, toks, z_in = st['hall'], st['gates'], st['toks'], st['z_in']
    dls = []
    for dl in (droot, dchroma, dbass):
        if dl is not None:
            dl = dl.contiguous()
            if dl.dtype != F32:
                return None
        dls.append(dl)
    adt = _act_dtype(prec, H)
    if (torch.cuda.is_current_stream_capturing() or hall.dtype != F32 or gates.dtype != adt or z.dtype != F32 or not z.is_contiguous()
            or not hall.is_contiguous() or not gates.is_contiguous() or not toks.is_contiguous() or not z_in.is_contiguous()):
        return None
    w_hh = P['gru.weight_hh_l0']
    wt = _WT(w_hh, prec) if adt == BF16 else None
    persist = bool(adt == BF16 and wt is not None and T >= 2 and persist_supported(1, B, H, T))
    S = persist_splitk(1, B, H) if persist else 0
    Z, Zi = z.shape[1], z_in.shape[1]
    dims = {'B': B, 'T': T, 'H': H, 'I': I, 'Z': Z, 'ZI': Zi, 'PREC': prec, 'ACT_BF16': adt == BF16, 'NROOT': P['root_out.weight'].shape[0],
            'NCHROMA': P['chroma_out.weight'].shape[0], 'NBASS': P['bass_out.weight'].shape[0], 'PERSIST': persist, 'SPLITK': S}
    G = {n: _gbuf(P[n]) for n in CHD_PARAM_NAMES}
    dz = _empty(B, Z, dev=dev)
    tens = {'Z': z, 'W_ZHID': P['z2dec_hid.weight'], 'W_ZIN': P['z2dec_in.weight'], 'W_IH': P['gru.weight_ih_l0'], 'W_HH': w_hh,
            'W_ROOT': P['root_out.weight'], 'W_CHROMA': P['chroma_out.weight'], 'W_BASS': P['bass_out.weight'], 'WT16_HH': wt,
            'HALL': hall, 'GATES': gates, 'TOKS': toks, 'Z_IN': z_in, 'DROOT': dls[0], 'DCHROMA': dls[1], 'DBASS': dls[2], 'DZ': dz,
            'G_INIT_INPUT': G['init_input'], 'G_W_ZHID': G['z2dec_hid.weight'], 'G_B_ZHID': G['z2dec_hid.bias'], 'G_W_ZIN': G['z2dec_in.weight'],
            'G_B_ZIN': G['z2dec_in.bias'], 'G_W_IH': G['gru.weight_ih_l0'], 'G_B_IH': G['gru.bias_ih_l0'], 'G_W_HH': G['gru.weight_hh_l0'],
            'G_B_HH': G['gru.bias_hh_l0'], 'G_W_ROOT': G['root_out.weight'], 'G_B_ROOT': G['root_out.bias'], 'G_W_CHROMA': G['chroma_out.weight'],
# ... 533 lines not shown
```

Baseline: 82000 samples/s.

## Fuse dual-K dx GEMMs, row-scatter epilogue, and in-BPTT dgi step sum

Adds a two-operand GEMM (ptv_gemm2) that sums two A·B products in one kernel and can scatter output rows through a row map. This replaces pairs of dx GEMMs plus a separate scatter_rows pass in the decoder backward. It also lets the persistent GRU backward kernel accumulate the time-summed dgi (dZG) directly, dropping the separate sum_steps launch. The cost is fewer launches and less intermediate traffic, but the fused path disables split-K and adds per-row indirection in the epilogue.

```diff
diff --git a/include/ptvae_hip.h b/include/ptvae_hip.h
--- a/include/ptvae_hip.h
+++ b/include/ptvae_hip.h
@@ -33,6 +33,10 @@
 int ptv_gemm_mtop_seg(int prec, int transA, int transB, int M, int N, int K, const void* A, long lda, const void* B, long ldb,
                       void* C, long ldc, const float* bias, float alpha, int accumulate, int act, int splitk, int dtypes,
                       const int* m_top, long m_unit, const int* seg_n, long seg_unit, int seg_period, void* stream);
+int ptv_gemm2(int prec, int transA, int transB, int M, int N, int K, const void* A, long lda, const void* B, long ldb,
+              int K2, const void* A2, long lda2, const void* B2, long ldb2, int dtypes2,
+              void* C, long ldc, const float* bias, float alpha, int accumulate, int act, int splitk, int dtypes,
+              const int* m_top, long m_unit, const int* row_map, void* stream);
 int ptv_gemm_priority(int p);
 
 int ptv_gru_seq_fwd(int prec, int M, int H, int T,
@@ -72,7 +76,8 @@
                         const void* const* dh_ext, const long* ext_step, const long* ext_ld, const int* ext_bf16,
                         const float* const* dh_last, const long* last_ld,
                         void* const* dgi, void* const* dgh, float* const* dh0,
-                        const int* reverse, void* const* xch, unsigned* sync, void* stream);
+                        const int* reverse, void* const* xch, float* const* dgi_sum, unsigned* sync, void* stream);
+int ptv_gru_persist_dgi_sum_supported(int NC, int M, int H, int S);
 int ptv_gru_persist_splitk_supported(int NC, int M, int H, int S);
 long ptv_gru_persist_part_elems(int NC, int M, int H, int S);
 int ptv_gru_persist_bwd_splitk(int S, int NC, int M, int H, int T,
@@ -80,7 +85,7 @@
                                const void* const* dh_ext, const long* ext_step, const long* ext_ld, const int* ext_bf16,
                                const float* const* dh_last, const long* last_ld,
                                void* const* dgi, void* const* dgh, float* const* dh0,
-                               const int* reverse, void* const* xch, float* const* part, unsigned* sync, void* stream);
+                               const int* reverse, void* const* xch, float* const* part, float* const* dgi_sum, unsigned* sync, void* stream);
 
 int ptv_copy2d(float* dst, long ldd, const float* src, long lds, long rows, int cols, float alpha,
                int accumulate, void* stream);
diff --git a/polyphonic_chord_texture_disentanglement_amd/csrc/composite.hip b/polyphonic_chord_texture_disentanglement_amd/csrc/composite.hip
--- a/polyphonic_chord_texture_disentanglement_amd/csrc/composite.hip
+++ b/polyphonic_chord_texture_disentanglement_amd/csrc/composite.hip
@@ -199,9 +199,9 @@
     void* xch_[1] = {M_<void>(t, PTV_CDB_XCH)}; float* part_[1] = {M_<float>(t, PTV_CDB_PART)};
     if (t[PTV_CDB_WAIT_EVENT] && hipStreamWaitEvent(s, (hipEvent_t)const_cast<void*>(t[PTV_CDB_WAIT_EVENT]), 0) != hipSuccess) return PTV_ERR_LAUNCH;
     if (S) PTV_TRY(ptv_gru_persist_bwd_splitk(S, 1, B, H, T, hall_, gates_, wt_, ext_, ext_step, ext_ld, ext_bf, last_, last_ld, dgi_, dgh_, dh0_, rev,
-                                              xch_, part_, M_<unsigned>(t, PTV_CDB_SYNC), stream));
+                                              xch_, part_, nullptr, M_<unsigned>(t, PTV_CDB_SYNC), stream));
     else PTV_TRY(ptv_gru_persist_bwd(1, B, H, T, hall_, gates_, wt_, ext_, ext_step, ext_ld, ext_bf, last_, last_ld, dgi_, dgh_, dh0_, rev, xch_,
-                                     M_<unsigned>(t, PTV_CDB_SYNC), stream));
+                                     nullptr, M_<unsigned>(t, PTV_CDB_SYNC), stream));
     if (t[PTV_CDB_RECORD_EVENT] && hipEventRecord((hipEvent_t)const_cast<void*>(t[PTV_CDB_RECORD_EVENT]), s) != hipSuccess) return PTV_ERR_LAUNCH;
   } else {
     const void* w = t[PTV_CDB_WT16_HH] ? T_(t, PTV_CDB_WT16_HH) : T_(t, PTV_CDB_W_HH);
@@ -237,7 +237,7 @@
         i != PTV_DTB_ROW_LEN && i != PTV_DTB_NS16S && i != PTV_DTB_DNS_S && i != PTV_DTB_DTOK_S && i != PTV_DTB_SEG_N)
       return PTV_ERR_ARG;
   const bool sorted = t[PTV_DTB_PERM] != nullptr;
-  if (sorted != (t[PTV_DTB_ROW_LEN] != nullptr) || sorted != (t[PTV_DTB_NS16S] != nullptr) || sorted != (t[PTV_DTB_DNS_S] != nullptr) ||
+  if (sorted != (t[PTV_DTB_ROW_LEN] != nullptr) || sorted != (t[PTV_DTB_NS16S] != nullptr) ||
       sorted != (t[PTV_DTB_DTOK_S] != nullptr) || (sorted && !t[PTV_DTB_TOP_H]))
     return PTV_ERR_ARG;
   const int* perm = (const int*)T_(t, PTV_DTB_PERM);
@@ -306,7 +306,6 @@
   float* dHN0 = GB(PTV_DTB_DHN0); int* top_step = M_<int>(t, PTV_DTB_TOP_STEP);
   float* dGC = GB(PTV_DTB_DGC);
   float* dNS_out = GB(PTV_DTB_DNS); float* dtok_out = GB(PTV_DTB_DTOK);
-  float* dNS = sorted ? GB(PTV_DTB_DNS_S) : dNS_out;
   float* dtok = sorted ? GB(PTV_DTB_DTOK_S) : dtok_out;
   const __bf16* wt_ih_n = (const __bf16*)T_(t, PTV_DTB_WT_IH_N);
   ptv_gemm_priority(1);
@@ -316,10 +315,9 @@
   if (hipMemsetAsync(dtok_out + 15L * R * E, 0, sizeof(float) * R * E, s) != hipSuccess) return PTV_ERR_LAUNCH;
   PTV_TRY(ptv_gemm_mtop_seg(P, 0, 0, (int)M, E, 3 * Hn, dgi_n, 3L * Hn, wt_ih_n + (long)Ht * 3 * Hn, 3L * Hn, dtok, E, nullptr, 1.f, 0, 0, 0, A16 | B16,
                             top_step, R, seg_n, R, 15, stream));
-  PTV_TRY(ptv_gemm(P, 0, 0, R, Ht, 3 * Hn, dGC, 3L * Hn, wt_ih_n, 3L * Hn, dNS, Ht, nullptr, 1.f, 0, 0, 0, B16, stream));
-  PTV_TRY(ptv_gemm(P, 0, 0, R, Ht, Hn, dHN0, Hn, T_(t, PTV_DTB_WT_T2N), Hn, dNS, Ht, nullptr, 1.f, 1, 0, 0, B16, stream));
+  PTV_TRY(ptv_gemm2(P, 0, 0, R, Ht, 3 * Hn, dGC, 3L * Hn, wt_ih_n, 3L * Hn, Hn, dHN0, Hn, T_(t, PTV_DTB_WT_T2N), Hn, B16, dNS_out, Ht, nullptr, 1.f, 0,
+                    0, 0, B16, nullptr, 0, sorted ? perm : nullptr, stream));
   if (sorted) {
-    PTV_TRY(ptv_scatter_rows(dNS_out, dNS, perm, R, Ht, 0, 0, 1, stream));
     PTV_TRY(ptv_scatter_rows_seg(dtok_out, dtok, perm, R, E, (long)R * E, (long)R * E, 15, seg_n, stream));
   }
   PTV_TRY(fork(2));
@@ -341,6 +339,7 @@
   float* dzhid = GB(PTV_DTB_DZHID); float* dZG = GB(PTV_DTB_DZG); float* dz_in = GB(PTV_DTB_DZ_IN); float* dTOKS = GB(PTV_DTB_DTOKS);
   float* dz = GB(PTV_DTB_DZ);
   const __bf16* wt_ih_t = (const __bf16*)T_(t, PTV_DTB_WT_IH_T);
+  const bool sum_in_bptt = ptv_gru_persist_dgi_sum_supported(1, B, Ht, S) != 0;
   ptv_gemm_priority(1);
   {
     const float* hall_[1] = {(const float*)T_(t, PTV_DTB_NS)}; const void* gates_[1] = {T_(t, PTV_DTB_GATES_T)};
@@ -349,19 +348,20 @@
     const float* last_[1] = {nullptr}; const long last_ld[1] = {0};
     void* dgi_[1] = {dgi_t}; void* dgh_[1] = {dgh_t}; float* dh0_[1] = {dzhid}; const int rev[1] = {0};
     void* xch_[1] = {M_<void>(t, PTV_DTB_XCH)}; float* part_[1] = {M_<float>(t, PTV_DTB_PART_T)};
+    float* sum_[1] = {sum_in_bptt ? dZG : nullptr};
     if (t[PTV_DTB_WAIT_EVENT] && hipStreamWaitEvent(s, (hipEvent_t)const_cast<void*>(t[PTV_DTB_WAIT_EVENT]), 0) != hipSuccess) return PTV_ERR_LAUNCH;
     if (S) PTV_TRY(ptv_gru_persist_bwd_splitk(S, 1, B, Ht, 32, hall_, gates_, wt_, ext_, ext_step, ext_ld, ext_bf, last_, last_ld, dgi_, dgh_, dh0_,
-                                              rev, xch_, part_, M_<unsigned>(t, PTV_DTB_SYNC), stream));
+                                              rev, xch_, part_, sum_, M_<unsigned>(t, PTV_DTB_SYNC), stream));
     else PTV_TRY(ptv_gru_persist_bwd(1, B, Ht, 32, hall_, gates_, wt_, ext_, ext_step, ext_ld, ext_bf, last_, last_ld, dgi_, dgh_, dh0_, rev, xch_,
-                                     M_<unsigned>(t, PTV_DTB_SYNC), stream));
+                                     sum_, M_<unsigned>(t, PTV_DTB_SYNC), stream));
     if (t[PTV_DTB_RECORD_EVENT] && hipEventRecord((hipEvent_t)const_cast<void*>(t[PTV_DTB_RECORD_EVENT]), s) != hipSuccess) return PTV_ERR_LAUNCH;
   }
-  PTV_TRY(ptv_sum_steps_top(dZG, dgi_t, (long)B * 3 * Ht, 32, (long)B * 3 * Ht, 0, 1, nullptr, stream));
+  if (!sum_in_bptt) PTV_TRY(ptv_sum_steps_top(dZG, dgi_t, (long)B * 3 * Ht, 32, (long)B * 3 * Ht, 0, 1, nullptr, stream));
   PTV_TRY(ptv_gemm(P, 0, 0, B, Zi, 3 * Ht, dZG, 3L * Ht, wt_ih_t + 2L * He * 3 * Ht, 3L * Ht, dz_in, Zi, nullptr, 1.f, 0, 0, 0, B16, stream));
   if (hipMemsetAsync(dTOKS + 32L * B * 2 * He, 0, sizeof(float) * B * 2 * He, s) != hipSuccess) return PTV_ERR_LAUNCH;
   PTV_TRY(ptv_gemm(P, 0, 0, R, 2 * He, 3 * Ht, dgi_t, 3L * Ht, wt_ih_t, 3L * Ht, dTOKS, 2L * He, nullptr, 1.f, 0, 0, 0, A16 | B16, stream));
-  PTV_TRY(ptv_gemm(P, 0, 0, B, Zs, Ht, dzhid, Ht, T_(t, PTV_DTB_WT_ZHID), Ht, dz, Zs, nullptr, 1.f, 0, 0, 0, B16, stream));
-  PTV_TRY(ptv_gemm(P, 0, 0, B, Zs, Zi, dz_in, Zi, T_(t, PTV_DTB_WT_ZIN), Zi, dz, Zs, nullptr, 1.f, 1, 0, 0, B16, stream));
+  PTV_TRY(ptv_gemm2(P, 0, 0, B, Zs, Ht, dzhid, Ht, T_(t, PTV_DTB_WT_ZHID), Ht, Zi, dz_in, Zi, T_(t, PTV_DTB_WT_ZIN), Zi, B16, dz, Zs, nullptr, 1.f, 0, 0,
+                    0, B16, nullptr, 0, nullptr, stream));
   PTV_TRY(fork(3));
   ptv_gemm_priority(0);
   {
@@ -413,9 +413,9 @@
     float* part_[2] = {M_<float>(t, PTV_BGB_PART0), M_<float>(t, PTV_BGB_PART1)};
     if (t[PTV_BGB_WAIT_EVENT] && hipStreamWaitEvent(s, (hipEvent_t)const_cast<void*>(t[PTV_BGB_WAIT_EVENT]), 0) != hipSuccess) return PTV_ERR_LAUNCH;
     if (S) PTV_TRY(ptv_gru_persist_bwd_splitk(S, 2, M, H, T, hall_, gates_, wt_, ext_, ext_step, ext_ld, ext_bf, last_, last_ld, dgi, dgh, dh0_, rev,
-                                              xch_, part_, M_<unsigned>(t, PTV_BGB_SYNC), stream));
+                                              xch_, part_, nullptr, M_<unsigned>(t, PTV_BGB_SYNC), stream));
     else PTV_TRY(ptv_gru_persist_bwd(2, M, H, T, hall_, gates_, wt_, ext_, ext_step, ext_ld, ext_bf, last_, last_ld, dgi, dgh, dh0_, rev, xch_,
-                                     M_<unsigned>(t, PTV_BGB_SYNC), stream));
+                                     nullptr, M_<unsigned>(t, PTV_BGB_SYNC), stream));
     if (t[PTV_BGB_RECORD_EVENT] && hipEventRecord((hipEvent_t)const_cast<void*>(t[PTV_BGB_RECORD_EVENT]), s) != hipSuccess) return PTV_ERR_LAUNCH;
   }
   const void* x = T_(t, PTV_BGB_X);
diff --git a/polyphonic_chord_texture_disentanglement_amd/csrc/gemm.hip b/polyphonic_chord_texture_disentanglement_amd/csrc/gemm.hip
--- a/polyphonic_chord_texture_disentanglement_amd/csrc/gemm.hip
+++ b/polyphonic_chord_texture_disentanglement_amd/csrc/gemm.hip
@@ -7,19 +7,22 @@
 
 namespace ptv {
 
-struct EpiPlain {
-  struct Params {
-    void* C; long ldc;
-    const float* bias;
-    float alpha;
-    int accumulate;
-    int act;
-    int atomic;
-    int c_bf16;
-    int c_blocked;
-    int c_rows;
-    long split_stride;
-  };
+struct EpiPlainParams {
+  void* C; long ldc;
+  const float* bias;
+  float alpha;
+  int accumulate;
+  int act;
+  int atomic;
+  int c_bf16;
+  int c_blocked;
+  int c_rows;
+  long split_stride;
+  const int* row_map = nullptr;
+};
+template <bool EXT>
+struct EpiPlainT {
+  using Params = EpiPlainParams;
   static __device__ __forceinline__ long coff(const Params& p, int m, int n) {
     return p.c_blocked ? (((long)(n >> p.c_blocked) * p.c_rows + m) << p.c_blocked) + (n & ((1 << p.c_blocked) - 1)) : (long)m * p.ldc + n;
   }
@@ -86,7 +89,9 @@
       for (int c = 0; c < RS::PASSES; c++) {
         const int row = RS::row(c);
         const f32x4 a = RS::get(st, row, u);
-        const long off = coff(p, m0 + i * 16 + row, n);
+        int m = m0 + i * 16 + row;
+        if constexpr (EXT) { if (p.row_map) m = p.row_map[m]; }
+        const long off = coff(p, m, n);
         float v0 = p.alpha * a[0] + b4.x, v1 = p.alpha * a[1] + b4.y, v2 = p.alpha * a[2] + b4.z, v3 = p.alpha * a[3] + b4.w;
         if constexpr (MODE == 1 || MODE == 4) {
           if constexpr (MODE == 4) {
@@ -115,6 +120,7 @@
       if (use_bias && n + e < N) v[e] += p.bias[n + e];
       if (p.act == 1) v[e] = expf(v[e]);
     }
+    if constexpr (EXT) { if (p.row_map) m = p.row_map[m]; }
     const long off = coff(p, m, n);
     if (p.atomic) {
       float* c = reinterpret_cast<float*>(p.C) + off;
@@ -129,6 +135,7 @@
     }
   }
 };
+using EpiPlain = EpiPlainT<false>;
 
 #ifndef PTV_PF_TN
 #define PTV_PF_TN 3
@@ -138,10 +145,10 @@
 #endif
 #define PLAIN_PF_BIG(KA, KB, SA, SB) ((SA) && (SB) ? ((KA) ? PTV_PF_TN : PTV_PF_NT) : 1)
 
-template <class CT, int BM, int BN, int WGM, int WGN, bool KA, bool KB, bool SA, bool SB>
-__global__ __launch_bounds__(NTHREADS, 2) void gemm_plain_kernel(GemmArgs g, EpiPlain::Params ep) {
+template <class CT, int BM, int BN, int WGM, int WGN, bool KA, bool KB, bool SA, bool SB, bool EXT = false>
+__global__ __launch_bounds__(NTHREADS, 2) void gemm_plain_kernel(GemmArgs g, EpiPlainParams ep) {
   if (g.prio) __builtin_amdgcn_s_setprio(3);
-  gemm_body<CT, BM, BN, WGM, WGN, 1, KA, KB, EpiPlain, SA, SB, (BM * BN <= 64 * 64 ? 2 : PLAIN_PF_BIG(KA, KB, SA, SB))>(g, ep);
+  gemm_body<CT, BM, BN, WGM, WGN, 1, KA, KB, EpiPlainT<EXT>, SA, SB, (BM * BN <= 64 * 64 ? 2 : PLAIN_PF_BIG(KA, KB, SA, SB)), EXT>(g, ep);
 }
 
 __global__ void splitk_reduce_kernel(float* __restrict__ C, long ldc, const float* __restrict__ ws, int M, int N, int splits, int accumulate) {
@@ -160,10 +167,10 @@
   for (; i < total; i += (long)gridDim.x * blockDim.x) C[(i / N) * ldc + (i % N)] = v;
 }
 
-template <class CT, int BM, int BN, bool KA, bool KB, bool SA, bool SB>
+template <class CT, int BM, int BN, bool KA, bool KB, bool SA, bool SB, bool EXT = false>
 static void launch_plain(const GemmArgs& g, const EpiPlain::Params& ep, int splits, hipStream_t s) {
   dim3 grid(cdiv(g.N, BN), cdiv(g.M, BM), splits);
-  hipLaunchKernelGGL((gemm_plain_kernel<CT, BM, BN, 2, 2, KA, KB, SA, SB>), grid, dim3(NTHREADS), 0, s, g, ep);
+  hipLaunchKernelGGL((gemm_plain_kernel<CT, BM, BN, 2, 2, KA, KB, SA, SB, EXT>), grid, dim3(NTHREADS), 0, s, g, ep);
 }
 
 int g_splitk_ordered = [] { const char* e = getenv("PTV_WGRAD_ORDERED"); return (e && e[0] == '0') ? 0 : 1; }();
@@ -194,8 +201,9 @@
   const int bm = big ? 128 : 64;
   long blocks = (long)cdiv(g.M, bm) * cdiv(g.N, bm);
   int splits = 1;
+  const bool one_pass = g.K2 > 0 || ep.row_map != nullptr;
   if (splitk > 0) splits = splitk;
-  else if (splitk == 0 && blocks < 256 && g.K >= 8 * CT::BK && ep.act == 0 && !ep.c_bf16) {
+  else if (splitk == 0 && !one_pass && blocks < 256 && g.K >= 8 * CT::BK && ep.act == 0 && !ep.c_bf16) {
     const long target = deepk ? (big ? 640 : 1536) : 512;
     splits = (int)((target + blocks - 1) / blocks);
     int maxs = g.K / (4 * CT::BK);
@@ -203,6 +211,7 @@
     if (splits > 192) splits = 192;
     if (splits < 1) splits = 1;
   }
+  if (one_pass && (splits > 1 || transA || transB)) return PTV_ERR_UNSUPPORTED;
   int kper = g.K;
   if (splits > 1) {
     if (splits >= 8) splits = (splits + 7) / 8 * 8;
@@ -236,7 +245,10 @@
     if (big) launch_plain<CT, 128, 128, KA, KB, SA, SB>(g, ep, splits, s);      \
     else launch_plain<CT, 64, 64, KA, KB, SA, SB>(g, ep, splits, s);            \
   } while (0)
-  if (!transA && !transB) PTV_LAUNCH(false, false);
+  if (one_pass) {
+    if (big) launch_plain<CT, 128, 128, false, false, SA, SB, true>(g, ep, 1, s);
+    else launch_plain<CT, 64, 64, false, false, SA, SB, true>(g, ep, 1, s);
+  } else if (!transA && !transB) PTV_LAUNCH(false, false);
   else if (!transA && transB) PTV_LAUNCH(false, true);
   else if (transA && transB) PTV_LAUNCH(true, true);
   else PTV_LAUNCH(true, false);
@@ -262,26 +274,28 @@
                            stream);
 }
 
-extern "C" int ptv_gemm_mtop_seg(int prec, int transA, int transB, int M, int N, int K,
-                                 const void* A, long lda, const void* B, long ldb,
-                                 void* C, long ldc, const float* bias, float alpha,
-                                 int accumulate, int act, int splitk, int dtypes, const int* m_top, long m_unit,
-                                 const int* seg_n, long seg_unit, int seg_period, void* stream) {
-  if (M < 0 || N < 0 || K < 0 || !A || !B || !C) return PTV_ERR_ARG;
+static int gemm_run(int prec, int transA, int transB, int M, int N, int K, const void* A, long lda, const void* B, long ldb,
+                    int K2, const void* A2, long lda2, const void* B2, long ldb2,
+                    void* C, long ldc, const float* bias, float alpha, int accumulate, int act, int splitk, int dtypes,
+                    const int* m_top, long m_unit, const int* seg_n, long seg_unit, int seg_period, const int* row_map, void* stream) {
+  if (M < 0 || N < 0 || K < 0 || K2 < 0 || !A || !B || !C || (K2 > 0 && (!A2 || !B2))) return PTV_ERR_ARG;
   if (M == 0 || N == 0) return PTV_OK;
   const bool sa = dtypes & 1, sb = dtypes & 2, sc = dtypes & 4;
+  const bool one_pass = K2 > 0 || row_map != nullptr;
   if ((sa || sb) && prec != PTV_PREC_BF16) return PTV_ERR_ARG;
   if (sc && splitk > 1) return PTV_ERR_ARG;
   if ((dtypes & 8) && (dtypes & 16)) return PTV_ERR_ARG;
   if ((dtypes & 8) && ((N & 31) || splitk > 1)) return PTV_ERR_ARG;
   if ((dtypes & 16) && ((N & 15) || splitk > 1)) return PTV_ERR_ARG;
+  if ((dtypes & 24) && row_map) return PTV_ERR_UNSUPPORTED;
   if ((dtypes & 24) && splitk == 0) splitk = 1;
-  if (prec == PTV_PREC_BF16 && transA && transB && !sc && !(dtypes & 24) && !bias && act == 0 && K >= 512 && splitk <= 0)
+  if (prec == PTV_PREC_BF16 && transA && transB && !sc && !(dtypes & 24) && !bias && act == 0 && K >= 512 && splitk <= 0 && !one_pass)
     return ptv_wgrad(M, N, K, A, lda, B, ldb, reinterpret_cast<float*>(C), ldc, alpha, accumulate, dtypes & 3, 0, nullptr, nullptr, 0, 0, stream);
   if (m_top && (transA || m_unit <= 0)) return PTV_ERR_ARG;
   if (seg_n && (transA || seg_unit <= 0 || (seg_unit & 127) || seg_period <= 0)) return PTV_ERR_ARG;
   ptv::GemmArgs g{A, lda, B, ldb, M, N, K, K, 0, m_top, m_unit, ptv::g_gemm_prio, seg_n, (int)seg_unit, seg_period};
-  ptv::EpiPlain::Params ep{C, ldc, bias, alpha, accumulate, act, 0, sc ? 1 : 0, (dtypes & 8) ? 5 : ((dtypes & 16) ? 4 : 0), M, 0};
+  if (K2 > 0) { g.A2 = A2; g.lda2 = lda2; g.B2 = B2; g.ldb2 = ldb2; g.K2 = K2; }
+  ptv::EpiPlain::Params ep{C, ldc, bias, alpha, accumulate, act, 0, sc ? 1 : 0, (dtypes & 8) ? 5 : ((dtypes & 16) ? 4 : 0), M, 0, row_map};
   hipStream_t s = (hipStream_t)stream;
   int rc;
   if (prec != PTV_PREC_BF16) rc = ptv::gemm_dispatch<ptv::F32, false, false>(transA, transB, g, ep, splitk, s);
@@ -294,6 +308,25 @@
   return PTV_OK;
 }
 
+extern "C" int ptv_gemm_mtop_seg(int prec, int transA, int transB, int M, int N, int K,
+                                 const void* A, long lda, const void* B, long ldb,
+                                 void* C, long ldc, const float* bias, float alpha,
+                                 int accumulate, int act, int splitk, int dtypes, const int* m_top, long m_unit,
+                                 const int* seg_n, long seg_unit, int seg_period, void* stream) {
+  return gemm_run(prec, transA, transB, M, N, K, A, lda, B, ldb, 0, nullptr, 0, nullptr, 0, C, ldc, bias, alpha, accumulate, act, splitk, dtypes, m_top,
+                  m_unit, seg_n, seg_unit, seg_period, nullptr, stream);
+}
+
+extern "C" int ptv_gemm2(int prec, int transA, int transB, int M, int N, int K,
+                         const void* A, long lda, const void* B, long ldb,
+                         int K2, const void* A2, long lda2, const void* B2, long ldb2, int dtypes2,
+                         void* C, long ldc, const float* bias, float alpha,
+                         int accumulate, int act, int splitk, int dtypes, const int* m_top, long m_unit, const int* row_map, void* stream) {
+  if (K2 > 0 && ((dtypes2 ^ dtypes) & 3)) return PTV_ERR_UNSUPPORTED;
+  return gemm_run(prec, transA, transB, M, N, K, A, lda, B, ldb, K2, A2, lda2, B2, ldb2, C, ldc, bias, alpha, accumulate, act, splitk, dtypes, m_top,
+                  m_unit, nullptr, 0, 0, row_map, stream);
+}
+
 extern "C" int ptv_gemm(int prec, int transA, int transB, int M, int N, int K,
                         const void* A, long lda, const void* B, long ldb,
                         void* C, long ldc, const float* bias, float alpha,
diff --git a/polyphonic_chord_texture_disentanglement_amd/csrc/gemm_core.hpp b/polyphonic_chord_texture_disentanglement_amd/csrc/gemm_core.hpp
--- a/polyphonic_chord_texture_disentanglement_amd/csrc/gemm_core.hpp
+++ b/polyphonic_chord_texture_disentanglement_amd/csrc/gemm_core.hpp
@@ -55,6 +55,9 @@
   const int* m_top; long m_unit;
   int prio;
   const int* seg_n = nullptr; int seg_unit = 0, seg_period = 0;
+  const void* A2 = nullptr; long lda2 = 0;
+  const void* B2 = nullptr; long ldb2 = 0;
+  int K2 = 0;
 };
 
 template <class CT> __device__ __forceinline__ int swz(int row, int k) {
@@ -325,7 +328,7 @@
   }
 };
 
-template <class CT, int BM, int BN, int WGM, int WGN, int NG, bool KMAJOR_A, bool KMAJOR_B, class Epi, bool SA = false, bool SB = false, int PF = 1>
+template <class CT, int BM, int BN, int WGM, int WGN, int NG, bool KMAJOR_A, bool KMAJOR_B, class Epi, bool SA = false, bool SB = false, int PF = 1, bool PAIR = false>
 __device__ __forceinline__ void gemm_body(const GemmArgs& g, const typename Epi::Params& ep) {
   static_assert(WGM * WGN == 4, "4 waves");
   static_assert(!(NG == 3 && KMAJOR_B), "gate gather needs K-contiguous weights");
@@ -366,18 +369,13 @@
   const bool dead = (g.m_top != nullptr && m_blk >= ((long)*g.m_top + 1) * g.m_unit) ||
                     (g.seg_n != nullptr && (m_blk % g.seg_unit) >= g.seg_n[(m_blk / g.seg_unit) % g.seg_period]);
   if (dead && Epi::dead_is_noop(ep)) return;
-  const int kend = dead ? kbeg : min(g.K, kbeg + g.k_per_split);
+  const int kend1 = dead ? kbeg : min(g.K, kbeg + g.k_per_split);
   const int wave = threadIdx.x >> 6;
   const int wm = wave / WGN, wn = wave % WGN;
 
   static_assert(!(SA || SB) || std::is_same<CT, BF16>::value, "bf16 sources feed the bf16 MFMA path only");
   using TA = typename SrcT<SA>::T;
   using TB = typename SrcT<SB>::T;
-  const TA* Ap = reinterpret_cast<const TA*>(g.A);
-  const TB* Bp = reinterpret_cast<const TB*>(g.B);
-  const bool vecA = ((g.lda & (SA ? 7 : 3)) == 0) && ((reinterpret_cast<uintptr_t>(g.A) & 15) == 0);
-  const bool vecB = ((g.ldb & (SB ? 7 : 3)) == 0) && ((reinterpret_cast<uintptr_t>(g.B) & 15) == 0);
-
   auto rowmapA = [&](int r) -> long { long m = m_blk + r; return m < g.M ? m : -1; };
   auto rowmapB = [&](int r) -> long {
     const int gate = r / BN, jj = r % BN;
@@ -397,6 +395,9 @@
 #pragma unroll
     for (int j = 0; j < NG * FN; j++) acc[i][j] = f32x4{0.f, 0.f, 0.f, 0.f};
 
+  auto kpass = [&](const TA* Ap, const TB* Bp, const long lda, const long ldb, const int kbeg, const int kend) __attribute__((always_inline)) {
+  const bool vecA = ((lda & (SA ? 7 : 3)) == 0) && ((reinterpret_cast<uintptr_t>(Ap) & 15) == 0);
+  const bool vecB = ((ldb & (SB ? 7 : 3)) == 0) && ((reinterpret_cast<uintptr_t>(Bp) & 15) == 0);
   const bool fullA = vecA && (m_blk + BM <= g.M);
   const bool fullB = vecB && (n_blk + BN <= g.N);
   auto rowfastA = [&](int r) -> long { return m_blk + r; };
@@ -405,25 +406,25 @@
   auto load_tiles = [&](auto& sa_, auto& sb_, int k0) {
     const bool kfull = k0 + CT::BK <= kend;
     if (fullA && kfull) {
-      if constexpr (KMAJOR_A) sa_.load_fast(Ap, g.lda, k0, m_blk);
-      else sa_.load_fast(Ap, g.lda, k0, rowfastA);
+      if constexpr (KMAJOR_A) sa_.load_fast(Ap, lda, k0, m_blk);
+      else sa_.load_fast(Ap, lda, k0, rowfastA);
     } else {
-      if constexpr (KMAJOR_A) sa_.load(Ap, g.lda, k0, kend, vecA, m_blk, g.M);
-      else sa_.load(Ap, g.lda, k0, kend, vecA, rowmapA);
+      if constexpr (KMAJOR_A) sa_.load(Ap, lda, k0, kend, vecA, m_blk, g.M);
+      else sa_.load(Ap, lda, k0, kend, vecA, rowmapA);
     }
     if (fullB && kfull) {
-      if constexpr (KMAJOR_B) sb_.load_fast(Bp, g.ldb, k0, n_blk);
-      else sb_.load_fast(Bp, g.ldb, k0, rowfastB);
+      if constexpr (KMAJOR_B) sb_.load_fast(Bp, ldb, k0, n_blk);
+      else sb_.load_fast(Bp, ldb, k0, rowfastB);
     } else {
-      if constexpr (KMAJOR_B) sb_.load(Bp, g.ldb, k0, kend, vecB, n_blk, g.N);
-      else sb_.load(Bp, g.ldb, k0, kend, vecB, rowmapB);
+      if constexpr (KMAJOR_B) sb_.load(Bp, ldb, k0, kend, vecB, n_blk, g.N);
+      else sb_.load(Bp, ldb, k0, kend, vecB, rowmapB);
     }
   };
   auto fast_tiles = [&](auto& sa_, auto& sb_, int k0) {
-    if constexpr (KMAJOR_A) sa_.load_fast(Ap, g.lda, k0, m_blk);
-    else sa_.load_fast(Ap, g.lda, k0, rowfastA);
-    if constexpr (KMAJOR_B) sb_.load_fast(Bp, g.ldb, k0, n_blk);
-    else sb_.load_fast(Bp, g.ldb, k0, rowfastB);
+    if constexpr (KMAJOR_A) sa_.load_fast(Ap, lda, k0, m_blk);
+    else sa_.load_fast(Ap, lda, k0, rowfastA);
+    if constexpr (KMAJOR_B) sb_.load_fast(Bp, ldb, k0, n_blk);
+    else sb_.load_fast(Bp, ldb, k0, rowfastB);
   };
   auto consume = [&](auto& sa_, auto& sb_) {
     __syncthreads();
@@ -463,6 +464,11 @@
     if (k0 + CT::BK < kend) load_tiles(sa[0], sb[0], k0 + CT::BK);
     mma();
   }
+  };
+  kpass(reinterpret_cast<const TA*>(g.A), reinterpret_cast<const TB*>(g.B), g.lda, g.ldb, kbeg, kend1);
+  if constexpr (PAIR) {
+    if (g.K2 > 0) kpass(reinterpret_cast<const TA*>(g.A2), reinterpret_cast<const TB*>(g.B2), g.lda2, g.ldb2, 0, dead ? 0 : g.K2);
+  }
   if constexpr (EPI_BYTES > 0) __syncthreads();
   Epi::template apply<FM, FN, NG>(ep, acc, pre, m_blk + wm * WTM, n_blk + wn * WTN, g.M, g.N, split, smem);
 }
diff --git a/polyphonic_chord_texture_disentanglement_amd/csrc/gru_persist.hip b/polyphonic_chord_texture_disentanglement_amd/csrc/gru_persist.hip
--- a/polyphonic_chord_texture_disentanglement_amd/csrc/gru_persist.hip
+++ b/polyphonic_chord_texture_disentanglement_amd/csrc/gru_persist.hip
@@ -37,6 +37,7 @@
   __bf16* xch;
   int reverse;
   float* part;
+  float* dgi_sum;
 };
 struct PGruBwdArgs {
   PChainB c[PMAXC];
@@ -59,6 +60,10 @@
   const bf16x4 v = *reinterpret_cast<const bf16x4*>(p);
   return make_float4((float)v[0], (float)v[1], (float)v[2], (float)v[3]);
 }
+__device__ __forceinline__ void add_bf16r(float4& s, const float (&v)[4]) {
+  s.x += (float)(__bf16)v[0]; s.y += (float)(__bf16)v[1]; s.z += (float)(__bf16)v[2]; s.w += (float)(__bf16)v[3];
+}
+constexpr bool dgi_sum_fits(int FM) { return FM <= 4; }
 __device__ __forceinline__ void st_bf16x4(__bf16* p, float a, float b, float c, float d) {
   bf16x4 v; v[0] = (__bf16)a; v[1] = (__bf16)b; v[2] = (__bf16)c; v[3] = (__bf16)d;
   *reinterpret_cast<bf16x4*>(p) = v;
@@ -262,6 +267,11 @@
   const int u = u0 + kq * 4;
   const int row0 = rg * a.rows_wg + wave * (FM * 16);
   int row[FM]; bool ok[FM]; unsigned rowoff[FM]; float4 dhz[FM];
+  constexpr int FS = dgi_sum_fits(FM) ? FM : 1;
+  const bool want_sum = dgi_sum_fits(FM) && c.dgi_sum != nullptr;
+  float4 sR[FS], sZ[FS], sN[FS];
+#pragma unroll
+  for (int i = 0; i < FS; i++) sR[i] = sZ[i] = sN[i] = make_float4(0.f, 0.f, 0.f, 0.f);
 #pragma unroll
   for (int i = 0; i < FM; i++) {
     const int r = row0 + i * 16 + rl;
@@ -333,6 +343,9 @@
       dR[i] = make_float4(dr[0], dr[1], dr[2], dr[3]); dZ[i] = make_float4(dz[0], dz[1], dz[2], dz[3]);
       dN[i] = make_float4(dn[0], dn[1], dn[2], dn[3]);
       dNR[i] = make_float4(dnr[0], dnr[1], dnr[2], dnr[3]);
+      if constexpr (dgi_sum_fits(FM)) {
+        if (want_sum) { add_bf16r(sR[i], dr); add_bf16r(sZ[i], dz); add_bf16r(sN[i], dn); }
+      }
       if (ok[i]) {
         __bf16* px = c.xch + (long)step * M3H + (long)row[i] * 8 + xe;
         store_bf16x4_sc1(px + (long)((u) >> 3) * M * 8, dr[0], dr[1], dr[2], dr[3]);
@@ -353,6 +366,18 @@
         st_bf16x4(pi + H, dZ[i].x, dZ[i].y, dZ[i].z, dZ[i].w);
         st_bf16x4(pi + 2 * H, dN[i].x, dN[i].y, dN[i].z, dN[i].w);
       }
+    }
+  }
+  if constexpr (dgi_sum_fits(FM)) {
+    if (want_sum) {
+#pragma unroll
+      for (int i = 0; i < FM; i++)
+        if (ok[i]) {
+          float* ps = c.dgi_sum + (long)row[i] * 3 * H + u;
+          *reinterpret_cast<float4*>(ps) = sR[i];
+          *reinterpret_cast<float4*>(ps + H) = sZ[i];
+          *reinterpret_cast<float4*>(ps + 2 * H) = sN[i];
+        }
     }
   }
 }
@@ -388,6 +413,11 @@
   const int rw0 = wave * (FM * 16);
   const int row0 = rg * a.rows_wg + rw0;
   int row[FM]; bool ok[FM]; unsigned rowoff[FM]; float4 dhz[FM];
+  constexpr int FS = dgi_sum_fits(FM) ? FM : 1;
+  const bool want_sum = dgi_sum_fits(FM) && c.dgi_sum != nullptr;
+  float4 sR[FS], sZ[FS], sN[FS];
+#pragma unroll
+  for (int i = 0; i < FS; i++) sR[i] = sZ[i] = sN[i] = make_float4(0.f, 0.f, 0.f, 0.f);
 #pragma unroll
   for (int i = 0; i < FM; i++) {
     const int r = row0 + i * 16 + rl;
@@ -508,6 +538,9 @@
       dR[i] = make_float4(dr[0], dr[1], dr[2], dr[3]); dZ[i] = make_float4(dz[0], dz[1], dz[2], dz[3]);
       dN[i] = make_float4(dn[0], dn[1], dn[2], dn[3]);
       dNR[i] = make_float4(dnr[0], dnr[1], dnr[2], dnr[3]);
+      if constexpr (dgi_sum_fits(FM)) {
+        if (want_sum) { add_bf16r(sR[i], dr); add_bf16r(sZ[i], dz); add_bf16r(sN[i], dn); }
+      }
       if (ok[i]) {
         __bf16* px = c.xch + (long)step * M3H + (long)row[i] * 8 + xe;
         store_bf16x4_sc1(px + (long)((u) >> 3) * M * 8, dr[0], dr[1], dr[2], dr[3]);
@@ -528,6 +561,18 @@
         st_bf16x4(pi + H, dZ[i].x, dZ[i].y, dZ[i].z, dZ[i].w);
         st_bf16x4(pi + 2 * H, dN[i].x, dN[i].y, dN[i].z, dN[i].w);
       }
+    }
+  }
+  if constexpr (dgi_sum_fits(FM)) {
+    if (want_sum) {
+#pragma unroll
+      for (int i = 0; i < FM; i++)
+        if (ok[i]) {
+          float* ps = c.dgi_sum + (long)row[i] * 3 * H + u;
+          *reinterpret_cast<float4*>(ps) = sR[i];
+          *reinterpret_cast<float4*>(ps + H) = sZ[i];
+          *reinterpret_cast<float4*>(ps + 2 * H) = sN[i];
+        }
     }
   }
 }
@@ -594,6 +639,12 @@
 extern "C" int ptv_gru_persist_supported(int NC, int M, int H) {
   int RG, rows, FM;
   return plan(NC, M, H, RG, rows, FM) == PTV_OK ? 1 : 0;
+}
+
+extern "C" int ptv_gru_persist_dgi_sum_supported(int NC, int M, int H, int S) {
+  int RG, rows, FM;
+  if (S ? (!splitk_ok(H, S) || plan(NC, M, H, RG, rows, FM, 8) != PTV_OK) : plan(NC, M, H, RG, rows, FM) != PTV_OK) return 0;
+  return dgi_sum_fits(FM) ? 1 : 0;
 }
 
 extern "C" int ptv_gru_persist_fwd(int NC, int M, int H, int T,
@@ -643,7 +694,7 @@
                                    const void* const* dh_ext, const long* ext_step, const long* ext_ld, const int* ext_bf16,
                                    const float* const* dh_last, const long* last_ld,
                                    void* const* dgi, void* const* dgh, float* const* dh0,
-                                   const int* reverse, void* const* xch, unsigned* sync, void* stream) {
+                                   const int* reverse, void* const* xch, float* const* dgi_sum, unsigned* sync, void* stream) {
   if (T <= 0 || !hall || !gates || !w_t16 || !dgi || !dgh || !reverse || !xch || !sync) return PTV_ERR_ARG;
   int RG, rows, FM;
   PTV_TRY(plan(NC, M, H, RG, rows, FM));
@@ -657,7 +708,8 @@
     a.c[i] = PChainB{(const __bf16*)w_t16[i], hall[i], (const __bf16*)gates[i],
                      hext ? dh_ext[i] : nullptr, hext ? ext_step[i] : 0, hext ? ext_ld[i] : 0, hext && ext_bf16 ? ext_bf16[i] : 0,
                      hl ? dh_last[i] : nullptr, hl ? last_ld[i] : 0,
-                     (__bf16*)dgi[i], (__bf16*)dgh[i], dh0 ? dh0[i] : nullptr, (__bf16*)xch[i], reverse[i]};
+                     (__bf16*)dgi[i], (__bf16*)dgh[i], dh0 ? dh0[i] : nullptr, (__bf16*)xch[i], reverse[i], nullptr, dgi_sum ? dgi_sum[i] : nullptr};
+    if (a.c[i].dgi_sum && !dgi_sum_fits(FM)) return PTV_ERR_UNSUPPORTED;
   }
   a.NC = NC; a.M = M; a.H = H; a.T = T; a.RG = RG; a.UG = H / PU; a.rows_wg = rows; a.sync = sync;
   const dim3 grid(NC * RG * a.UG), block(NTHREADS);
@@ -687,7 +739,8 @@
                                           const void* const* dh_ext, const long* ext_step, const long* ext_ld, const int* ext_bf16,
                                           const float* const* dh_last, const long* last_ld,
                                           void* const* dgi, void* const* dgh, float* const* dh0,
-                                          const int* reverse, void* const* xch, float* const* part, unsigned* sync, void* stream) {
+                                          const int* reverse, void* const* xch, float* const* part, float* const* dgi_sum, unsigned* sync,
+                                          void* stream) {
   if (T <= 0 || !hall || !gates || !w_t16 || !dgi || !dgh || !reverse || !xch || !part || !sync) return PTV_ERR_ARG;
   if (!splitk_ok(H, S)) return PTV_ERR_UNSUPPORTED;
   int RG, rows, FM;
@@ -702,7 +755,8 @@
     a.c[i] = PChainB{(const __bf16*)w_t16[i], hall[i], (const __bf16*)gates[i],
                      hext ? dh_ext[i] : nullptr, hext ? ext_step[i] : 0, hext ? ext_ld[i] : 0, hext && ext_bf16 ? ext_bf16[i] : 0,
                      hl ? dh_last[i] : nullptr, hl ? last_ld[i] : 0,
-                     (__bf16*)dgi[i], (__bf16*)dgh[i], dh0 ? dh0[i] : nullptr, (__bf16*)xch[i], reverse[i], part[i]};
+                     (__bf16*)dgi[i], (__bf16*)dgh[i], dh0 ? dh0[i] : nullptr, (__bf16*)xch[i], reverse[i], part[i], dgi_sum ? dgi_sum[i] : nullptr};
+    if (a.c[i].dgi_sum && !dgi_sum_fits(FM)) return PTV_ERR_UNSUPPORTED;
   }
   a.NC = NC; a.M = M; a.H = H; a.T = T; a.RG = RG; a.UG = H / PU; a.rows_wg = rows; a.sync = sync;
   if (NC * RG > 32 || NC * RG * (a.UG / S) > 128) return PTV_ERR_UNSUPPORTED;
diff --git a/polyphonic_chord_texture_disentanglement_amd/functional.py b/polyphonic_chord_texture_disentanglement_amd/functional.py
--- a/polyphonic_chord_texture_disentanglement_amd/functional.py
+++ b/polyphonic_chord_texture_disentanglement_amd/functional.py
@@ -229,6 +229,28 @@
     return out
 
 
+def gemm2(a, b, a2, b2, out, *, acc=False, prec=0, m_top=None, m_unit=0, row_map=None):
+    (M, K), (N, Kb), (M2, K2), (N2, K2b) = a.shape, b.shape, a2.shape, b2.shape
+    assert K == Kb and K2 == K2b and M == M2 and N == N2 and tuple(out.shape) == (M, N), (a.shape, b.shape, a2.shape, b2.shape, out.shape)
+    assert _bf(a) == _bf(a2) and _bf(b) == _bf(b2)
+    dt = _bf(a) | (_bf(b) << 1) | (_bf(out) << 2)
+    _chain_prio()
+    call('ptv_gemm2', prec, 0, 0, M, N, K, ptr(a), _ld(a), ptr(b), _ld(b), K2, ptr(a2), _ld(a2), ptr(b2), _ld(b2), dt & 3,
+         ptr(out), _ld(out), None, 1.0, int(acc), 0, 0, dt, ptr(m_top), int(m_unit), ptr(row_map), stream_ptr())
+    return out
+
+
+def gemm_dx2(dy, w, cols, dy2, w2, out=None, *, prec=0):
+    wt, wt2 = _WT(w, prec), _WT(w2, prec)
+    if wt is not None and wt2 is not None and dy.dtype == dy2.dtype:
+        b = wt if cols is None else wt[cols, :]
+        if out is None:
+            out = _empty(dy.shape[0], b.shape[0], dev=dy.device)
+        return gemm2(dy, b, dy2, wt2, out, prec=prec)
+    out = gemm_dx(dy, w, cols, out=out, prec=prec)
+    return gemm_dx(dy2, w2, out=out, acc=True, prec=prec)
+
+
 def copy2d(dst, src, *, alpha=1.0, acc=False, rows=None, cols=None, lds=None):
     rows = dst.shape[0] if rows is None else rows
     cols = dst.shape[1] if cols is None else cols
@@ -431,6 +453,9 @@
     sync = _persist_sync(NC, dev)
     xch = [torch.empty(T * M * 3 * H, device=dev, dtype=BF16) for _ in chains]
     S = persist_splitk(NC, M, H)
+    sums = g('dgi_sum')
+    sum_in_kernel = any(x is not None for x in sums) and bool(lib().ptv_gru_persist_dgi_sum_supported(NC, M, H, S))
+    ksums = _parr(sums) if sum_in_kernel else None
     args = (NC, M, H, T, _parr(g('hall')), _parr(g('gates')), _parr(g('wt16')),
             _parr(ext), _larr([e.stride(0) if e is not None else 0 for e in ext]),
             _larr([e.stride(1) if e is not None else 0 for e in ext]),
@@ -442,10 +467,14 @@
         if S:
             n = lib().ptv_gru_persist_part_elems(NC, M, H, S)
             part = [torch.empty(n, device=dev) for _ in chains]
-            rc = lib().ptv_gru_persist_bwd_splitk(S, *args, _parr(part), ptr(sync), stream_ptr())
+            rc = lib().ptv_gru_persist_bwd_splitk(S, *args, _parr(part), ksums, ptr(sync), stream_ptr())
         else:
-            rc = lib().ptv_gru_persist_bwd(*args, ptr(sync), stream_ptr())
+            rc = lib().ptv_gru_persist_bwd(*args, ksums, ptr(sync), stream_ptr())
     check(rc, 'ptv_gru_persist_bwd')
+    if not sum_in_kernel:
+        for c in chains:
+            if c.get('dgi_sum') is not None:
+                sum_steps(c['dgi'], out=c['dgi_sum'])
 
 
 def _persist_fwd_ok(prec, M, H, T, gi, gi2, gates, gi_idx, hall16, w16, NC=1):
@@ -473,7 +502,7 @@
     return _empty(T1, M, H, dev=dev, dtype=BF16) if _act_dtype(prec, H) == BF16 else None
 
 
-def gru_bwd(prec, hall, gates, w_hh, *, dh_ext=None, dh_last=None, lr=None, reverse=False, need_dh0=True, allow_persist=True):
+def gru_bwd(prec, hall, gates, w_hh, *, dh_ext=None, dh_last=None, lr=None, reverse=False, need_dh0=True, allow_persist=True, dgi_sum=None):
     T1, M, H = hall.shape
     T = T1 - 1
     dev = hall.device
@@ -490,11 +519,13 @@
         if (allow_persist and wt is not None and lr is None and T >= 2 and gates.dtype == BF16 and persist_supported(1, M, H, T)
                 and (dh_ext is None or dh_ext.stride(2) == 1)):
             gru_persist_bwd(M, H, T, [dict(hall=hall, gates=gates, wt16=wt, dh_ext=dh_ext, dh_last=dh_last, dgi=dgi, dgh=dgh,
-                                           dh0=dh0, reverse=reverse)])
+                                           dh0=dh0, reverse=reverse, dgi_sum=dgi_sum)])
             return dgi, dgh, dh0
         w_hh = wt if wt is not None else w_hh
     call('ptv_gru_seq_bwd', prec, M, H, T, ptr(hall), ptr(gates), ptr(w_hh), *ext, *last, *lra, ptr(dgi),
          ptr(dgh), ptr(dhz), ptr(dh0), int(reverse), _gru_flags(gates, dg=dgi, w=w_hh, ext=dh_ext), stream_ptr())
+    if dgi_sum is not None:
+        sum_steps(dgi, out=dgi_sum)
     return dgi, dgh, dh0
 
 
@@ -1756,7 +1787,7 @@
             'SYNC': _persist_sync(1, dev)}
     srt = st.get('sorted')
     if srt is not None:
-        tens.update(PERM=srt['perm'], ROW_LEN=srt['len'], NS16S=srt['NS16S'], TOK_OP=srt['TOK_S'].view(M, E), DNS_S=_empty(R, Ht, dev=dev),
+        tens.update(PERM=srt['perm'], ROW_LEN=srt['len'], NS16S=srt['NS16S'], TOK_OP=srt['TOK_S'].view(M, E),
                     DTOK_S=_empty(15, R, E, dev=dev), SEG_N=srt.get('seg_n'))
     if POISON_DEAD_STEPS and top_h is not None and st.get('live_top') is not None:
         _poison(tens['DNSUM'], tens['DGI_N'], tens['DGH_N'], tens['DY16'])
@@ -1935,9 +1966,7 @@
 
     def notes_dx():
         gemm_dx(dgi_n.view(M, 3 * Hn), w_ih_n, slice(Ht, None), out=dtok[:15].view(M, E), prec=prec, m_top=top_step, m_unit=R)
-        dNS = gemm_dx(dGC, w_ih_n, slice(0, Ht), prec=prec)
-        w_tn = W['dec_time_to_notes_hid.weight']
-        gemm_dx(dHN0, w_tn, out=dNS, acc=True, prec=prec)
+        dNS = gemm_dx2(dGC, w_ih_n, slice(0, Ht), dHN0, W['dec_time_to_notes_hid.weight'], prec=prec)
         return dtok, dNS
 
     def notes_wgrads():
@@ -1963,17 +1992,16 @@
 
     mark('dec_bwd:notes_dx')
     w_hh_t, w_ih_t = W['dec_time_gru.weight_hh_l0'], W['dec_time_gru.weight_ih_l0']
-    dgi_t, dgh_t, dzhid = gru_bwd(prec, NS, st['gates_t'], w_hh_t, dh_ext=dNS.view(32, B, Ht))
+    dZG = _empty(B, 3 * Ht, dev=dev)
+    dgi_t, dgh_t, dzhid = gru_bwd(prec, NS, st['gates_t'], w_hh_t, dh_ext=dNS.view(32, B, Ht), dgi_sum=dZG)
     mark('dec_bwd:time_bptt')
-    dZG = sum_steps(dgi_t)
     dz_in = gemm_dx(dZG, w_ih_t, slice(2 * He, None), prec=prec)
     dTOKS = _empty(33, B, 2 * He, dev=dev)
     dTOKS[32].zero_()
     gemm_dx(dgi_t.view(R, 3 * Ht), w_ih_t, slice(0, 2 * He), out=dTOKS[:32].view(R, 2 * He), prec=prec)
     st['ev_dtoks'] = record_event() if SUMMARY_FAMILY_SLOT >= 0 and OVERLAP else None
     w_zh, w_zi = W['z2dec_hid_linear.weight'], W['z2dec_in_linear.weight']
-    dz = gemm_dx(dzhid, w_zh, prec=prec)
-    gemm_dx(dz_in, w_zi, out=dz, acc=True, prec=prec)
+    dz = gemm_dx2(dzhid, w_zh, None, dz_in, w_zi, prec=prec)
 
     def time_wgrads():
         wgrad_b('dec_time_gru.weight_hh_l0', 'dec_time_gru.bias_hh_l0', dgh_t.view(R, 3 * Ht), NSo[:32].view(R, Ht))
```

New measurement: 77890 samples/s. -5.0%, worse.
